# electronicarts/mesh2splat

Measured on AMD Instinct MI355X. Metric: Gaussians/sec emitted (mesh->3DGS conversion pass, density 1024^2), higher is better.
Workload: dtype f32

## Files before the change

### __graft_entry__.py

```python
import os
import subprocess
import sys

ROOT = os.path.dirname(os.path.abspath(__file__))
if ROOT not in sys.path:
    sys.path.insert(0, ROOT)


def build() -> None:
    from mesh2splat_amd import _lib
    _lib.build(force=False)
    _lib.load()
    subprocess.run(["make", "-C", os.path.join(ROOT, "oracle"), "all"], check=True, stdout=subprocess.DEVNULL)
    subprocess.run(["make", "-C", os.path.join(ROOT, "tests", "stub_rccl")], check=True, stdout=subprocess.DEVNULL)
    subprocess.run(["make", "-C", os.path.join(ROOT, "tests", "exact_math")], check=True, stdout=subprocess.DEVNULL)
    import mesh2splat_amd


def smoke() -> None:
    import numpy as np
    from mesh2splat_amd import synth
    from mesh2splat_amd.converter import ConversionPass, RenderContext
    from oracle import oracle

    scene = synth.cube_sphere(24, tex_size=64)
    ctx = RenderContext(scene, resolutionTarget=128, device=0)
    ConversionPass().execute(ctx)
    rec = ctx.converter.download()
    total, ref, _ = oracle.convert(scene, 128)
    assert ctx.numberOfGaussians == total, (ctx.numberOfGaussians, total)
    sys.path.insert(0, os.path.join(ROOT, "tests"))
    from parity import assert_records_match
    assert_records_match(rec, ref, "smoke")
    ran = [ctx.converter.last_pipeline]
    for pipe in ("multipass", "team", "lean"):
        ctx.converter.set_pipeline(pipe)
        assert ctx.converter.convert(128) == total
        assert np.array_equal(ctx.converter.download().view(np.uint32), rec.view(np.uint32)), pipe
        ran.append(ctx.converter.last_pipeline)
    import camera
    from mesh2splat_amd.prepass import PrepassParams
    pp = PrepassParams(view_mat=camera.look_at((1.6, 1.1, 2.3), (0.1, 0.0, -0.1)), proj_mat=camera.perspective(45.0, 16 / 9, 0.01, 100.0),
                       renderer_resolution=(1280, 720), resolution_target=128)
    vis, quads, depths = ctx.converter.prepass(pp)
    ovis, oquads, odepths = oracle.prepass(pp, rec)
    assert vis == ovis and np.array_equal(quads.view(np.uint32), oquads.view(np.uint32)) and np.array_equal(depths, odepths), "prepass"
    sq = ctx.converter.sort_prepass()
    assert np.array_equal(sq.view(np.uint32), oquads[np.argsort(odepths.view(np.uint32), kind="stable")].view(np.uint32)), "sort_prepass"
    assert np.array_equal(ctx.converter.prepass_sorted(pp).view(np.uint32), sq.view(np.uint32)), "prepass_sorted"
    import meshdepth_ref
    img, md_counts = ctx.converter.mesh_depth(pp)
    tri_pos, tri_opaque = meshdepth_ref.scene_triangles(scene)
    want = meshdepth_ref.mesh_depth(tri_pos, tri_opaque, pp.proj_mat, pp.view_mat, pp.model_mat, 1280, 720, want_winner=False)
    assert np.array_equal(img.view(np.uint32), want["image"].view(np.uint32)) and md_counts["drawn"] == want["counts"][0], "mesh_depth"
    occluded = ctx.converter.prepass(ctx.converter._with_device_mesh_depth(pp), download=False)
    assert 0 < occluded < vis, (occluded, vis)
    import tempfile
    from mesh2splat_amd.converter import write_ply
    ctx.converter.set_pipeline("auto")
    t2 = ctx.converter.convert(120)
    assert t2 == oracle.convert(scene, 120, count_only=True)[0]
    rec2 = ctx.converter.download()
    with tempfile.TemporaryDirectory() as d:
        for fmt in (1, 2):
            dev, host, sl = (os.path.join(d, n) for n in ("dev.ply", "host.ply", "slice.ply"))
            ctx.converter.export_ply(dev, fmt, 0.65)
            write_ply(host, rec2, fmt, np.float32(0.65) / np.float32(120))
            assert open(dev, "rb").read() == open(host, "rb").read(), f"device-encoded format {fmt}"
            half = len(rec2) // 2
            ctx.converter.export_ply_slice(sl, fmt, 0.65, half, len(rec2) - half, len(rec2))
            ctx.converter.export_ply_slice(sl, fmt, 0.65, 0, half, len(rec2))
            assert os.path.getsize(sl) == os.path.getsize(dev)
    from mesh2splat_amd.splat import SplatParams
    pp.resolution_target = 120
    ctx.converter.contrib_begin()
    assert ctx.converter.prepass_sorted(pp, download=False) > 0
    ctx.converter.contrib_accumulate(SplatParams((1280, 720), 0))
    wmax, _ = ctx.converter.download_contrib()
    pruned = ctx.converter.prune(0.0, 0)
    assert pruned["before"] == t2 and 0 < pruned["kept"] == int((wmax > 0).sum()) <= t2, pruned
    assert np.array_equal(ctx.converter.download().view(np.uint32), rec2[wmax > 0].view(np.uint32)), "prune"
    print(f"smoke ok: {total} Gaussians, prepass keeps {vis} ({occluded} with the mesh as occluder), bit-identical floats vs oracle: {(rec.view(np.uint32) == ref.view(np.uint32)).mean():.6f}, "
          f"pipelines run: {ran}; new density {t2} Gaussians, device-encoded .ply rows byte-identical to the host writer; "
          f"one view prunes {t2} -> {pruned['kept']}")


if __name__ == "__main__":
    build()
    if len(sys.argv) > 1 and sys.argv[1] == "smoke":
        smoke()
```

### include/m2s.h

```cpp
#ifndef M2S_H
#define M2S_H

#include <stddef.h>
#include <stdint.h>

#ifdef __cplusplus
extern "C" {
#endif

#define M2S_ABI_VERSION 1

typedef enum m2s_status {
    M2S_OK = 0,
    M2S_ERR_INVALID = 1,
    M2S_ERR_NO_DEVICE = 2,
    M2S_ERR_HIP = 3,
    M2S_ERR_OOM = 4,
    M2S_ERR_CAPACITY = 5,
    M2S_ERR_IO = 6,
    M2S_ERR_STATE = 7
} m2s_status;

typedef struct m2s_ctx m2s_ctx;

// ... 151 lines not shown
m2s_status m2s_last_splat_stage_ms(const m2s_ctx* ctx, float out_ms[3]);
m2s_status m2s_last_splat_counts(const m2s_ctx* ctx, uint64_t out[3]);

m2s_status m2s_contrib_begin(m2s_ctx* ctx);
m2s_status m2s_contrib_accumulate(m2s_ctx* ctx, const m2s_splat_params* params, float count_weight);
const void* m2s_device_contrib(const m2s_ctx* ctx, uint32_t which);
m2s_status m2s_download_contrib(m2s_ctx* ctx, uint32_t* dst_wmax, uint32_t* dst_npix, uint64_t capacity);
float m2s_last_contrib_ms(const m2s_ctx* ctx);
m2s_status m2s_last_contrib_stage_ms(const m2s_ctx* ctx, float out_ms[3]);
typedef struct m2s_prune_params {
    float min_weight;
    uint32_t min_pixels;
    uint32_t reserved;
} m2s_prune_params;
m2s_status m2s_prune(m2s_ctx* ctx, const m2s_prune_params* params, uint64_t* out_kept);
m2s_status m2s_last_prune_counts(const m2s_ctx* ctx, uint64_t out[4]);
float m2s_last_prune_ms(const m2s_ctx* ctx);

typedef struct m2s_light_params {
    float light_position[3];
    float light_color[3];
    float light_intensity;
    float camera_position[3];
    float near_far[2];
    int32_t render_mode;
    int32_t resolution[2];
    uint32_t shadow_resolution;
    uint32_t want_shadow_counts;
    uint32_t reserved;
} m2s_light_params;

typedef struct m2s_shadow_quad {
    float mean2d_ndc[4];
    float quad_scale_ndc[4];
    float ws_pos[4];
} m2s_shadow_quad;

m2s_status m2s_shadow(m2s_ctx* ctx, const m2s_prepass_params* prepass, const m2s_light_params* light, const void* d_records, uint64_t n,
                      uint64_t out_per_face[6], uint64_t* out_skipped);
m2s_status m2s_shadow_from_quads(m2s_ctx* ctx, const m2s_light_params* light, const m2s_shadow_quad* host_quads, const uint64_t per_face[6],
                                 uint64_t* out_skipped);
const void* m2s_device_shadow_cubemap(const m2s_ctx* ctx);
m2s_status m2s_download_shadow_cubemap(m2s_ctx* ctx, float* dst, uint64_t capacity_floats);
m2s_status m2s_download_shadow_quads(m2s_ctx* ctx, uint32_t face, m2s_shadow_quad* dst, uint64_t capacity_quads);
m2s_status m2s_upload_shadow_cubemap(m2s_ctx* ctx, const float* host, uint32_t S);
float m2s_last_shadow_ms(const m2s_ctx* ctx);
m2s_status m2s_last_shadow_stage_ms(const m2s_ctx* ctx, float out_ms[3]);
m2s_status m2s_last_shadow_counts(const m2s_ctx* ctx, uint64_t out[9]);

m2s_status m2s_relight(m2s_ctx* ctx, const m2s_light_params* light);
m2s_status m2s_upload_gbuffer(m2s_ctx* ctx, const void* const planes[5], int32_t W, int32_t H);
const void* m2s_device_frame(const m2s_ctx* ctx);
m2s_status m2s_download_frame(m2s_ctx* ctx, void* dst, uint64_t capacity_bytes);
m2s_status m2s_download_shadow_counts(m2s_ctx* ctx, uint8_t* dst, uint64_t capacity_bytes);
float m2s_last_relight_ms(const m2s_ctx* ctx);

typedef struct m2s_mesh_depth_params {
    float world_to_view[16], view_to_clip[16], model_to_world[16];
    int32_t resolution[2];
    uint32_t reserved[2];
} m2s_mesh_depth_params;
m2s_status m2s_mesh_depth(m2s_ctx* ctx, const m2s_mesh_depth_params* params, uint64_t out_counts[5]);
const void* m2s_device_mesh_depth(const m2s_ctx* ctx);
m2s_status m2s_download_mesh_depth(m2s_ctx* ctx, float* dst, uint64_t capacity_floats);
float m2s_last_mesh_depth_ms(const m2s_ctx* ctx);
m2s_status m2s_last_mesh_depth_stage_ms(const m2s_ctx* ctx, float out_ms[3]);
m2s_status m2s_last_mesh_depth_counts(const m2s_ctx* ctx, uint64_t out[5]);
m2s_status m2s_debug_set_mesh_depth_inplace(m2s_ctx* ctx, int32_t max_box);

typedef struct m2s_mesh_render_params {
    float world_to_view[16], view_to_clip[16], model_to_world[16];
    int32_t resolution[2];
    float near_far[2];
    int32_t render_mode;
    uint32_t reserved;
} m2s_mesh_render_params;
m2s_status m2s_mesh_render(m2s_ctx* ctx, const m2s_mesh_render_params* params, uint64_t out_counts[6]);
const void* m2s_device_mesh_gbuffer(const m2s_ctx* ctx, uint32_t attachment);
m2s_status m2s_download_mesh_gbuffer(m2s_ctx* ctx, uint32_t attachment, void* dst, uint64_t capacity_bytes);
m2s_status m2s_download_mesh_visibility(m2s_ctx* ctx, uint64_t* dst, uint64_t capacity_pixels);
float m2s_last_mesh_render_ms(const m2s_ctx* ctx);
m2s_status m2s_last_mesh_render_stage_ms(const m2s_ctx* ctx, float out_ms[4]);
m2s_status m2s_last_mesh_render_counts(const m2s_ctx* ctx, uint64_t out[6]);

m2s_status m2s_relight_split(m2s_ctx* ctx, const m2s_light_params* light, float split_position);

m2s_status m2s_relight_mesh(m2s_ctx* ctx, const m2s_light_params* light);
const void* m2s_device_mesh_frame(const m2s_ctx* ctx);
m2s_status m2s_download_mesh_frame(m2s_ctx* ctx, void* dst, uint64_t capacity_bytes);

enum { M2S_SCORE_NO_COVER = 1, M2S_SCORE_WANT_MAP = 2 };
typedef struct m2s_score_params {
    int32_t  resolution[2];
    uint32_t mask_mode;
    uint32_t flags;
    uint32_t reserved[2];
} m2s_score_params;
typedef struct m2s_score_result {
    uint64_t pixels;
    uint64_t cover[4];
    uint64_t sse[3], sad[3];
    uint32_t max_abs[3], pad;
    uint64_t windows;
    int64_t  ssim_q32;
} m2s_score_result;
m2s_status m2s_score_frames(m2s_ctx* ctx, const m2s_score_params* params, const void* d_a, const void* d_b, const void* d_cover_a,
                            const void* d_cover_b, m2s_score_result* out);
const void* m2s_device_score_map(const m2s_ctx* ctx);
m2s_status m2s_download_score_map(m2s_ctx* ctx, void* dst, uint64_t capacity_bytes);
float m2s_last_score_ms(const m2s_ctx* ctx);

typedef struct m2s_bake_params {
    float model_to_world[16];
    uint32_t degree;
    uint32_t n_theta, n_phi;
    uint32_t use_shadows;
    uint32_t viewer_metallic;
    uint32_t want_shadow_counts;
    uint32_t reserved;
} m2s_bake_params;
m2s_status m2s_bake_light(m2s_ctx* ctx, const m2s_bake_params* params, const m2s_light_params* light, const void* d_records, uint64_t n);
m2s_status m2s_bake_directions(uint32_t n_theta, uint32_t n_phi, float* out, uint64_t capacity_floats);
const void* m2s_device_sh(const m2s_ctx* ctx);
m2s_status m2s_download_sh(m2s_ctx* ctx, float* dst, uint64_t capacity_records);
m2s_status m2s_download_bake_shadow_counts(m2s_ctx* ctx, uint8_t* dst, uint64_t capacity_bytes);
float m2s_last_bake_ms(const m2s_ctx* ctx);
m2s_status m2s_sh_shade_records(m2s_ctx* ctx, const float model_to_world[16], const float camera_position[3], const void* d_records,
                                uint64_t n, void* d_dst);
m2s_status m2s_write_ply_sh(const char* path, const m2s_gaussian* records, const float* sh, uint64_t n, float scale_multiplier);
m2s_status m2s_export_ply_sh(m2s_ctx* ctx, const char* path, float gaussian_std);

m2s_status m2s_write_ply_compact(const char* path, const m2s_gaussian* records, const float* sh, uint32_t sh_degree, uint64_t n,
                                 float scale_multiplier, uint64_t out_counts[3]);
m2s_status m2s_export_ply_compact(m2s_ctx* ctx, const char* path, float gaussian_std, int use_baked_sh, uint64_t out_counts[3]);
m2s_status m2s_last_compact_stage_ms(const m2s_ctx* ctx, float out_ms[4]);

typedef struct m2s_host_scene m2s_host_scene;
m2s_status m2s_load_glb(const char* path, m2s_host_scene** out_scene);
void m2s_free_host_scene(m2s_host_scene* scene);
uint32_t m2s_host_scene_num_meshes(const m2s_host_scene* scene);
const m2s_mesh* m2s_host_scene_meshes(const m2s_host_scene* scene);
const char* m2s_host_scene_mesh_name(const m2s_host_scene* scene, uint32_t i);
const char* m2s_host_scene_warnings(const m2s_host_scene* scene);
m2s_status m2s_read_ply(const char* path, m2s_gaussian** out_records, uint64_t* out_n, int* out_has_pbr);
void m2s_free_records(m2s_gaussian* records);
const char* m2s_io_last_error(void);

enum { M2S_PIPELINE_AUTO = 0, M2S_PIPELINE_MULTIPASS = 1,
       M2S_PIPELINE_TEAM = 3 ,
       M2S_PIPELINE_SPARSE = 4 ,
       M2S_PIPELINE_LEAN = 5  };
m2s_status m2s_set_pipeline(m2s_ctx* ctx, int pipeline);
int m2s_last_pipeline(const m2s_ctx* ctx);

enum { M2S_K_COUNT = 0, M2S_K_SCAN = 1, M2S_K_OFFSETS = 2, M2S_K_EMIT = 3, M2S_K_FUSED = 4, M2S_K_N = 5 };
m2s_status m2s_set_profiling(m2s_ctx* ctx, int enabled);
m2s_status m2s_last_kernel_ms(const m2s_ctx* ctx, float out_ms[M2S_K_N]);
uint64_t m2s_num_triangles(const m2s_ctx* ctx);
m2s_status m2s_debug_set_launch_counter(m2s_ctx* ctx, uint32_t value);

#ifdef __cplusplus
}
#endif
#endif
```

### mesh2splat_amd/_lib.py

```python
from __future__ import annotations

import ctypes as C
import os
import subprocess

_HERE = os.path.dirname(os.path.abspath(__file__))
CSRC = os.path.join(_HERE, "csrc")
LIB_PATH = os.environ.get("M2S_LIB_PATH") or os.path.join(_HERE, "_build", "libm2s_hip.so")

M2S_OK = 0
STATUS_NAMES = {0: "M2S_OK", 1: "M2S_ERR_INVALID", 2: "M2S_ERR_NO_DEVICE", 3: "M2S_ERR_HIP", 4: "M2S_ERR_OOM",
                5: "M2S_ERR_CAPACITY", 6: "M2S_ERR_IO", 7: "M2S_ERR_STATE"}
KERNEL_NAMES = ("count", "scan", "offsets", "emit", "fused")

EXPORTS = (
    "m2s_abi_version", "m2s_create", "m2s_destroy", "m2s_last_error", "m2s_set_triangle_range", "m2s_upload_scene",
    "m2s_set_max_gaussians", "m2s_convert", "m2s_convert_into", "m2s_convert_submit", "m2s_convert_wait", "m2s_last_pipeline", "m2s_set_keep_positions", "m2s_positions_ready", "m2s_debug_set_launch_counter", "m2s_set_async_lanes", "m2s_num_stored", "m2s_device_records", "m2s_download",
    "m2s_download_triangle_counts", "m2s_write_ply", "m2s_export_ply", "m2s_set_profiling", "m2s_last_kernel_ms",
    "m2s_num_triangles", "m2s_set_pipeline", "m2s_load_glb", "m2s_free_host_scene", "m2s_host_scene_num_meshes",
    "m2s_host_scene_meshes", "m2s_host_scene_mesh_name", "m2s_host_scene_warnings", "m2s_read_ply", "m2s_free_records",
    "m2s_io_last_error", "m2s_sort_by_depth", "m2s_device_sorted_records", "m2s_download_sorted", "m2s_last_sort_ms",
    "m2s_upload_records", "m2s_prepass", "m2s_device_quads", "m2s_device_prepass_depths", "m2s_download_prepass", "m2s_last_prepass_ms",
    "m2s_sort_prepass", "m2s_prepass_sorted", "m2s_device_sorted_quads", "m2s_download_sorted_quads", "m2s_last_sort_prepass_ms",
    "m2s_last_upload_ms", "m2s_write_ply_slice", "m2s_export_ply_slice",
    "m2s_dist_unique_id", "m2s_dist_create", "m2s_dist_destroy", "m2s_dist_rank", "m2s_dist_world", "m2s_dist_last_error",
    "m2s_dist_shard_ranges", "m2s_dist_all_gather_counts", "m2s_dist_publish_count", "m2s_dist_collect_counts",
    "m2s_dist_clamp_to_cap", "m2s_dist_gather_records", "m2s_dist_wait", "m2s_set_records", "m2s_reserve_records", "m2s_prepare",
    "m2s_dist_local_id", "m2s_dist_sort_by_depth", "m2s_device_sorted_keys", "m2s_num_sorted", "m2s_last_resolution",
    "m2s_set_resolution_hint", "m2s_last_warm_ms", "m2s_dist_transport", "m2s_last_sort_stage_ms",
    "m2s_splat", "m2s_upload_quads", "m2s_device_gbuffer", "m2s_download_gbuffer", "m2s_last_splat_ms", "m2s_last_splat_stage_ms",
    "m2s_last_splat_counts",
    "m2s_shadow", "m2s_shadow_from_quads", "m2s_device_shadow_cubemap", "m2s_download_shadow_cubemap", "m2s_download_shadow_quads", "m2s_upload_shadow_cubemap",
    "m2s_last_shadow_ms", "m2s_last_shadow_stage_ms", "m2s_last_shadow_counts", "m2s_relight", "m2s_upload_gbuffer", "m2s_device_frame",
    "m2s_download_frame", "m2s_download_shadow_counts", "m2s_last_relight_ms",
    "m2s_mesh_depth", "m2s_device_mesh_depth", "m2s_download_mesh_depth", "m2s_last_mesh_depth_ms", "m2s_last_mesh_depth_stage_ms",
    "m2s_last_mesh_depth_counts", "m2s_debug_set_mesh_depth_inplace",
    "m2s_mesh_render", "m2s_device_mesh_gbuffer", "m2s_download_mesh_gbuffer", "m2s_download_mesh_visibility", "m2s_last_mesh_render_ms",
    "m2s_last_mesh_render_stage_ms", "m2s_last_mesh_render_counts", "m2s_relight_split",
    "m2s_relight_mesh", "m2s_device_mesh_frame", "m2s_download_mesh_frame", "m2s_score_frames", "m2s_device_score_map",
    "m2s_download_score_map", "m2s_last_score_ms",
    "m2s_bake_light", "m2s_bake_directions", "m2s_device_sh", "m2s_download_sh", "m2s_download_bake_shadow_counts", "m2s_last_bake_ms",
    "m2s_sh_shade_records", "m2s_write_ply_sh", "m2s_export_ply_sh",
    "m2s_device_sorted_sources", "m2s_download_sorted_sources", "m2s_upload_quad_sources", "m2s_contrib_begin", "m2s_contrib_accumulate", "m2s_device_contrib",
    "m2s_download_contrib", "m2s_last_contrib_ms", "m2s_last_contrib_stage_ms", "m2s_prune", "m2s_last_prune_counts", "m2s_last_prune_ms",
    "m2s_write_ply_compact", "m2s_export_ply_compact", "m2s_last_compact_stage_ms",
)


class M2SError(RuntimeError):
    def __init__(self, status: int, message: str):
        super().__init__(f"{STATUS_NAMES.get(status, status)}: {message}")
        self.status = status


class Texture(C.Structure):
    _fields_ = [("rgba8", C.c_void_p), ("width", C.c_uint32), ("height", C.c_uint32)]


class MeshC(C.Structure):
    _fields_ = [("vertices", C.c_void_p), ("n_vertices", C.c_uint32), ("stride_floats", C.c_uint32),
                ("bbox_min", C.c_float * 3), ("bbox_max", C.c_float * 3), ("base_color", C.c_float * 4),
                ("tex", Texture * 3)]


def build(force: bool = False) -> str:
    srcs = [os.path.join(CSRC, f) for f in os.listdir(CSRC)] + [os.path.join(_HERE, "..", "include", "m2s.h")]
    stale = (not os.path.exists(LIB_PATH)) or any(os.path.getmtime(s) > os.path.getmtime(LIB_PATH) for s in srcs)
    if force or stale:
        r = subprocess.run(["make", "-C", CSRC, "all"], stdout=subprocess.PIPE, stderr=subprocess.STDOUT, text=True)
        if r.returncode:
            raise RuntimeError("building libm2s_hip.so failed:\n" + r.stdout)
    return LIB_PATH


_lib = None


def _preload_torch_hip_runtime():
    import importlib.util
    import sys
    if "torch" in sys.modules:
        return
    try:
        spec = importlib.util.find_spec("torch")
        if spec is None or not spec.submodule_search_locations:
            return
        cand = os.path.join(list(spec.submodule_search_locations)[0], "lib", "libamdhip64.so")
        if os.path.exists(cand):
            C.CDLL(cand, mode=C.RTLD_GLOBAL)
    except Exception:
        pass


def load():
    global _lib
    if _lib is not None:
        return _lib
    if not os.path.exists(LIB_PATH):
        raise ImportError(f"{LIB_PATH} is missing: run `python -c 'import __graft_entry__ as g; g.build()'` "
                          "(there is no CPU fallback for the conversion pass)")
    _preload_torch_hip_runtime()
    L = C.CDLL(LIB_PATH)
    vp, u32, u64, i64 = C.c_void_p, C.c_uint32, C.c_uint64, C.c_int64
    sigs = {
        "m2s_abi_version": (u32, []),
        "m2s_create": (C.c_int, [C.c_int, C.POINTER(vp)]),
        "m2s_destroy": (None, [vp]),
        "m2s_last_error": (C.c_char_p, [vp]),
        "m2s_set_triangle_range": (C.c_int, [vp, u64, u64]),
        "m2s_upload_scene": (C.c_int, [vp, C.POINTER(MeshC), u32]),
        "m2s_set_max_gaussians": (C.c_int, [vp, i64]),
        "m2s_convert": (C.c_int, [vp, u32, C.POINTER(u64)]),
        "m2s_convert_into": (C.c_int, [vp, u32, vp, u64, vp, C.POINTER(u64)]),
        "m2s_convert_submit": (C.c_int, [vp, u32, vp, u64, vp]),
        "m2s_convert_wait": (C.c_int, [vp, C.POINTER(u64)]),
        "m2s_upload_records": (C.c_int, [vp, vp, u64]),
        "m2s_prepass": (C.c_int, [vp, vp, vp, u64, C.POINTER(u64)]),
        "m2s_device_quads": (vp, [vp]),
        "m2s_device_prepass_depths": (vp, [vp]),
        "m2s_download_prepass": (C.c_int, [vp, vp, vp, u64]),
        "m2s_last_prepass_ms": (C.c_float, [vp]),
        "m2s_sort_prepass": (C.c_int, [vp, C.POINTER(u64)]),
        "m2s_prepass_sorted": (C.c_int, [vp, vp, C.POINTER(u64)]),
        "m2s_device_sorted_quads": (vp, [vp]),
        "m2s_download_sorted_quads": (C.c_int, [vp, vp, u64]),
        "m2s_last_sort_prepass_ms": (C.c_float, [vp]),
        "m2s_last_pipeline": (C.c_int, [vp]),
        "m2s_set_keep_positions": (C.c_int, [vp, C.c_int]),
        "m2s_positions_ready": (C.c_int, [vp]),
        "m2s_debug_set_launch_counter": (C.c_int, [vp, u32]),
        "m2s_set_async_lanes": (C.c_int, [vp, C.c_int]),
        "m2s_num_stored": (u64, [vp]),
        "m2s_device_records": (vp, [vp]),
        "m2s_download": (C.c_int, [vp, vp, u64]),
        "m2s_download_triangle_counts": (C.c_int, [vp, vp, u64]),
        "m2s_write_ply": (C.c_int, [C.c_char_p, vp, u64, u32, C.c_float]),
        "m2s_export_ply": (C.c_int, [vp, C.c_char_p, u32, C.c_float]),
        "m2s_set_profiling": (C.c_int, [vp, C.c_int]),
        "m2s_last_kernel_ms": (C.c_int, [vp, C.POINTER(C.c_float)]),
        "m2s_num_triangles": (u64, [vp]),
        "m2s_set_pipeline": (C.c_int, [vp, C.c_int]),
        "m2s_load_glb": (C.c_int, [C.c_char_p, C.POINTER(vp)]),
        "m2s_free_host_scene": (None, [vp]),
        "m2s_host_scene_num_meshes": (u32, [vp]),
        "m2s_host_scene_meshes": (C.POINTER(MeshC), [vp]),
        "m2s_host_scene_mesh_name": (C.c_char_p, [vp, u32]),
        "m2s_host_scene_warnings": (C.c_char_p, [vp]),
        "m2s_read_ply": (C.c_int, [C.c_char_p, C.POINTER(vp), C.POINTER(u64), C.POINTER(C.c_int)]),
        "m2s_free_records": (None, [vp]),
        "m2s_io_last_error": (C.c_char_p, []),
        "m2s_sort_by_depth": (C.c_int, [vp, C.POINTER(C.c_float), C.POINTER(u64)]),
        "m2s_device_sorted_records": (vp, [vp]),
        "m2s_download_sorted": (C.c_int, [vp, vp, u64]),
        "m2s_last_sort_ms": (C.c_float, [vp]),
        "m2s_last_upload_ms": (C.c_int, [vp, C.POINTER(C.c_float)]),
        "m2s_write_ply_slice": (C.c_int, [C.c_char_p, vp, u64, u32, C.c_float, u64, u64]),
        "m2s_export_ply_slice": (C.c_int, [vp, C.c_char_p, u32, C.c_float, u64, u64, u64]),
        "m2s_dist_unique_id": (C.c_int, [vp]),
        "m2s_dist_create": (C.c_int, [C.c_int, vp, C.c_int, C.c_int, C.POINTER(vp)]),
        "m2s_dist_destroy": (None, [vp]),
        "m2s_dist_rank": (C.c_int, [vp]),
        "m2s_dist_world": (C.c_int, [vp]),
        "m2s_dist_last_error": (C.c_char_p, [vp]),
        "m2s_dist_shard_ranges": (C.c_int, [C.POINTER(MeshC), u32, u32, C.c_int, C.POINTER(u64), C.POINTER(u64)]),
        "m2s_dist_all_gather_counts": (C.c_int, [vp, u64, C.POINTER(u64), C.POINTER(u64)]),
        "m2s_dist_publish_count": (C.c_int, [vp, u64]),
        "m2s_dist_collect_counts": (C.c_int, [vp, C.POINTER(u64), C.POINTER(u64)]),
        "m2s_dist_clamp_to_cap": (None, [C.POINTER(u64), C.c_int, u64, C.POINTER(u64)]),
        "m2s_dist_gather_records": (C.c_int, [vp, vp, C.POINTER(u64), vp, C.c_int, vp]),
        "m2s_dist_wait": (C.c_int, [vp, vp]),
        "m2s_set_records": (C.c_int, [vp, vp, u64, u32]),
        "m2s_reserve_records": (C.c_int, [vp, u64, C.POINTER(vp)]),
        "m2s_prepare": (C.c_int, [vp, u32]),
        "m2s_dist_local_id": (C.c_int, [C.c_int, vp]),
        "m2s_dist_sort_by_depth": (C.c_int, [vp, vp, C.POINTER(C.c_float), C.POINTER(u64), C.POINTER(u64)]),
        "m2s_device_sorted_keys": (vp, [vp]),
        "m2s_num_sorted": (u64, [vp]),
        "m2s_last_resolution": (u32, [vp]),
        "m2s_set_resolution_hint": (C.c_int, [vp, u32]),
        "m2s_last_warm_ms": (C.c_float, [vp]),
        "m2s_dist_transport": (C.c_char_p, [vp]),
        "m2s_last_sort_stage_ms": (C.c_int, [vp, C.POINTER(C.c_float)]),
        "m2s_splat": (C.c_int, [vp, vp, vp, u64, C.POINTER(u64)]),
        "m2s_upload_quads": (C.c_int, [vp, vp, u64]),
        "m2s_device_gbuffer": (vp, [vp, u32]),
        "m2s_download_gbuffer": (C.c_int, [vp, u32, vp, u64]),
        "m2s_last_splat_ms": (C.c_float, [vp]),
        "m2s_last_splat_stage_ms": (C.c_int, [vp, C.POINTER(C.c_float)]),
        "m2s_last_splat_counts": (C.c_int, [vp, C.POINTER(u64)]),
        "m2s_shadow": (C.c_int, [vp, vp, vp, vp, u64, C.POINTER(u64), C.POINTER(u64)]),
        "m2s_shadow_from_quads": (C.c_int, [vp, vp, vp, C.POINTER(u64), C.POINTER(u64)]),
        "m2s_device_shadow_cubemap": (vp, [vp]),
        "m2s_download_shadow_cubemap": (C.c_int, [vp, vp, u64]),
        "m2s_download_shadow_quads": (C.c_int, [vp, u32, vp, u64]),
        "m2s_upload_shadow_cubemap": (C.c_int, [vp, vp, u32]),
        "m2s_last_shadow_ms": (C.c_float, [vp]),
        "m2s_last_shadow_stage_ms": (C.c_int, [vp, C.POINTER(C.c_float)]),
        "m2s_last_shadow_counts": (C.c_int, [vp, C.POINTER(u64)]),
        "m2s_relight": (C.c_int, [vp, vp]),
        "m2s_upload_gbuffer": (C.c_int, [vp, C.POINTER(vp), C.c_int32, C.c_int32]),
        "m2s_device_frame": (vp, [vp]),
        "m2s_download_frame": (C.c_int, [vp, vp, u64]),
        "m2s_download_shadow_counts": (C.c_int, [vp, vp, u64]),
        "m2s_last_relight_ms": (C.c_float, [vp]),
        "m2s_mesh_depth": (C.c_int, [vp, vp, C.POINTER(u64)]),
        "m2s_device_mesh_depth": (vp, [vp]),
        "m2s_download_mesh_depth": (C.c_int, [vp, vp, u64]),
        "m2s_last_mesh_depth_ms": (C.c_float, [vp]),
        "m2s_last_mesh_depth_stage_ms": (C.c_int, [vp, C.POINTER(C.c_float)]),
        "m2s_last_mesh_depth_counts": (C.c_int, [vp, C.POINTER(u64)]),
        "m2s_debug_set_mesh_depth_inplace": (C.c_int, [vp, C.c_int32]),
        "m2s_mesh_render": (C.c_int, [vp, vp, C.POINTER(u64)]),
        "m2s_device_mesh_gbuffer": (vp, [vp, C.c_uint32]),
        "m2s_download_mesh_gbuffer": (C.c_int, [vp, C.c_uint32, vp, u64]),
        "m2s_download_mesh_visibility": (C.c_int, [vp, vp, u64]),
        "m2s_last_mesh_render_ms": (C.c_float, [vp]),
        "m2s_last_mesh_render_stage_ms": (C.c_int, [vp, C.POINTER(C.c_float)]),
        "m2s_last_mesh_render_counts": (C.c_int, [vp, C.POINTER(u64)]),
        "m2s_relight_split": (C.c_int, [vp, vp, C.c_float]),
        "m2s_relight_mesh": (C.c_int, [vp, vp]),
        "m2s_device_mesh_frame": (vp, [vp]),
        "m2s_download_mesh_frame": (C.c_int, [vp, vp, u64]),
        "m2s_score_frames": (C.c_int, [vp, vp, vp, vp, vp, vp, vp]),
        "m2s_device_score_map": (vp, [vp]),
        "m2s_download_score_map": (C.c_int, [vp, vp, u64]),
        "m2s_last_score_ms": (C.c_float, [vp]),
        "m2s_bake_light": (C.c_int, [vp, vp, vp, vp, u64]),
        "m2s_bake_directions": (C.c_int, [u32, u32, vp, u64]),
        "m2s_device_sh": (vp, [vp]),
        "m2s_download_sh": (C.c_int, [vp, vp, u64]),
        "m2s_download_bake_shadow_counts": (C.c_int, [vp, vp, u64]),
        "m2s_last_bake_ms": (C.c_float, [vp]),
        "m2s_sh_shade_records": (C.c_int, [vp, vp, vp, vp, u64, vp]),
        "m2s_write_ply_sh": (C.c_int, [C.c_char_p, vp, vp, u64, C.c_float]),
        "m2s_export_ply_sh": (C.c_int, [vp, C.c_char_p, C.c_float]),
        "m2s_device_sorted_sources": (vp, [vp]),
        "m2s_download_sorted_sources": (C.c_int, [vp, vp, u64]),
        "m2s_upload_quad_sources": (C.c_int, [vp, vp, u64]),
        "m2s_contrib_begin": (C.c_int, [vp]),
        "m2s_contrib_accumulate": (C.c_int, [vp, vp, C.c_float]),
        "m2s_device_contrib": (vp, [vp, u32]),
        "m2s_download_contrib": (C.c_int, [vp, vp, vp, u64]),
        "m2s_last_contrib_ms": (C.c_float, [vp]),
        "m2s_last_contrib_stage_ms": (C.c_int, [vp, C.POINTER(C.c_float)]),
        "m2s_prune": (C.c_int, [vp, vp, C.POINTER(u64)]),
        "m2s_last_prune_counts": (C.c_int, [vp, C.POINTER(u64)]),
        "m2s_last_prune_ms": (C.c_float, [vp]),
        "m2s_write_ply_compact": (C.c_int, [C.c_char_p, vp, vp, u32, u64, C.c_float, C.POINTER(u64)]),
        "m2s_export_ply_compact": (C.c_int, [vp, C.c_char_p, C.c_float, C.c_int, C.POINTER(u64)]),
        "m2s_last_compact_stage_ms": (C.c_int, [vp, C.POINTER(C.c_float)]),
    }
    for name, (res, args) in sigs.items():
        fn = getattr(L, name)
        fn.restype = res
        fn.argtypes = args
    _lib = L
    return L
```

### mesh2splat_amd/converter.py

```python
from __future__ import annotations

import ctypes as C
import os
from typing import Optional

import numpy as np

from . import _lib
from .scene import RECORD_FLOATS, TEXTURE_SLOTS, Scene


def marshal_scene(scene: Scene):
    n = scene.n_meshes
    arr = (_lib.MeshC * max(1, n))()
    keep = []
    for i, m in enumerate(scene.meshes):
        v = np.ascontiguousarray(m.vertices, np.float32)
        keep.append(v)
        arr[i].vertices = v.ctypes.data
        arr[i].n_vertices = v.shape[0]
        arr[i].stride_floats = v.shape[1]
        for k in range(3):
            arr[i].bbox_min[k] = float(m.bbox_min[k])
            arr[i].bbox_max[k] = float(m.bbox_max[k])
# ... 611 lines not shown
            raise ValueError(f"{what} holds {img.numel() * img.element_size()} bytes, W x H x 4 is {nbytes}")
        return img.data_ptr(), True

    def score_frames(self, params, a=None, b=None, cover_a=None, cover_b=None, download_map: bool = False):
        from . import score as _sc
        pc = _sc.to_c(params)
        W, H = int(pc.resolution[0]), int(pc.resolution[1])
        ptrs, tensors = [], False
        for img, what in ((a, "a"), (b, "b"), (cover_a, "cover_a"), (cover_b, "cover_b")):
            ptr, is_tensor = self._image_ptr(img, what, max(W, 0) * max(H, 0) * 4)
            ptrs.append(ptr)
            tensors = tensors or is_tensor
        if tensors:
            import torch
            torch.cuda.current_stream().synchronize()
        out = _sc.ScoreResultC()
        self._check(self._L.m2s_score_frames(self._h, C.byref(pc), ptrs[0], ptrs[1], ptrs[2], ptrs[3], C.byref(out)))
        res = _sc.ScoreResult.from_c(out)
        if download_map:
            res.error_map = self.download_score_map(W, H)
        return res

    def download_score_map(self, W: int, H: int) -> np.ndarray:
        m = np.empty((int(H), int(W), 4), np.uint8)
        self._check(self._L.m2s_download_score_map(self._h, m.ctypes.data, m.nbytes))
        return m

    @property
    def device_score_map(self) -> int:
        return int(self._L.m2s_device_score_map(self._h) or 0)

    @property
    def last_score_ms(self) -> float:
        return float(self._L.m2s_last_score_ms(self._h))

    def score(self, prepass_params, light_params, mask_mode: int = 2, mesh_depth_test: bool = False, want_map: bool = False):
        from . import score as _sc
        self.render_frame(prepass_params, light_params, mesh_depth_test=mesh_depth_test, download=False)
        self.mesh_render(prepass_params, download=False)
        self.relight_mesh(light_params, download=False)
        res = tuple(int(v) for v in prepass_params.renderer_resolution)
        return self.score_frames(_sc.ScoreParams(res, int(mask_mode), False, bool(want_map)), download_map=bool(want_map))

    def score_views(self, cameras, resolution_target: int, light_position, light_intensity: float, gaussian_std: float = 0.65,
                    render_mode: int = 6, shadow_resolution: int = 1024, mask_mode: int = 2, mesh_depth_test: bool = False):
        from . import score as _sc
        views = [self.score(*cam.frame_params(resolution_target, light_position, light_intensity, gaussian_std, render_mode, shadow_resolution),
                            mask_mode=mask_mode, mesh_depth_test=mesh_depth_test) for cam in cameras]
        return views, _sc.pool(views)

    @property
    def device_sorted_sources(self) -> int:
        return int(self._L.m2s_device_sorted_sources(self._h) or 0)

    def download_sorted_sources(self, n: int) -> np.ndarray:
        out = np.empty(int(n), np.uint32)
        self._check(self._L.m2s_download_sorted_sources(self._h, out.ctypes.data, out.size))
        return out

    def upload_quad_sources(self, sources):
        s = np.ascontiguousarray(sources, np.uint32).reshape(-1)
        self._check(self._L.m2s_upload_quad_sources(self._h, s.ctypes.data if s.size else None, s.size))

    def contrib_begin(self):
        self._check(self._L.m2s_contrib_begin(self._h))

    def contrib_accumulate(self, params, count_weight: float = 1.0 / 255.0):
        from . import splat as _sp
        pc = _sp.to_c(params)
        self._check(self._L.m2s_contrib_accumulate(self._h, C.byref(pc), C.c_float(count_weight)))

    def download_contrib(self):
        n = self.num_stored
        w = np.empty(n, np.float32)
        k = np.empty(n, np.uint32)
        self._check(self._L.m2s_download_contrib(self._h, w.ctypes.data, k.ctypes.data, n))
        return w, k

    def device_contrib(self, which: int) -> int:
        return int(self._L.m2s_device_contrib(self._h, int(which)) or 0)

    @property
    def last_contrib_ms(self) -> float:
        return float(self._L.m2s_last_contrib_ms(self._h))

    def last_contrib_stage_ms(self) -> dict:
        ms = (C.c_float * 3)()
        self._check(self._L.m2s_last_contrib_stage_ms(self._h, ms))
        return {"setup_bin": float(ms[0]), "grouping": float(ms[1]), "blend": float(ms[2])}

    def prune(self, min_weight: float = 0.0, min_pixels: int = 0) -> dict:
        from . import prune as _pr
        pc = _pr.PruneParamsC(float(min_weight), int(min_pixels), 0)
        kept = C.c_uint64()
        had_plane = bool(self.device_sh)
        self._check(self._L.m2s_prune(self._h, C.byref(pc), C.byref(kept)))
        counts = self.last_prune_counts()
        if had_plane and getattr(self, "_last_bake_n", None) == counts["before"]:
            self._last_bake_n = counts["kept"]
        return counts

    def last_prune_counts(self) -> dict:
        v = (C.c_uint64 * 4)()
        self._check(self._L.m2s_last_prune_counts(self._h, v))
        return {"before": int(v[0]), "kept": int(v[1]), "dropped_weight": int(v[2]), "dropped_pixels": int(v[3])}

    @property
    def last_prune_ms(self) -> float:
        return float(self._L.m2s_last_prune_ms(self._h))

    def prune_views(self, cameras, resolution_target: int, size=None, gaussian_std: float = 0.65, count_weight: float = 1.0 / 255.0,
                    min_weight: float = 1.0 / 255.0, min_pixels: int = 1) -> dict:
        import dataclasses
        from . import splat as _sp
        if size is not None:
            size = (int(size[0]), int(size[1]))
        self.contrib_begin()
        for cam in cameras:
            pp, _ = cam.frame_params(resolution_target, (0.0, 0.0, 0.0), 0.0, gaussian_std)
            if size is not None:
                pp = dataclasses.replace(pp, renderer_resolution=size)
            if self.prepass_sorted(pp, download=False):
                self.contrib_accumulate(_sp.SplatParams(tuple(pp.renderer_resolution), 0), count_weight)
        return self.prune(min_weight, min_pixels)

    @property
    def last_shadow_ms(self) -> float:
        return float(self._L.m2s_last_shadow_ms(self._h))

    def last_shadow_stage_ms(self) -> dict:
        ms = (C.c_float * 3)()
        self._check(self._L.m2s_last_shadow_stage_ms(self._h, ms))
        return {"quads": float(ms[0]), "bin": float(ms[1]), "raster": float(ms[2])}

    def last_shadow_counts(self) -> dict:
        v = (C.c_uint64 * 9)()
        self._check(self._L.m2s_last_shadow_counts(self._h, v))
        return {"quads_per_face": [int(v[k]) for k in range(6)], "pairs": int(v[6]), "texel_updates": int(v[7]), "skipped": int(v[8])}

    @property
    def last_relight_ms(self) -> float:
        return float(self._L.m2s_last_relight_ms(self._h))

    def set_pipeline(self, name: str):
        self._check(self._L.m2s_set_pipeline(self._h, {"auto": 0, "multipass": 1, "team": 3, "sparse": 4, "lean": 5}[name]))

    def set_async_lanes(self, lanes: int):
        self._check(self._L.m2s_set_async_lanes(self._h, int(lanes)))

    @property
    def last_pipeline(self) -> str:
        return {0: "none", 1: "multipass", 3: "team", 4: "sparse", 5: "lean"}[self._L.m2s_last_pipeline(self._h)]

    def set_profiling(self, on: bool):
        self._check(self._L.m2s_set_profiling(self._h, 1 if on else 0))

    def last_kernel_ms(self) -> dict:
        ms = (C.c_float * len(_lib.KERNEL_NAMES))()
        self._check(self._L.m2s_last_kernel_ms(self._h, ms))
        return {k: float(ms[i]) for i, k in enumerate(_lib.KERNEL_NAMES)}


def write_ply(path: str, records: np.ndarray, fmt: int, scale_multiplier: float):
    r = np.ascontiguousarray(records, np.float32)
    if r.ndim != 2 or r.shape[1] != RECORD_FLOATS:
        raise ValueError("records must be (n, 24) float32")
    st = _lib.load().m2s_write_ply(os.fsencode(path), r.ctypes.data, r.shape[0], int(fmt), float(scale_multiplier))
    if st != _lib.M2S_OK:
        raise _lib.M2SError(st, f"could not write {path}")


def write_ply_compact(path: str, records: np.ndarray, scale_multiplier: float, sh: np.ndarray | None = None, sh_degree: int = 0) -> dict:
    r = np.ascontiguousarray(records, np.float32).reshape(-1, RECORD_FLOATS)
    p = None
    if sh is not None:
        p = np.ascontiguousarray(sh, np.float32)
        if p.shape != (r.shape[0], 48):
            raise ValueError("sh must be (n, 48) float32")
    counts = (C.c_uint64 * 3)()
    st = _lib.load().m2s_write_ply_compact(os.fsencode(path), r.ctypes.data if r.size else None, p.ctypes.data if p is not None else None,
                                           int(sh_degree), r.shape[0], float(scale_multiplier), counts)
    if st != _lib.M2S_OK:
        raise _lib.M2SError(st, f"could not write {path}")
    return {"rows": int(counts[0]), "chunks": int(counts[1]), "skipped": int(counts[2])}


def write_ply_slice(path: str, records: np.ndarray, fmt: int, scale_multiplier: float, first_row: int, total_rows: int):
    r = np.ascontiguousarray(records, np.float32).reshape(-1, RECORD_FLOATS)
    st = _lib.load().m2s_write_ply_slice(os.fsencode(path), r.ctypes.data, r.shape[0], int(fmt), float(scale_multiplier),
                                         int(first_row), int(total_rows))
    if st != _lib.M2S_OK:
        raise _lib.M2SError(st, f"could not write {path}")


class RenderContext:

    def __init__(self, scene: Optional[Scene] = None, resolutionTarget: int = 520, gaussianStd: float = 0.65,
                 device: int = 0):
        self.scene = scene
        self.resolutionTarget = int(resolutionTarget)
        self.gaussianStd = float(gaussianStd)
        self.numberOfGaussians = 0
        self.device = int(device)
        self.converter: Optional[Converter] = None
        self.rendererResolution = (1280, 720)
        self.renderMode = 0
        self.gBuffer = None
        self.splatSkipped = 0
        self.prepassParams = None
        self.lightParams = None
        self.shadowCubemap = None
        self.mesh_depth = None
        self.frame = None
        self.meshGBuffer = None
        self.splitScreenEnabled = False
        self.splitScreenPosition = 0.5
        self._uploaded_scene = None


class IRenderPass:

    def __init__(self):
        self._enabled = False

    def execute(self, context: RenderContext):
        raise NotImplementedError

    def isEnabled(self) -> bool:
        return self._enabled

    def setIsEnabled(self, enabled: bool):
        self._enabled = bool(enabled)


class ConversionPass(IRenderPass):

    def execute(self, context: RenderContext):
        if context.scene is None:
            raise ValueError("RenderContext.scene is not set (SceneManager::loadModel has not run)")
        if context.converter is None:
            context.converter = Converter(context.device)
        if context._uploaded_scene is not context.scene:
            context.converter.set_resolution_hint(context.resolutionTarget)
            context.converter.upload_scene(context.scene)
            context._uploaded_scene = context.scene
        context.numberOfGaussians = context.converter.convert(context.resolutionTarget)


class DepthPrepass(IRenderPass):

    def execute(self, context: RenderContext):
        if context.converter is None or context.prepassParams is None or context._uploaded_scene is None:
            raise RuntimeError("needs an uploaded scene (ConversionPass) and context.prepassParams")
        context.mesh_depth, _ = context.converter.mesh_depth(context.prepassParams)
        if context.prepassParams.perform_mesh_depth_test:
            context.prepassParams.mesh_depth = context.mesh_depth


class MeshRenderPass(IRenderPass):

    def execute(self, context: RenderContext):
        if context.converter is None or context.prepassParams is None or context._uploaded_scene is None:
            raise RuntimeError("needs an uploaded scene (ConversionPass) and context.prepassParams")
        context.meshGBuffer, _ = context.converter.mesh_render(context.prepassParams)


class GaussianSplattingPass(IRenderPass):

    def execute(self, context: RenderContext):
        from .splat import SplatParams
        if context.converter is None:
            raise RuntimeError("no quads: run the conversion, the prepass and the depth sort first")
        res = getattr(context, "rendererResolution", (1280, 720))
        mode = getattr(context, "renderMode", 0)
        context.gBuffer, context.splatSkipped = context.converter.splat(SplatParams(renderer_resolution=tuple(res), render_mode=int(mode)))


class GaussianShadowPass(IRenderPass):

    def execute(self, context: RenderContext):
        if context.converter is None or context.prepassParams is None or context.lightParams is None:
            raise RuntimeError("needs converted records, context.prepassParams and context.lightParams")
        _, _, context.shadowCubemap = context.converter.shadow(context.prepassParams, context.lightParams)


class GaussianRelightingPass(IRenderPass):

    def execute(self, context: RenderContext):
        if context.converter is None or context.lightParams is None:
            raise RuntimeError("needs a G-buffer, a shadow cube and context.lightParams")
        if context.splitScreenEnabled and context.meshGBuffer is not None:
            r = context.converter.relight_split(context.lightParams, context.splitScreenPosition)
        else:
            r = context.converter.relight(context.lightParams)
        context.frame = r[0] if isinstance(r, tuple) else r


class SceneManager:

    def __init__(self, context: RenderContext):
        self.renderContext = context

    def exportPly(self, outputFile: str, exportFormat: int = 0):
        ctx = self.renderContext
        if ctx.converter is None:
            raise RuntimeError("nothing converted yet")
# ... 2 lines not shown
```

### mesh2splat_amd/csrc/m2s_context.cpp

```cpp
#include "m2s_ctx.h"
#include "m2s_ply.h"

#include <algorithm>
#include <array>
#include <chrono>
#include <cstdio>
#include <cstring>
#include <string>
#include <thread>
#include <tuple>
#include <vector>

using namespace m2s;
using namespace m2s_host;

namespace {
thread_local std::string g_create_error = "";
}

namespace m2s_host {
void free_scene(m2s_ctx* c) {
    if (c->tri_mem) (void)hipFree(c->tri_mem);
    if (c->scene_arena) (void)hipFree(c->scene_arena);
    if (c->d_chain_b) (void)hipFree(c->d_chain_b);
    if (c->d_setup) (void)hipFree(c->d_setup);
    if (c->d_off_b) (void)hipFree(c->d_off_b);
    if (c->d_start_b) (void)hipFree(c->d_start_b);
    if (c->d_setup_b) (void)hipFree(c->d_setup_b);
    if (c->d_total_b) (void)hipFree(c->d_total_b);
    c->d_chain_b = nullptr; c->d_setup = nullptr;
    c->d_off_b = nullptr; c->d_start_b = nullptr; c->start_b_cap = 0; c->d_setup_b = nullptr; c->d_total_b = nullptr;
    c->tri_mem = nullptr; c->scene_arena = nullptr;
    c->d_meshes = nullptr; c->d_mesh_first = nullptr;
    c->d_cnt = c->d_off = c->d_partials = nullptr;
    c->d_chain = nullptr; c->d_biglist = nullptr; c->d_bigmeta = nullptr; c->d_bands = nullptr; c->run_table_words = 0; c->d_run_order = nullptr; c->run_order_unit = 0;
    c->d_batch_first = nullptr; c->n_batch_tab = 0; c->chain_words = 0;
    c->rinfo.clear();
    ++c->rinfo_gen;
    c->frag_per_R2 = -1.0;
    c->warm_R = 0; c->warm_total = 0; c->warm_mismatch_seen = false;
    c->sparse_off_R = c->team_off_R = c->lean_off_R = UINT32_MAX;
    c->lean_ok = false;
    c->scene = SceneDev{};
    c->has_scene = false;
}

m2s_ctx::RInfo& rinfo_for(m2s_ctx* c, uint32_t R) {
    auto it = c->rinfo.find(R);
    if (it != c->rinfo.end()) return it->second;
    if (c->rinfo.size() >= (size_t)kBandSlots) { drain_in_flight(c); c->rinfo.clear(); ++c->rinfo_gen; }
    m2s_ctx::RInfo ri;
    ri.gen = c->rinfo_gen;
    ri.band_slot = (int)c->rinfo.size();
    return c->rinfo.emplace(R, ri).first->second;
}

static bool spin_waits() { static const bool on = !debug_on("M2S_NO_SPIN"); return on; }
template <class Query, class Block>
static hipError_t spin_then_block(Query query, Block block) {
    if (spin_waits()) {
        const auto t0 = std::chrono::steady_clock::now();
        for (uint32_t i = 0;; ++i) {
            const hipError_t e = query();
            if (e != hipErrorNotReady) return e;
            if ((i & 15u) == 15u && std::chrono::steady_clock::now() - t0 > std::chrono::microseconds(400)) break;
        }
        (void)hipGetLastError();
    }
    return block();
}
hipError_t wait_stream(hipStream_t st) { return spin_then_block([&] { return hipStreamQuery(st); }, [&] { return hipStreamSynchronize(st); }); }
hipError_t wait_event(hipEvent_t ev) { return spin_then_block([&] { return hipEventQuery(ev); }, [&] { return hipEventSynchronize(ev); }); }

void drain_in_flight(m2s_ctx* c) {
    for (uint32_t k = 0; k < c->slot_count; ++k) {
        auto& sl = c->slot[(c->slot_head + k) % M2S_MAX_IN_FLIGHT];
        if (!sl.sync_result) (void)hipEventSynchronize(sl.done);
    }
}

hipError_t next_epoch(m2s_ctx* c, uint32_t* out) {
    const uint32_t e = ++c->epoch;
    *out = e;
    if ((e & 0xFFFFu) != 0) return hipSuccess;
    const size_t bytes = std::max<size_t>(c->chain_words, 1) * sizeof(unsigned long long);
    hipError_t r = hipDeviceSynchronize();
    if (r == hipSuccess && c->d_chain) r = hipMemset(c->d_chain, 0, bytes);
    if (r == hipSuccess && c->d_chain_b) r = hipMemset(c->d_chain_b, 0, bytes);
    return r;
}

m2s_status ensure_records(m2s_ctx* c, uint64_t want) {
    if (c->records_cap >= want && c->d_records) return M2S_OK;
    uint64_t grow = std::max<uint64_t>(want, 1);
    if (c->records_cap) grow = std::max(grow, 2 * c->records_cap);
    if (c->cap_policy < 0) grow = std::max(want, std::min<uint64_t>(grow, kMaxGaussiansToSort));
    drain_in_flight(c);
    if (c->d_records && c->last_records == c->d_records) { c->last_records = nullptr; c->last_stored = 0; }
    if (c->d_records) { (void)hipFree(c->d_records); c->d_records = nullptr; c->records_cap = 0; }
    hipError_t e = hipMalloc(&c->d_records, grow * sizeof(m2s_gaussian));
    if (e != hipSuccess && grow > want) { grow = want; e = hipMalloc(&c->d_records, grow * sizeof(m2s_gaussian)); }
    HIPCHK(c, e);
    c->records_cap = grow;
    for (uint32_t k = 0; k < c->slot_count; ++k) {
        auto& sl = c->slot[(c->slot_head + k) % M2S_MAX_IN_FLIGHT];
        if (sl.own_lane == 0) { sl.d_out = c->d_records; sl.gen = c->buf_gen[0] - 1u; }
    }
    return M2S_OK;
}
}

extern "C" {

uint32_t m2s_abi_version(void) { return M2S_ABI_VERSION; }

const char* m2s_last_error(const m2s_ctx* ctx) { return ctx ? ctx->err.c_str() : g_create_error.c_str(); }

m2s_status m2s_create(int device, m2s_ctx** out_ctx) {
    if (!out_ctx) { g_create_error = "out_ctx is NULL"; return M2S_ERR_INVALID; }
    *out_ctx = nullptr;
    int n = 0;
    hipError_t e = hipGetDeviceCount(&n);
    if (e != hipSuccess || n <= 0) {
        g_create_error = std::string("no HIP device available (") + (e != hipSuccess ? hipGetErrorString(e) : "count=0") +
                         "); this library has no CPU path";
        return M2S_ERR_NO_DEVICE;
    }
    if (device < 0 || device >= n) { g_create_error = "device index out of range"; return M2S_ERR_NO_DEVICE; }
    m2s_ctx* c = new (std::nothrow) m2s_ctx();
    if (!c) { g_create_error = "host allocation failed"; return M2S_ERR_OOM; }
    c->device = device;
    auto bail = [&](const char* what, hipError_t he) {
        g_create_error = std::string(what) + ": " + hipGetErrorString(he);
        delete c;
        return M2S_ERR_HIP;
    };
    if ((e = hipSetDevice(device)) != hipSuccess) return bail("hipSetDevice", e);
    if ((e = hipStreamCreateWithFlags(&c->stream, hipStreamNonBlocking)) != hipSuccess) return bail("hipStreamCreate", e);
    if ((e = hipMalloc(&c->d_total, sizeof(unsigned long long))) != hipSuccess) return bail("hipMalloc", e);
    if ((e = hipHostMalloc((void**)&c->h_total, m2s_ctx::kPinnedWords * sizeof(unsigned long long), hipHostMallocDefault)) != hipSuccess)
        return bail("hipHostMalloc", e);
    for (auto& ev : c->ev)
        if ((e = hipEventCreate(&ev)) != hipSuccess) return bail("hipEventCreate", e);
    for (auto& ev : c->stage_ev)
        if ((e = hipEventCreateWithFlags(&ev, hipEventDisableTiming)) != hipSuccess) return bail("hipEventCreate", e);
    unsigned done_flags = hipEventDisableTiming;
    if (const char* v = debug_env("M2S_DONE_EVENT_FLAGS")) {
        const unsigned f = (unsigned)strtoul(v, nullptr, 0);
        if ((f & ~(hipEventBlockingSync | hipEventDisableTiming | hipEventReleaseToDevice | hipEventReleaseToSystem)) == 0u) done_flags = f;
    }
    for (auto& sl : c->slot)
        if ((e = hipEventCreateWithFlags(&sl.done, done_flags)) != hipSuccess || (e = hipEventCreate(&sl.t0)) != hipSuccess ||
            (e = hipEventCreate(&sl.t1)) != hipSuccess)
            return bail("hipEventCreate", e);
    *out_ctx = c;
    return M2S_OK;
}

void m2s_destroy(m2s_ctx* c) {
    if (!c) return;
    (void)hipSetDevice(c->device);
    if (c->stream) (void)hipStreamSynchronize(c->stream);
    drain_in_flight(c);
    free_scene(c);
    if (c->d_start) (void)hipFree(c->d_start);
    if (c->d_records) (void)hipFree(c->d_records);
    if (c->d_records_b) (void)hipFree(c->d_records_b);
    if (c->stream_b) { (void)hipStreamSynchronize(c->stream_b); (void)hipStreamDestroy(c->stream_b); }
    for (int k = 0; k < 2; ++k) {
        if (c->h_stage[k]) (void)hipHostFree(c->h_stage[k]);
        if (c->d_stage[k]) (void)hipFree(c->d_stage[k]);
        if (c->stage_ev[k]) (void)hipEventDestroy(c->stage_ev[k]);
    }
    if (c->d_total) (void)hipFree(c->d_total);
    if (c->h_total) (void)hipHostFree(c->h_total);
    for (auto& ev : c->ev) if (ev) (void)hipEventDestroy(ev);
    for (auto& sl : c->slot) {
        if (sl.done) (void)hipEventDestroy(sl.done);
        if (sl.t0) (void)hipEventDestroy(sl.t0);
        if (sl.t1) (void)hipEventDestroy(sl.t1);
    }
    if (c->stream) (void)hipStreamDestroy(c->stream);
    delete c;
}

m2s_status m2s_set_triangle_range(m2s_ctx* c, uint64_t first, uint64_t count) {
    if (!c) return M2S_ERR_INVALID;
    c->range_first = first;
    c->range_count = count;
    return M2S_OK;
}

m2s_status m2s_set_max_gaussians(m2s_ctx* c, int64_t cap) {
    if (!c) return M2S_ERR_INVALID;
    if (cap < -1) return fail(c, M2S_ERR_INVALID, "cap must be -1 (reference formula), 0 (unlimited) or > 0");
    c->cap_policy = cap;
    return M2S_OK;
}

m2s_status m2s_set_profiling(m2s_ctx* c, int enabled) {
    if (!c) return M2S_ERR_INVALID;
    c->profiling = enabled != 0;
    return M2S_OK;
}

m2s_status m2s_set_pipeline(m2s_ctx* c, int pipeline) {
    if (!c) return M2S_ERR_INVALID;
    if (pipeline < M2S_PIPELINE_AUTO || pipeline > M2S_PIPELINE_LEAN) return fail(c, M2S_ERR_INVALID, "unknown pipeline");
    if (pipeline == 2) return fail(c, M2S_ERR_INVALID, "pipeline 2 (the one-wave-per-batch kernel of rounds 1-5) no longer exists: use M2S_PIPELINE_TEAM");
    if (c->slot_count) return fail(c, M2S_ERR_STATE, kInFlightMsg);
    if (c->pipeline != pipeline) {
        c->rinfo.clear();
        ++c->rinfo_gen;
    }
    c->pipeline = pipeline;
    return M2S_OK;
}

int m2s_last_pipeline(const m2s_ctx* c) { return c ? c->last_pipeline : 0; }

int m2s_positions_ready(const m2s_ctx* c) {
    return c && c->d_pos_plane && c->last_records && c->pos_plane_of == c->last_records && c->pos_plane_n == c->last_stored &&
           c->pos_plane_epoch == c->records_epoch && c->last_stored ? 1 : 0;
}

m2s_status m2s_set_keep_positions(m2s_ctx* c, int enabled) {
    if (!c) return M2S_ERR_INVALID;
    c->keep_positions = enabled != 0;
    return M2S_OK;
}

m2s_status m2s_debug_set_launch_counter(m2s_ctx* c, uint32_t value) {
    if (!c) return M2S_ERR_INVALID;
    if (c->slot_count) return fail(c, M2S_ERR_STATE, kInFlightMsg);
    c->epoch = value;
    return M2S_OK;
}

m2s_status m2s_set_async_lanes(m2s_ctx* c, int lanes) {
    if (!c) return M2S_ERR_INVALID;
    if (lanes != 1 && lanes != 2) return fail(c, M2S_ERR_INVALID, "lanes must be 1 or 2");
    if (c->slot_count) return fail(c, M2S_ERR_STATE, kInFlightMsg);
    c->lanes = lanes;
    return M2S_OK;
}

m2s_status m2s_last_kernel_ms(const m2s_ctx* c, float out_ms[M2S_K_N]) {
    if (!c || !out_ms) return M2S_ERR_INVALID;
    memcpy(out_ms, c->last_ms, sizeof c->last_ms);
    return M2S_OK;
}

}
```

### mesh2splat_amd/csrc/m2s_ctx.h

```cpp
#pragma once
#include "../../include/m2s.h"
#include "m2s_devbuf.h"
#include "m2s_device.h"

#include <cstdint>
#include <cstdlib>
#include <map>
#include <string>

namespace m2s_host {
constexpr uint32_t kMaxGaussiansToSort = 7000000u;
constexpr uint64_t kMaxTriangles = (1ull << 28) - 1;
inline size_t align_up(size_t v, size_t a) { return (v + a - 1) / a * a; }
inline const char* const kStaleMsg = "the records of the conversion last waited for have been overwritten by a later submission at another R "
                                     "(wait for it, or submit into your own buffers)";
inline const char* const kInFlightMsg = "conversions are still in flight: m2s_convert_wait first";
struct GBufPlanes {
    DevBuf<void> plane[5];
    void* ptr[5] = {};
    m2s_status reserve(std::string& err, uint64_t px) {
        for (int k = 0; k < 5; ++k) {
            const m2s_status s = plane[k].reserve(err, px, (k == 2 || k == 4) ? 4 : 8);
            ptr[k] = plane[k].get();
            if (s) return s;
        }
        return M2S_OK;
    }
};
}

constexpr int kBandSlotsMax = 64;
struct m2s_ctx {
    int device = 0;
    hipStream_t stream = nullptr;
    std::string err;

    void* tri_mem = nullptr;
    m2s::SceneDev scene{};
    m2s::MeshParams* d_meshes = nullptr;
    uint32_t* d_mesh_first = nullptr;
    uint32_t n_meshes_total = 0;
    bool has_scene = false;
    bool lean_ok = false;
    uint64_t range_first = 0, range_count = UINT64_MAX;

    uint32_t* d_cnt = nullptr;
    uint32_t* d_off = nullptr;
    uint32_t* d_partials = nullptr;
    uint32_t* d_start = nullptr;
    size_t start_cap = 0;
    unsigned long long* d_total = nullptr;
    unsigned long long* h_total = nullptr;
    static constexpr int kPinnedPrepass = 2 + 2 * M2S_MAX_IN_FLIGHT;
    static constexpr int kPinnedSortMM = 4 + 2 * M2S_MAX_IN_FLIGHT;
    static constexpr int kPinnedWords = 6 + 2 * M2S_MAX_IN_FLIGHT;
    unsigned long long* d_chain = nullptr;
    m2s::BigItem* d_biglist = nullptr;
    uint32_t* d_bigmeta = nullptr;
    struct RInfo {
        int form = M2S_PIPELINE_AUTO;
        uint32_t tpw = 0;
        bool async_ok = false;
        bool mp_ready = false;
        bool bands_ready = false;
        uint32_t bands_unit = 0;
        int band_slot = 0;
        uint32_t gen = 0;
    };
    uint32_t sparse_off_R = UINT32_MAX, team_off_R = UINT32_MAX, lean_off_R = UINT32_MAX;
    uint32_t rinfo_gen = 0;
    std::map<uint32_t, RInfo> rinfo;
    double frag_per_R2 = -1.0;
    uint64_t warm_total = 0;
    uint64_t warm_big = 0;
    bool warm_mismatch_seen = false;
    uint32_t hint_R = 0;
    uint32_t warm_R = 0;
    int warm_spec_form = 0;
    uint32_t warm_spec_unit = 0, warm_spec_shift = 0;
    unsigned long long* d_bands = nullptr;
    size_t run_table_words = 0;
    uint32_t* d_run_order = nullptr;
    uint32_t run_order_unit = 0, run_order_shift = 0;
    uint32_t* d_batch_first = nullptr;
    uint32_t n_batch_tab = 0;
    size_t chain_words = 0;
    void* d_setup = nullptr;
    int last_pipeline = 0;
    int lanes = 1;
    hipStream_t stream_b = nullptr;
    unsigned long long* d_chain_b = nullptr;
    void* d_records_b = nullptr;
    uint64_t records_b_cap = 0;
    uint32_t* d_off_b = nullptr;
    uint32_t* d_start_b = nullptr;
    size_t start_b_cap = 0;
    void* d_setup_b = nullptr;
    unsigned long long* d_total_b = nullptr;
    int pipeline = M2S_PIPELINE_AUTO;
    uint32_t epoch = 0;

    struct Slot { hipEvent_t done = nullptr, t0 = nullptr, t1 = nullptr; uint64_t limit = 0; void* d_out = nullptr; uint32_t R = 0;
                  bool sync_result = false; uint64_t sync_total = 0; bool prof = false; float ms[M2S_K_N] = {};
                  int own_lane = -1; uint32_t gen = 0;
                  bool wrote_bands = false; uint32_t bands_unit = 0; uint32_t ri_gen = 0;
                  hipStream_t st = nullptr; bool shared_work = false; };
    Slot slot[M2S_MAX_IN_FLIGHT];
    uint32_t slot_head = 0, slot_count = 0;
    hipStream_t last_submit_stream = nullptr;
    uint32_t buf_R[2] = { 0, 0 };
    uint32_t buf_gen[2] = { 0, 0 };
    bool records_stale = false;

    void* d_records = nullptr;
    uint64_t records_cap = 0;
    const void* last_records = nullptr;
    int64_t cap_policy = -1;
    uint64_t last_total = 0, last_stored = 0;
    uint32_t last_R = 0;

    m2s_host::DevBuf<float4> d_sorted;
    uint64_t sorted_n = 0;
    m2s_host::DevBuf<uint32_t> d_sort_u32;
    uint32_t sorted_key_offset = 0;
    m2s_host::DevBuf<void> d_sort_temp;
    float last_sort_ms = 0.0f;
    float last_sort_stage_ms[3] = { 0, 0, 0 };
    m2s_host::DevBuf<float4> d_pos_plane;
    uint64_t pos_plane_n = 0, pos_plane_epoch = 0;
    const void* pos_plane_of = nullptr;
    bool keep_positions = false;
    uint64_t records_epoch = 1;
    m2s_host::DevBuf<float4> d_quads;
    m2s_host::DevBuf<float> d_pp_depths;
    uint64_t pp_visible = 0;
    m2s_host::DevBuf<unsigned long long> d_pp_chain;
    uint32_t pp_epoch = 0;
    m2s_host::DevBuf<float> d_pp_depthtex;
    float last_prepass_ms = 0.0f;
    m2s_host::PinnedBuf<m2s_gaussian> h_export[2];
    void* h_stage[2] = { nullptr, nullptr };
    void* d_stage[2] = { nullptr, nullptr };
    hipEvent_t stage_ev[2] = { nullptr, nullptr };
    void* scene_arena = nullptr;
    float last_upload_ms[5] = { 0, 0, 0, 0, 0 };
    m2s_host::DevBuf<uint8_t> d_rows;
    m2s_host::DevBuf<void> d_loaded;
    m2s_host::DevBuf<float4> d_sorted_quads;
    uint64_t sq_n = 0;
    float last_sort_prepass_ms = 0.0f;
    m2s_host::GBufPlanes d_gbuf;
    int32_t gbuf_w = 0, gbuf_h = 0;
    m2s_host::BinWork splat_work;
    m2s_host::DevBuf<uint32_t> d_splat_tiles;
    float last_splat_ms = 0.0f;
    float last_splat_stage_ms[3] = { 0, 0, 0 };
    uint64_t last_splat_counts[3] = { 0, 0, 0 };
    const uint32_t* sq_src = nullptr;
    uint64_t sq_src_epoch = 0;
    m2s_host::DevBuf<uint32_t> d_sq_src;
    m2s_host::DevBuf<uint32_t> d_contrib;
    uint64_t contrib_n = 0, contrib_epoch = 0;
    const void* contrib_of = nullptr;
    bool contrib_active = false;
    float last_contrib_ms = 0.0f;
    float last_contrib_stage_ms[3] = { 0, 0, 0 };
    m2s_host::DevBuf<uint32_t> d_prune_u32;
    m2s_host::DevBuf<char> d_prune_temp;
    m2s_host::DevBuf<float4> d_prune_stage;
    uint64_t last_prune_counts[4] = { 0, 0, 0, 0 };
    float last_prune_ms = 0.0f;
    m2s_host::EventSet<2> prune_ev;
    m2s_host::DevBuf<float4> d_shadow_quads;
    uint32_t shadow_base[7] = { 0, 0, 0, 0, 0, 0, 0 };
    bool shadow_lists = false;
    m2s_host::DevBuf<float> d_shadow_cube;
    int32_t shadow_S = 0;
    m2s_host::DevBuf<uint32_t> d_sh_tab;
    m2s_host::DevBuf<float> d_sh_views;
    m2s_host::BinWork shadow_work;
    m2s_host::EventSet<10> light_ev;
    float last_shadow_ms = 0.0f;
    float last_shadow_stage_ms[3] = { 0, 0, 0 };
    uint64_t last_shadow_counts[9] = {};
    m2s_host::DevBuf<uint32_t> d_frame;
    m2s_host::DevBuf<uint8_t> d_shadow_counts;
    int32_t frame_w = 0, frame_h = 0;
    bool frame_has_counts = false;
    float last_relight_ms = 0.0f;
    m2s_host::DevBuf<float> d_md_image;
    int32_t md_w = 0, md_h = 0;
    int32_t md_inplace = -1;
    m2s_host::DevBuf<uint32_t> d_md_deferred;
    m2s_host::BinWork md_work;
    m2s_host::EventSet<6> md_ev;
    float last_md_ms = 0.0f;
    float last_md_stage_ms[3] = { 0, 0, 0 };
// ... 106 lines not shown
```

### mesh2splat_amd/csrc/m2s_devfn.h

```cpp
#pragma once
#include "m2s_device.h"
#include "m2s_exact.h"

#pragma clang fp contract(off)

namespace m2s {

__device__ __forceinline__ float len3(float x, float y, float z) { return sqrtf((x * x + y * y) + z * z); }
__device__ __forceinline__ float len3sq(float x, float y, float z) { return (x * x + y * y) + z * z; }
__device__ __forceinline__ float inv_len3(float x, float y, float z) {
    const float q = len3sq(x, y, z);
    if (wave_all(in_sqrt_range(q))) return rcp_rn(sqrt_rn(q));
    return 1.0f / sqrtf(q);
}

__device__ __forceinline__ uint32_t wave_incl_scan(uint32_t v, int ) {
    v += (uint32_t)__builtin_amdgcn_update_dpp(0, (int)v, 0x111, 0xf, 0xf, true);
    v += (uint32_t)__builtin_amdgcn_update_dpp(0, (int)v, 0x112, 0xf, 0xf, true);
    v += (uint32_t)__builtin_amdgcn_update_dpp(0, (int)v, 0x114, 0xf, 0xf, true);
    v += (uint32_t)__builtin_amdgcn_update_dpp(0, (int)v, 0x118, 0xf, 0xf, true);
    v += (uint32_t)__builtin_amdgcn_update_dpp(0, (int)v, 0x142, 0xa, 0xf, true);
    v += (uint32_t)__builtin_amdgcn_update_dpp(0, (int)v, 0x143, 0xc, 0xf, true);
    return v;
}
__device__ __forceinline__ uint32_t wave_sum(uint32_t v) {
    return (uint32_t)__builtin_amdgcn_readlane((int)wave_incl_scan(v, 0), 63);
}
__device__ __forceinline__ void wave_lds_sync() {
    __builtin_amdgcn_fence(__ATOMIC_RELEASE, "workgroup");
    __builtin_amdgcn_wave_barrier();
    __builtin_amdgcn_fence(__ATOMIC_ACQUIRE, "workgroup");
}

__device__ __forceinline__ double rcp_f64(double d) {
    double y = __builtin_amdgcn_rcp(d);
    double e = __builtin_fma(-d, y, 1.0);
    y = __builtin_fma(e, y, y);
    e = __builtin_fma(-d, y, 1.0);
    return __builtin_fma(e, y, y);
}
__device__ __forceinline__ long long floordivmod_by(long long num, long long den, double y, long long& rem) {
    long long q = (long long)floor((double)num * y);
    long long r = num - q * den;
    if (r < 0) { q -= 1; r += den; }
    else if (r >= den) { q += 1; r -= den; }
    rem = r;
    return q;
}
__device__ __forceinline__ long long floordiv_pos(long long num, long long den) {
    long long r;
    return floordivmod_by(num, den, rcp_f64((double)den), r);
}

typedef const __attribute__((address_space(4))) MeshParams* ConstMeshPtr;
__device__ __forceinline__ ConstMeshPtr kConstMesh(const MeshParams* p) { return (ConstMeshPtr)p; }

struct Geo {
    float xx, xy, xz;
    float nx, ny, nz;
    float ou[3], ov[3];
};

__device__ __forceinline__ void geo_setup(const float p[9], const float* __restrict__ bmin,
                                          const float* __restrict__ bmax, Geo& g) {
    float e1x = p[3] - p[0], e1y = p[4] - p[1], e1z = p[5] - p[2];
    float e2x = p[6] - p[0], e2y = p[7] - p[1], e2z = p[8] - p[2];
    float e3x = p[6] - p[3], e3y = p[7] - p[4], e3z = p[8] - p[5];
    const float q1 = len3sq(e1x, e1y, e1z), q2 = len3sq(e2x, e2y, e2z), q3 = len3sq(e3x, e3y, e3z);
    const bool fast_len = wave_all(in_sqrt_range3(q1, q2, q3));
    float l1, l2, l3;
    if (fast_len) { l1 = sqrt_rn(q1); l2 = sqrt_rn(q2); l3 = sqrt_rn(q3); }
    else { l1 = sqrtf(q1); l2 = sqrtf(q2); l3 = sqrtf(q3); }
    float ls = l1;
    if (l2 > l1 && l2 > l3) {
        float tx = e1x, ty = e1y, tz = e1z;
        e1x = e2x; e1y = e2y; e1z = e2z;
        e2x = tx; e2y = ty; e2z = tz;
        ls = l2;
    } else if (l3 > l1 && l3 > l2) {
        e1x = e3x; e1y = e3y; e1z = e3z;
        ls = l3;
    }
    float inv;
    if (fast_len) inv = rcp_rn(ls);
    else inv = 1.0f / ls;
    g.xx = e1x * inv; g.xy = e1y * inv; g.xz = e1z * inv;
    float cx = g.xy * e2z - g.xz * e2y, cy = g.xz * e2x - g.xx * e2z, cz = g.xx * e2y - g.xy * e2x;
    inv = inv_len3(cx, cy, cz);
    g.nx = cx * inv; g.ny = cy * inv; g.nz = cz * inv;
    float ax = fabsf(g.nx), ay = fabsf(g.ny), az = fabsf(g.nz);
    const bool first = (ax > ay) && (ax > az);
    const bool second = !first && (ay > az);
    const bool useY_asA = first;
    const bool useY_asB = !first && !second;
    float bminA = useY_asA ? bmin[1] : bmin[0], bmaxA = useY_asA ? bmax[1] : bmax[0];
    float bminB = useY_asB ? bmin[1] : bmin[2], bmaxB = useY_asB ? bmax[1] : bmax[2];
    float range = fmaxf(bmaxA - bminA, bmaxB - bminB);
    float ra[3], rb[3];
#pragma unroll
    for (int i = 0; i < 3; i++) {
        const float pa = useY_asA ? p[3 * i + 1] : p[3 * i + 0];
        const float pb = useY_asB ? p[3 * i + 1] : p[3 * i + 2];
        ra[i] = pa - bminA;
        rb[i] = pb - bminB;
    }
    const float lo = fminf(fminf(fminf(fabsf(ra[0]), fabsf(ra[1])), fabsf(ra[2])), fminf(fminf(fabsf(rb[0]), fabsf(rb[1])), fminf(fabsf(rb[2]), range)));
    const float hi = fmaxf(fmaxf(fmaxf(fabsf(ra[0]), fabsf(ra[1])), fabsf(ra[2])), fmaxf(fmaxf(fabsf(rb[0]), fabsf(rb[1])), fmaxf(fabsf(rb[2]), range)));
    if (wave_all(lo >= kDivLo && hi <= kDivHi)) {
        const float y = rcp_rn(range);
#pragma unroll
        for (int i = 0; i < 3; i++) { g.ou[i] = div_rn(ra[i], range, y); g.ov[i] = div_rn(rb[i], range, y); }
    } else {
#pragma unroll
        for (int i = 0; i < 3; i++) { g.ou[i] = ra[i] / range; g.ov[i] = rb[i] / range; }
    }
}

template <class MP>
__device__ __forceinline__ void geo_setup_mp(const float p[9], MP mp, Geo& g) {
    const float bmin[3] = { mp->bmin[0], mp->bmin[1], mp->bmin[2] }, bmax[3] = { mp->bmax[0], mp->bmax[1], mp->bmax[2] };
    geo_setup(p, bmin, bmax, g);
}

__device__ __forceinline__ float i64_to_f32(long long v) {
    const double d = __builtin_fma((double)(int)(v >> 32), 4294967296.0, (double)(unsigned)v);
    return (float)d;
}

__device__ __forceinline__ float fma_(float a, float b, float c) { return __builtin_fmaf(a, b, c); }
__device__ __forceinline__ float dot3_(float ax, float ay, float az, float bx, float by, float bz) { return fma_(az, bz, fma_(ay, by, ax * bx)); }
__device__ __forceinline__ float fast_rcp(float x) { return __builtin_amdgcn_rcpf(x); }
__device__ __forceinline__ float fast_rsq(float x) { return __builtin_amdgcn_rsqf(x); }
__device__ __forceinline__ float fast_sqrt(float x) { return __builtin_amdgcn_sqrtf(x); }
__device__ __forceinline__ float fast_log2(float x) { return __builtin_amdgcn_logf(x); }

__device__ __forceinline__ void geo_flat(const float p[9], const Geo& g, float& sx, float& sy, float4& rot) {
    float cx = g.ny * g.xz - g.nz * g.xy, cy = g.nz * g.xx - g.nx * g.xz, cz = g.nx * g.xy - g.ny * g.xx;
    const float inv = inv_len3(cx, cy, cz);
    float yx = cx * inv, yy = cy * inv, yz = cz * inv;
    const float m00 = g.xx, m01 = g.xy, m02 = g.xz;
    const float m10 = yx, m11 = yy, m12 = yz;
    const float m20 = g.nx, m21 = g.ny, m22 = g.nz;
    float fx = m00 - m11 - m22, fy = m11 - m00 - m22, fz = m22 - m00 - m11, fw = m00 + m11 + m22;
    int bi = 0;
    float fb = fw;
    if (fx > fb) { fb = fx; bi = 1; }
    if (fy > fb) { fb = fy; bi = 2; }
    if (fz > fb) { fb = fz; bi = 3; }
    {
        const float bv = fast_sqrt(fb + 1.0f) * 0.5f;
        const float mult = 0.25f * fast_rcp(bv);
        const float d0 = m12 - m21, d1 = m20 - m02, d2 = m01 - m10;
        const float s0 = m01 + m10, s1 = m20 + m02, s2 = m12 + m21;
        float qw, qx, qy, qz;
        if (bi == 0) { qw = bv; qx = d0 * mult; qy = d1 * mult; qz = d2 * mult; }
// ... 286 lines not shown
                    else k1 = f < k1 ? f : k1;
                } else k1 = -1;
            }
        }
    }
    w.x0 = s.x0; w.x1 = s.x1;
    w.lower = 0;
    if (k0 > k1) { k0 = 0; k1 = -1; }
    w.k0 = (int)k0; w.k1 = (int)k1;
    const int yy = y + (int)k0 * stride;
    const long long steps = k1 - k0;
    const long long Py = 256ll * yy + 128;
    bool safe = true;
#pragma unroll
    for (int i = 0; i < 3; i++) {
        const long long alpha = 256ll * s.a[i];
        const long long beta = 128ll * s.a[i] + (long long)s.b[i] * Py + s.c[i] + ((s.bias >> i) & 1);
        const long long bs = 256ll * s.b[i] * stride;
        long long q;
        walker_edge(alpha, beta, bs, q, w.r[i], w.sq[i], w.sr[i], w.D[i]);
        if (alpha > 0 || alpha == 0) w.lower |= 1 << i;
        if (alpha == 0) { q = -2 * kWalk32; w.D[i] = 1u; }
        else if (steps >= 0) {
            const float qe = fabsf((float)q + (float)(int)steps * (float)w.sq[i]);
            safe = safe && (q >> 29) == (q >> 63) && qe < 268435456.0f;
        }
        w.q[i] = (int)q;
    }
    return safe || steps < 0;
}
__device__ __forceinline__ uint32_t jump_quot(unsigned long long x, uint32_t D, uint32_t& rem) {
    uint32_t e = (uint32_t)((float)x * __builtin_amdgcn_rcpf((float)D));
    long long r = (long long)x - (long long)((unsigned long long)e * D);
    if (r < 0) { e -= 1u; r += D; }
    else if (r >= (long long)D) { e += 1u; r -= D; }
    rem = (uint32_t)r;
    return e;
}
__device__ __forceinline__ void row_walker32_jump(RowWalker32& w, uint32_t d) {
#pragma unroll
    for (int i = 0; i < 3; i++) {
        uint32_t rem;
        const uint32_t e = jump_quot((unsigned long long)w.r[i] + (unsigned long long)d * w.sr[i], w.D[i], rem);
        w.q[i] = (int)((uint32_t)w.q[i] + d * (uint32_t)w.sq[i] + e);
        w.r[i] = rem;
    }
}
__device__ __forceinline__ void row_walker32_next(RowWalker32& w, int& xa, int& xb) {
    int lo = w.x0, hi = w.x1;
#pragma unroll
    for (int i = 0; i < 3; i++) {
        const bool l = (w.lower >> i) & 1;
        const int ql = l ? w.q[i] : (int)0x80000000, qh = l ? 0x7FFFFFFF : w.q[i];
        lo = ql > lo ? ql : lo;
        hi = qh < hi ? qh : hi;
        const uint32_t t = w.r[i] + w.sr[i];
        const bool c = t >= w.D[i];
        w.r[i] = c ? t - w.D[i] : t;
        w.q[i] += w.sq[i] + (c ? 1 : 0);
    }
    xa = lo; xb = hi;
}

__device__ __forceinline__ Raster shfl_raster(const Raster& s, int src) {
    Raster r;
#pragma unroll
    for (int i = 0; i < 3; i++) {
        r.a[i] = __shfl(s.a[i], src);
        r.b[i] = __shfl(s.b[i], src);
        r.c[i] = __shfl(s.c[i], src);
    }
    r.area2 = 0;
    r.bias = __shfl(s.bias, src);
    r.ext = 0;
    r.x0 = __shfl(s.x0, src); r.x1 = __shfl(s.x1, src);
    r.y0 = __shfl(s.y0, src); r.y1 = __shfl(s.y1, src);
    return r;
}

__device__ __forceinline__ void load_positions(const TriPlanes& tp, uint32_t t, float p[9]) {
    float4 a0 = tp.A0[t], a1 = tp.A1[t];
    float a2 = tp.A2[t];
    p[0] = a0.x; p[1] = a0.y; p[2] = a0.z; p[3] = a0.w;
    p[4] = a1.x; p[5] = a1.y; p[6] = a1.z; p[7] = a1.w;
    p[8] = a2;
}

__device__ __forceinline__ uint32_t find_mesh(const SceneDev& sc, uint32_t gt) {
    uint32_t lo = 0, hi = sc.n_meshes;
    while (hi - lo > 1) {
        uint32_t mid = (lo + hi) >> 1;
        if (sc.mesh_first[mid] <= gt) lo = mid; else hi = mid;
    }
    return lo;
}

__device__ __forceinline__ uint32_t mesh_of_range(const SceneDev& sc, uint32_t t0, uint32_t t_last, bool& uniform) {
    const __attribute__((address_space(4))) uint32_t* q = (const __attribute__((address_space(4))) uint32_t*)sc.mesh_of8;
    const uint32_t m = q[2u * (t0 >> 3)], end = q[2u * (t0 >> 3) + 1u];
    uniform = end > t_last;
    return m;
}

__device__ __forceinline__ bool setup_raster_for(const SceneDev& sc, uint32_t t, uint32_t mesh_hint, bool uniform_mesh,
                                                 uint32_t R, Raster& rs) {
    float p[9];
    load_positions(sc.tri, t, p);
    uint32_t m = uniform_mesh ? mesh_hint : find_mesh(sc, sc.tri_first + t);
    const MeshParams* mp = sc.meshes + m;
    Geo g;
    geo_setup(p, mp->bmin, mp->bmax, g);
    return raster_setup(g, R, rs);
}

constexpr float kUnorm8 = 0.003921568859368563f;

struct __attribute__((packed, aligned(4))) ComboPair { uint32_t v[6]; };

typedef const __attribute__((address_space(1))) char* GlobalBytes;
__device__ __forceinline__ GlobalBytes as_global(const void* p) { return (GlobalBytes)p; }
__device__ __forceinline__ ComboPair ld_combo(GlobalBytes base, uint32_t dword_off) {
    const __attribute__((address_space(1))) uint32_t* p = reinterpret_cast<const __attribute__((address_space(1))) uint32_t*>(base + (size_t)(dword_off * 4u));
    ComboPair r;
#pragma unroll
    for (int i = 0; i < 6; ++i) r.v[i] = p[i];
    return r;
}
__device__ __forceinline__ uint32_t ld_texel(GlobalBytes base, uint32_t texel) {
    return *reinterpret_cast<const __attribute__((address_space(1))) uint32_t*>(base + (size_t)(texel * 4u));
}


struct TriShade {
    int a1, b1, a2, b2;
    long long e1, e2;
    float inva, sx, sy, lod0;
    float4 rot;
    float lod1, lod2;
    uint32_t org;
    uint32_t mesh;
};
static_assert(sizeof(TriShade) == 80, "TriShade must be five float4");

struct TriShadeS {
    short a1, b1, a2, b2;
    int e1, e2;
    float inva, sx, sy, lod0;
    float4 rot;
    float lod1, lod2;
    uint32_t org;
    uint32_t mesh;
};
static_assert(sizeof(TriShadeS) == 64, "TriShadeS must be four float4");

__device__ __forceinline__ float lod_from_grad(float fw, float fh, float dudx, float dvdx, float dudy, float dvdy) {
    const float sx = dudx * fw, tx = dvdx * fh, sy = dudy * fw, ty = dvdy * fh;
    const float r2 = fmaxf(fma_(tx, tx, sx * sx), fma_(ty, ty, sy * sy));
    return 0.5f * fast_log2(r2);
}

template <class MP, class TS>
__device__ __forceinline__ void tri_shade_rest(const float p[9], const Geo& g, int a1, int b1, int a2, int b2, MP mp,
                                               float4 b0, float2 b1uv, TS& ts) {
    ts.mesh = 0;
    const float A1 = (float)a1 * 256.0f * ts.inva, B1 = (float)b1 * 256.0f * ts.inva;
    const float A2 = (float)a2 * 256.0f * ts.inva, B2 = (float)b2 * 256.0f * ts.inva;
    geo_flat(p, g, ts.sx, ts.sy, ts.rot);
    ts.lod0 = ts.lod1 = ts.lod2 = 0.0f;
    const auto ta = &mp->tex[0];
    const auto tn = &mp->tex[1];
    const auto tm = &mp->tex[2];
    const bool hasA = ta->texels != nullptr, hasN = tn->texels != nullptr, hasM = tm->texels != nullptr;
    if (hasA || hasN || hasM) {
        const float du1 = b0.z - b0.x, du2 = b1uv.x - b0.x, dv1 = b0.w - b0.y, dv2 = b1uv.y - b0.y;
        const float dudx = fma_(A2, du2, A1 * du1), dvdx = fma_(A2, dv2, A1 * dv1);
        const float dudy = fma_(B2, du2, B1 * du1), dvdy = fma_(B2, dv2, B1 * dv1);
        if (hasA) ts.lod0 = lod_from_grad((float)ta->w, (float)ta->h, dudx, dvdx, dudy, dvdy);
        if (hasN) ts.lod1 = (hasA && tn->w == ta->w && tn->h == ta->h) ? ts.lod0
                          : lod_from_grad((float)tn->w, (float)tn->h, dudx, dvdx, dudy, dvdy);
        if (hasM) ts.lod2 = (hasA && tm->w == ta->w && tm->h == ta->h) ? ts.lod0
                          : (hasN && tm->w == tn->w && tm->h == tn->h) ? ts.lod1
                          : lod_from_grad((float)tm->w, (float)tm->h, dudx, dvdx, dudy, dvdy);
        if (mp->combo.texels != nullptr) {
            const uint32_t nl = ta->n_levels;
            const float q = (float)(nl - 1), lambda = ts.lod0;
            float d = 0.0f, f = 0.0f;
            if (lambda > 0.0f) {
                if (lambda >= q) d = q;
                else { d = floorf(lambda); f = lambda - d; }
            }
            const uint32_t l0 = (uint32_t)d, l1 = min(l0 + 1u, nl - 1u);
            const uint32_t c1 = mp->combo.coff[1], c2 = mp->combo.coff[2], c3 = mp->combo.coff[3], c4 = mp->combo.coff[4];
            const uint32_t off0 = l0 == 0 ? 0u : l0 == 1 ? c1 : l0 == 2 ? c2 : l0 == 3 ? c3 : c4;
            const uint32_t off1 = l1 == 0 ? 0u : l1 == 1 ? c1 : l1 == 2 ? c2 : l1 == 3 ? c3 : c4;
            ts.lod0 = f;
            ts.lod1 = __uint_as_float(off0);
            ts.lod2 = __uint_as_float(off1);
            ts.mesh = (l0 | (l1 << 4)) << 24;
        }
    }
}

template <class MP>
__device__ __forceinline__ void tri_shade_setup(const float p[9], const Geo& g, const Raster& rs, MP mp,
                                                float4 b0, float2 b1, TriShade& ts) {
    {
#pragma clang fp contract(off)
        ts.inva = rcp_rn((float)rs.area2);
    }
    const long long Px0 = 256ll * rs.x0 + 128, Py0 = 256ll * rs.y0 + 128;
    ts.a1 = rs.a[1]; ts.b1 = rs.b[1]; ts.a2 = rs.a[2]; ts.b2 = rs.b[2];
    ts.e1 = (long long)rs.a[1] * Px0 + (long long)rs.b[1] * Py0 + rs.c[1];
    ts.e2 = (long long)rs.a[2] * Px0 + (long long)rs.b[2] * Py0 + rs.c[2];
    ts.org = ((uint32_t)rs.y0 << 12) | (uint32_t)rs.x0;
    tri_shade_rest(p, g, rs.a[1], rs.b[1], rs.a[2], rs.b[2], mp, b0, b1, ts);
}

template <class MP>
__device__ __forceinline__ void tri_shade_small(const float p[9], const Geo& g, const RasterHead& h, const RasterSmall& rs, MP mp, float4 b0, float2 b1,
                                                uint32_t m, TriShadeS& c) {
    {
#pragma clang fp contract(off)
        c.inva = rcp_rn((float)rs.area2);
    }
    c.a1 = (short)rs.a[1]; c.b1 = (short)rs.b[1]; c.a2 = (short)rs.a[2]; c.b2 = (short)rs.b[2];
    c.e1 = rs.e[1]; c.e2 = rs.e[2];
    c.org = ((uint32_t)h.y0 << 12) | (uint32_t)h.x0;
    tri_shade_rest(p, g, rs.a[1], rs.b[1], rs.a[2], rs.b[2], mp, b0, b1, c);
    c.mesh |= m;
}

struct TexTap {
    uint32_t o00, o10, o01, o11;
    float w00, w10, w01, w11;
};

__device__ __forceinline__ void tex_tap(uint32_t W, uint32_t H, uint32_t level_off, float uf, float vf, TexTap& t) {
    float up, vp;
    {
#pragma clang fp contract(off)
        up = uf * (float)W - 0.5f;
        vp = vf * (float)H - 0.5f;
    }
    const float fi = floorf(up), fj = floorf(vp);
    const float a = up - fi, b = vp - fj;
    int i0 = (int)fi, j0 = (int)fj;
    int i1 = i0 + 1, j1 = j0 + 1;
    i0 = i0 < 0 ? i0 + (int)W : i0;
    j0 = j0 < 0 ? j0 + (int)H : j0;
    i1 = i1 >= (int)W ? i1 - (int)W : i1;
    j1 = j1 >= (int)H ? j1 - (int)H : j1;
    const uint32_t r0 = level_off + __umul24((uint32_t)j0, W), r1 = level_off + __umul24((uint32_t)j1, W);
    t.o00 = r0 + (uint32_t)i0; t.o10 = r0 + (uint32_t)i1;
    t.o01 = r1 + (uint32_t)i0; t.o11 = r1 + (uint32_t)i1;
    const float na = 1.0f - a, nb = 1.0f - b;
    t.w00 = na * nb; t.w10 = a * nb; t.w01 = na * b; t.w11 = a * b;
}

struct TexState {
    TexTap lo, hi;
    float f;
};

template <class TD>
__device__ __forceinline__ void tex_state(TD t, float uf, float vf, float lambda, TexState& st) {
    const uint32_t nl = t->n_levels, w = t->w, h = t->h;
    const float q = (float)(nl - 1);
    float d = 0.0f, f = 0.0f;
    if (lambda > 0.0f) {
        if (lambda >= q) d = q;
        else { d = floorf(lambda); f = lambda - d; }
    }
    const uint32_t l0 = (uint32_t)d, l1 = min(l0 + 1u, nl - 1u);
    const uint32_t o1 = t->off[1], o2 = t->off[2], o3 = t->off[3], o4 = t->off[4];
    const uint32_t off0 = l0 == 0 ? 0u : l0 == 1 ? o1 : l0 == 2 ? o2 : l0 == 3 ? o3 : o4;
    const uint32_t off1 = l1 == 0 ? 0u : l1 == 1 ? o1 : l1 == 2 ? o2 : l1 == 3 ? o3 : o4;
    tex_tap(max(1u, w >> l0), max(1u, h >> l0), off0, uf, vf, st.lo);
    st.f = f;
    if (__ballot(f != 0.0f) != 0ull) tex_tap(max(1u, w >> l1), max(1u, h >> l1), off1, uf, vf, st.hi);
    else st.hi = st.lo;
}

struct TexFetch { uint32_t lo[4], hi[4]; };
__device__ __forceinline__ void tex_issue(const uint32_t* __restrict__ texels, const TexState& st, TexFetch& tf) {
    const GlobalBytes gb = as_global(texels);
    tf.lo[0] = ld_texel(gb, st.lo.o00); tf.lo[1] = ld_texel(gb, st.lo.o10); tf.lo[2] = ld_texel(gb, st.lo.o01); tf.lo[3] = ld_texel(gb, st.lo.o11);
    tf.hi[0] = ld_texel(gb, st.hi.o00); tf.hi[1] = ld_texel(gb, st.hi.o10); tf.hi[2] = ld_texel(gb, st.hi.o01); tf.hi[3] = ld_texel(gb, st.hi.o11);
}
template <int NCH>
__device__ __forceinline__ void tap_filter(const uint32_t t[4], const TexTap& tp, float out[NCH]) {
#pragma unroll
    for (int ch = 0; ch < NCH; ch++) {
        const float c00 = (float)((t[0] >> (8 * ch)) & 255u), c10 = (float)((t[1] >> (8 * ch)) & 255u);
        const float c01 = (float)((t[2] >> (8 * ch)) & 255u), c11 = (float)((t[3] >> (8 * ch)) & 255u);
        out[ch] = fma_(tp.w11, c11, fma_(tp.w01, c01, fma_(tp.w10, c10, tp.w00 * c00)));
    }
}
template <int NCH>
__device__ __forceinline__ void tex_finish(const TexFetch& tf, const TexState& st, float out[NCH]) {
    float lo[NCH], hi[NCH];
    tap_filter<NCH>(tf.lo, st.lo, lo);
    tap_filter<NCH>(tf.hi, st.hi, hi);
    const float f = st.f, nf = 1.0f - st.f;
#pragma unroll
    for (int ch = 0; ch < NCH; ch++) out[ch] = fma_(f, hi[ch], nf * lo[ch]) * kUnorm8;
}


struct ComboTap {
    uint32_t o0, o1;
    float w00, w10, w01, w11;
};

__device__ __forceinline__ void combo_tap(uint32_t level_off, uint32_t W, uint32_t H, float uf, float vf, ComboTap& t) {
    float up, vp;
    {
#pragma clang fp contract(off)
        up = uf * (float)W - 0.5f;
        vp = vf * (float)H - 0.5f;
    }
    const float fi = floorf(up), fj = floorf(vp);
    const float a = up - fi, b = vp - fj;
    int i0 = (int)fi, j0 = (int)fj;
    int j1 = j0 + 1;
    i0 = i0 < 0 ? i0 + (int)W : i0;
    j0 = j0 < 0 ? j0 + (int)H : j0;
    j1 = j1 >= (int)H ? j1 - (int)H : j1;
    const uint32_t stride = W + 1;
    t.o0 = level_off + (__umul24((uint32_t)j0, stride) + (uint32_t)i0) * 3u;
    t.o1 = level_off + (__umul24((uint32_t)j1, stride) + (uint32_t)i0) * 3u;
    const float na = 1.0f - a, nb = 1.0f - b;
    t.w00 = na * nb; t.w10 = a * nb; t.w01 = na * b; t.w11 = a * b;
}

__device__ __forceinline__ void combo_filter(const ComboPair& r0, const ComboPair& r1, const ComboTap& t, float out[9]) {
#define M2S_CH(word, sh) fma_(t.w11, (float)((r1.v[(word) + 3] >> (sh)) & 255u), fma_(t.w01, (float)((r1.v[word] >> (sh)) & 255u), \
                          fma_(t.w10, (float)((r0.v[(word) + 3] >> (sh)) & 255u), t.w00 * (float)((r0.v[word] >> (sh)) & 255u))))
    out[0] = M2S_CH(0, 0); out[1] = M2S_CH(0, 8); out[2] = M2S_CH(0, 16); out[3] = M2S_CH(0, 24);
    out[4] = M2S_CH(1, 0); out[5] = M2S_CH(1, 8); out[6] = M2S_CH(1, 16);
    out[7] = M2S_CH(2, 8); out[8] = M2S_CH(2, 16);
#undef M2S_CH
}

__device__ __forceinline__ float frac_repeat(float u) {
    float f = u - floorf(u);
    f = (f >= 0.0f) ? f : 0.0f;
    return fminf(f, 1.0f);
}

struct ComboFetch {
    ComboTap tlo, thi;
    ComboPair a0, a1, b0, b1;
    float f;
};
template <class MP, class TD, class TS>
__device__ __forceinline__ void combo_issue(MP mp, TD t, float uf, float vf, const TS& ts, ComboFetch& cf) {
    const uint32_t w = t->w, h = t->h;
    const float f = ts.lod0;
    const uint32_t off0 = __float_as_uint(ts.lod1), off1 = __float_as_uint(ts.lod2);
    const uint32_t l0 = (ts.mesh >> 24) & 15u, l1 = ts.mesh >> 28;
    const uint32_t* __restrict__ base = mp->combo.texels;
    ComboTap& tlo = cf.tlo;
    ComboTap& thi = cf.thi;
    cf.f = f;
    combo_tap(off0, max(1u, w >> l0), max(1u, h >> l0), uf, vf, tlo);
    combo_tap(off1, max(1u, w >> l1), max(1u, h >> l1), uf, vf, thi);
    const GlobalBytes gb = as_global(base);
    cf.a0 = ld_combo(gb, tlo.o0);
    cf.a1 = ld_combo(gb, tlo.o1);
    cf.b0 = ld_combo(gb, thi.o0);
    cf.b1 = ld_combo(gb, thi.o1);
#ifdef M2S_FUSED3_PRIO
    __builtin_amdgcn_s_setprio(0);
#endif
}
__device__ __forceinline__ void combo_finish(ComboFetch& cf, float out[9]) {
    ComboTap& tlo = cf.tlo;
    ComboTap& thi = cf.thi;
    const float f = cf.f;
    const float klo = (1.0f - f) * kUnorm8, khi = f * kUnorm8;
    tlo.w00 *= klo; tlo.w10 *= klo; tlo.w01 *= klo; tlo.w11 *= klo;
    thi.w00 *= khi; thi.w10 *= khi; thi.w01 *= khi; thi.w11 *= khi;
    float lo[9], hi[9];
    combo_filter(cf.a0, cf.a1, tlo, lo);
    combo_filter(cf.b0, cf.b1, thi, hi);
#pragma unroll
    for (int ch = 0; ch < 9; ch++) out[ch] = lo[ch] + hi[ch];
}
template <class MP, class TD, class TS>
__device__ __forceinline__ void combo_sample(MP mp, TD t, float uf, float vf, const TS& ts, float out[9]) {
    ComboFetch cf;
    combo_issue(mp, t, uf, vf, ts, cf);
    combo_finish(cf, out);
}


template <typename T>
__device__ __forceinline__ T ld_plane(const T* base, uint32_t t) {
    return *reinterpret_cast<const T*>(reinterpret_cast<const char*>(base) + (size_t)(t * (uint32_t)sizeof(T)));
}

template <bool kNT, typename T>
__device__ __forceinline__ T ld_attr(const T* base, uint32_t t) {
    if constexpr (!kNT) return ld_plane(base, t);
    else {
        const T* p = reinterpret_cast<const T*>(reinterpret_cast<const char*>(base) + (size_t)(t * (uint32_t)sizeof(T)));
        if constexpr (sizeof(T) == 16) {
            return make_float4(__builtin_nontemporal_load(&p->x), __builtin_nontemporal_load(&p->y),
                               __builtin_nontemporal_load(&p->z), __builtin_nontemporal_load(&p->w));
        } else return __builtin_nontemporal_load(p);
    }
}


template <class MP, class TS = TriShade, bool kComboOnly = false, bool kStreamAttr = false>
__device__ __forceinline__ void shade_from_tri(const TriPlanes& tp, uint32_t t, int x, int y, MP mp,
                                               const TS& ts, float4 rec[6], unsigned long long* stamps = nullptr,
                                               const float2* uvl = nullptr ,
                                               const float* posl = nullptr ) {
    const int dx256 = (x - (int)(ts.org & 0xFFFu)) * 256, dy256 = (y - (int)(ts.org >> 12)) * 256;
    float l1, l2;
    if constexpr (sizeof(ts.e1) == 4) {
        const int E1 = ts.e1 + (int)ts.a1 * dx256 + (int)ts.b1 * dy256;
        const int E2 = ts.e2 + (int)ts.a2 * dx256 + (int)ts.b2 * dy256;
        l1 = (float)E1 * ts.inva;
        l2 = (float)E2 * ts.inva;
    } else {
        const long long E1 = ts.e1 + (long long)ts.a1 * dx256 + (long long)ts.b1 * dy256;
        const long long E2 = ts.e2 + (long long)ts.a2 * dx256 + (long long)ts.b2 * dy256;
        l1 = i64_to_f32(E1) * ts.inva;
        l2 = i64_to_f32(E2) * ts.inva;
    }

    float4 b0 = make_float4(0, 0, 0, 0);
    float2 b1 = make_float2(0, 0);
    if (uvl == nullptr) {
        b0 = ld_plane(tp.B0, t);
        b1 = ld_plane(tp.B1, t);
    }
    float4 a0, a1;
    float a2;
    if (posl == nullptr) {
        a0 = ld_plane(tp.A0, t); a1 = ld_plane(tp.A1, t);
        a2 = ld_plane(tp.A2, t);
    }
    const float4 c0 = ld_attr<kStreamAttr>(tp.C0, t), c1 = ld_attr<kStreamAttr>(tp.C1, t);
    const float c2 = ld_attr<kStreamAttr>(tp.C2, t);
    const float4 d0 = ld_attr<kStreamAttr>(tp.D0, t), d1 = ld_attr<kStreamAttr>(tp.D1, t), d2 = ld_attr<kStreamAttr>(tp.D2, t);
    if (posl != nullptr) {
        a0 = make_float4(posl[0], posl[1], posl[2], posl[3]);
        a1 = make_float4(posl[4], posl[5], posl[6], posl[7]);
        a2 = posl[8];
    }
    float U, V;
    {
#pragma clang fp contract(off)
        if (uvl != nullptr) {
            const float2 q0 = uvl[0], q1 = uvl[1], q2 = uvl[2];
            U = (q0.x + l1 * q1.x) + l2 * q2.x;
            V = (q0.y + l1 * q1.y) + l2 * q2.y;
        } else {
            U = (b0.x + l1 * (b0.z - b0.x)) + l2 * (b1.x - b0.x);
            V = (b0.y + l1 * (b0.w - b0.y)) + l2 * (b1.y - b0.y);
        }
    }
#define M2S_LERP(f0, f1, f2) fma_(l2, (f2) - (f0), fma_(l1, (f1) - (f0), (f0)))

    const auto ta = &mp->tex[0];
    const auto tn = &mp->tex[1];
    const auto tm = &mp->tex[2];
    const uint32_t* xa = ta->texels;
    const uint32_t* xn = tn->texels;
    const uint32_t* xm = tm->texels;
    if (stamps) stamps[0] = __builtin_amdgcn_s_memtime();
    const float uf = frac_repeat(U), vf = frac_repeat(V);
    float col[4] = { 1.0f, 1.0f, 1.0f, 1.0f };
    float nrm[3] = { 0.0f, 0.0f, 1.0f };
    float metal = 0.1f, rough = 0.5f;
    const uint32_t* __restrict__ cmb = mp->combo.texels;
    if (cmb != nullptr) {
        float acc[9];
        combo_sample(mp, ta, uf, vf, ts, acc);
        col[0] = acc[0]; col[1] = acc[1]; col[2] = acc[2]; col[3] = acc[3];
        nrm[0] = acc[4]; nrm[1] = acc[5]; nrm[2] = acc[6];
        rough = acc[7]; metal = acc[8];
    } else if constexpr (!kComboOnly) {
        TexState sa, sn, sm;
        TexFetch fa, fn, fm;
        const bool n_like_a = xa != nullptr && xn != nullptr && tn->w == ta->w && tn->h == ta->h;
        const bool m_like_a = xa != nullptr && xm != nullptr && tm->w == ta->w && tm->h == ta->h;
        const bool m_like_n = xn != nullptr && xm != nullptr && tm->w == tn->w && tm->h == tn->h;
        if (xa != nullptr) tex_state(ta, uf, vf, ts.lod0, sa);
        if (xn != nullptr) { if (n_like_a) sn = sa; else tex_state(tn, uf, vf, ts.lod1, sn); }
        if (xm != nullptr) {
            if (xn != nullptr ? m_like_n : m_like_a) sm = (xn != nullptr) ? sn : sa;
            else tex_state(tm, uf, vf, ts.lod2, sm);
        }
        if (xa != nullptr) tex_issue(xa, sa, fa);
        if (xn != nullptr) tex_issue(xn, sn, fn);
        if (xm != nullptr) tex_issue(xm, sm, fm);
        if (xa != nullptr) tex_finish<4>(fa, sa, col);
        if (xn != nullptr) tex_finish<3>(fn, sn, nrm);
        if (xm != nullptr) {
            float sv[3];
            tex_finish<3>(fm, sm, sv);
            metal = sv[2]; rough = sv[1];
        }
    }
    if (stamps) stamps[1] = __builtin_amdgcn_s_memtime();
    const float Pxw = M2S_LERP(a0.x, a0.w, a1.z), Pyw = M2S_LERP(a0.y, a1.x, a1.w), Pzw = M2S_LERP(a0.z, a1.y, a2);
    const float Nx = M2S_LERP(c0.x, c0.w, c1.z), Ny = M2S_LERP(c0.y, c1.x, c1.w), Nz = M2S_LERP(c0.z, c1.y, c2);
    float ox = Nx, oy = Ny, oz = Nz;
    if (xn != nullptr) {
        const float Tx = M2S_LERP(d0.x, d1.x, d2.x), Ty = M2S_LERP(d0.y, d1.y, d2.y), Tz = M2S_LERP(d0.z, d1.z, d2.z);
        const float Tw = M2S_LERP(d0.w, d1.w, d2.w);
        float rx = fma_(nrm[0], 2.0f, -1.0f), ry = fma_(nrm[1], 2.0f, -1.0f), rz = fma_(nrm[2], 2.0f, -1.0f);
        float inv = fast_rsq(dot3_(rx, ry, rz, rx, ry, rz));
        rx *= inv; ry *= inv; rz *= inv;
        float bx = fma_(Ny, Tz, -(Nz * Ty)), by = fma_(Nz, Tx, -(Nx * Tz)), bz = fma_(Nx, Ty, -(Ny * Tx));
        inv = fast_rsq(dot3_(bx, by, bz, bx, by, bz)) * Tw;
        bx *= inv; by *= inv; bz *= inv;
        inv = fast_rsq(dot3_(Nx, Ny, Nz, Nx, Ny, Nz));
        const float nnx = Nx * inv, nny = Ny * inv, nnz = Nz * inv;
        const float wx = fma_(nnx, rz, fma_(bx, ry, Tx * rx)), wy = fma_(nny, rz, fma_(by, ry, Ty * rx)), wz = fma_(nnz, rz, fma_(bz, ry, Tz * rx));
        inv = fast_rsq(dot3_(wx, wy, wz, wx, wy, wz));
        ox = wx * inv; oy = wy * inv; oz = wz * inv;
    }
#undef M2S_LERP
    if (stamps) stamps[2] = __builtin_amdgcn_s_memtime();
    rec[0] = make_float4(Pxw, Pyw, Pzw, 1.0f);
    rec[1] = make_float4(col[0] * mp->color[0], col[1] * mp->color[1], col[2] * mp->color[2], col[3] * mp->color[3]);
    rec[2] = make_float4(ts.sx, ts.sy, 1e-7f, 0.0f);
    rec[3] = make_float4(ox, oy, oz, 0.0f);
    rec[4] = ts.rot;
    rec[5] = make_float4(metal, rough, 0.0f, 1.0f);
}

__device__ __forceinline__ void nt_store(float4* p, float4 v) {
    __builtin_nontemporal_store(v.x, &p->x); __builtin_nontemporal_store(v.y, &p->y);
    __builtin_nontemporal_store(v.z, &p->z); __builtin_nontemporal_store(v.w, &p->w);
}

}
```

### mesh2splat_amd/csrc/m2s_device.h

```cpp
#pragma once
#include <cstdlib>
#include <hip/hip_runtime.h>
#include <stdint.h>

namespace m2s {

#ifdef M2S_DEBUG_BUILD
inline const char* debug_env(const char* name) {
    static const bool enabled = std::getenv("M2S_DEBUG") != nullptr;
    return enabled ? std::getenv(name) : nullptr;
}
#else
inline const char* debug_env(const char*) { return nullptr; }
#endif
inline bool debug_on(const char* name) { const char* v = debug_env(name); return v && *v && *v != '0'; }

constexpr int kBlock = 256;
constexpr int kTriPerBlock = 1024;
constexpr int kEmitF = 1024;
constexpr int kRowsThread = 32;
constexpr int kRowsCount = 128;
constexpr int kStageStride = 7;

struct TriPlanes {
    const float4* A0;
    const float4* A1;
    const float*  A2;
    const float4* B0;
    const float2* B1;
    const float4* C0;
    const float4* C1;
    const float*  C2;
    const float4* D0;
    const float4* D1;
    const float4* D2;
};

struct TexDesc {
    const uint32_t* texels;
    uint32_t w, h, n_levels;
    uint32_t off[5];
};

struct ComboDesc {
    const uint32_t* texels;
    uint32_t coff[5];
};

struct MeshParams {
    float bmin[3];
    float bmax[3];
    float color[4];
    TexDesc tex[3];
    ComboDesc combo;
};

struct BigItem {
    uint32_t t, cnt;
    unsigned long long off;
};

struct SceneDev {
    TriPlanes tri;
    const MeshParams* meshes;
    const uint32_t* mesh_first;
    const uint2* mesh_of8;
    uint32_t n_meshes;
    uint32_t n_tri;
    uint32_t tri_first;
};

void launch_repack(const float* d_aos, uint32_t stride_floats, uint32_t n_tri_src, uint32_t src_first,
                   uint32_t n, uint32_t dst_first, TriPlanes dst , hipStream_t st);
void launch_mesh_table(const SceneDev& sc, uint2* table, hipStream_t st);
void launch_mip_level(const uint32_t* src, uint32_t sw, uint32_t sh, uint32_t* dst, uint32_t dw, uint32_t dh,
                      hipStream_t st);
void launch_combo_level(const uint32_t* a, const uint32_t* n, const uint32_t* m, uint32_t w, uint32_t h, uint32_t* dst,
                        hipStream_t st);
void launch_count(const SceneDev& sc, uint32_t R, uint32_t* cnt, uint32_t* partials, hipStream_t st);
void launch_scan_partials(uint32_t* partials, uint32_t n_partials, unsigned long long* total, hipStream_t st);
void launch_big_share(const uint32_t* cnt, uint32_t n_tri, uint32_t threshold, unsigned long long* out, hipStream_t st);
void launch_unit_bases(const uint32_t* cnt, const uint32_t* partials, uint32_t n_tri, uint32_t unit, uint32_t shift, unsigned long long* run_base, hipStream_t st);
void launch_run_order(const unsigned long long* run_base, uint32_t n_runs, const unsigned long long* total, uint32_t* order, uint32_t n_slots,
                      uint32_t first_set, hipStream_t st);
inline uint32_t resident_workgroups(const void* kernel, int threads) {
    int dev = 0, cus = 0, per_cu = 0;
    if (hipGetDevice(&dev) != hipSuccess || hipDeviceGetAttribute(&cus, hipDeviceAttributeMultiprocessorCount, dev) != hipSuccess ||
        hipOccupancyMaxActiveBlocksPerMultiprocessor(&per_cu, kernel, threads, 0) != hipSuccess || cus <= 0 || per_cu <= 0) {
        (void)hipGetLastError();
        return 0u;
    }
    return (uint32_t)per_cu * (uint32_t)cus;
}
uint32_t fused2_resident_workgroups();
uint32_t fused3_resident_workgroups();
uint32_t sparse_resident_workgroups();
inline uint32_t run_order_slots(uint32_t n_units, uint32_t shift) { return ((n_units + (8u << shift) - 1u) / (8u << shift)) * 8u; }
uint32_t emit2_slices(uint64_t limit);
uint32_t count_scan_blocks(uint32_t n_tri);
size_t setup_bytes(uint32_t n_tri);
size_t setup_tall_offset(uint32_t n_tri);
void launch_count_scan(const SceneDev& sc, uint32_t R, uint32_t* off, uint32_t* start, uint32_t n_start, unsigned long long* chain,
                       uint32_t epoch, unsigned long long* total, void* setup, uint32_t* status, unsigned long long* total_host, hipStream_t st);
void launch_emit2(const SceneDev& sc, uint32_t R, const uint32_t* off, const uint32_t* start, const unsigned long long* total,
                  uint64_t limit, const void* setup, float4* out, hipStream_t st);

void launch_encode_rows(const float4* rec, uint64_t n, uint32_t format, float scale_multiplier, uint8_t* out, hipStream_t st);

struct RunInfo {
    const unsigned long long* base;
    unsigned long long* out;
    uint32_t shift;
    const uint32_t* order;
};
inline uint32_t run_shift_for(uint32_t n_units) {
    if (const char* v = debug_env("M2S_RUN_SHIFT")) { const uint32_t s = (uint32_t)std::atoi(v) & 15u; return n_units >= (32u << s) ? s : 0u; }
    for (uint32_t shift = 5; shift >= 3; --shift)
        if (n_units >= (32u << shift)) return shift;
    return 0u;
}
inline uint32_t n_runs(uint32_t n_units, uint32_t shift) { return (n_units + (1u << shift) - 1u) >> shift; }
struct BatchTable {
    const uint32_t* first;
    uint32_t n;
    uint32_t tpw;
};
uint32_t fused2_band_workgroups(uint32_t n_tri);
void launch_fused2(const SceneDev& sc, uint32_t R, unsigned long long* chain, uint64_t limit, float4* out,
                   unsigned long long* total, uint32_t* status, uint32_t epoch, BigItem* biglist, uint32_t* bigmeta,
                   const RunInfo& runs, const BatchTable& batches, hipStream_t st);
void launch_fused3(const SceneDev& sc, uint32_t R, unsigned long long* chain, uint64_t limit, float4* out,
                   unsigned long long* total, uint32_t* status, uint32_t epoch, BigItem* biglist, uint32_t* bigmeta,
                   const RunInfo& runs, const BatchTable& batches, hipStream_t st);
void launch_sparse(const SceneDev& sc, uint32_t R, unsigned long long* chain, uint64_t limit, float4* out,
                   unsigned long long* total, uint32_t* status, uint32_t epoch, BigItem* biglist, uint32_t* bigmeta,
                   const RunInfo& runs, hipStream_t st, float4* plane = nullptr);
bool sparse_supported(uint32_t n_tri);
uint32_t sparse_workgroups(uint32_t n_tri);
constexpr uint32_t kSparseTrianglesPerWorkgroup = 512;
void launch_emit_big(const SceneDev& sc, uint32_t R, const BigItem* biglist, uint32_t n_big, uint32_t max_cnt, uint64_t limit,
                     float4* out, hipStream_t st);

struct PrepassK {
    float M[16], V[16], P[16];
    float MinvT[16];
    float mr_inv[9];
    float ms2[3];
    float res[2], near_far[2], std_dev;
    int32_t render_mode;
    uint32_t format, ply_has_pbr, depth_test, arrival_order;
    const float* depth;
    uint32_t depth_w, depth_h;
    uint32_t global_w;
};
}
struct m2s_prepass_params;
namespace m2s {
void prepass_prepare(const m2s_prepass_params& p, uint64_t n, PrepassK* out);
hipError_t launch_prepass(const PrepassK& k, const float4* rec, uint32_t n, float4* quads, float* depths, unsigned long long* chain,
                          uint32_t epoch, unsigned long long* counter, unsigned long long* total, uint32_t* status, hipStream_t st,
                          const uint32_t* perm = nullptr, bool dense = false, uint32_t* sources = nullptr);

size_t sort_prepass_temp_bytes(uint32_t n);
hipError_t sort_prepass(const float* depths, const float4* quads, uint32_t n, uint32_t* keys_out, uint32_t* vals_out, void* temp,
                        size_t temp_bytes, float4* sorted, hipStream_t st);
size_t sort_temp_bytes(uint32_t n);
hipError_t sort_by_depth(const float4* rec, uint32_t n, const float view[16], uint32_t* keys_in, uint32_t* keys_out, uint32_t* vals_out,
                         void* temp, size_t temp_bytes, float4* sorted, float4* plane, bool plane_valid, hipEvent_t* stage_ev, hipStream_t st,
                         uint32_t* key_offset_out, uint32_t* pinned_mm );
void launch_add_to_keys(uint32_t* keys, uint32_t n, uint32_t offset, hipStream_t st);
hipError_t sort_prepass_permutation(const float4* rec, uint32_t n, const float model[16], const float view[16], const float proj[16], bool cull,
                                    uint32_t* keys_in, uint32_t* keys_out, uint32_t* vals_out, void* temp, size_t temp_bytes, float4* plane, bool plane_valid,
                                    hipEvent_t* ev, hipStream_t st, uint32_t* pinned_mm4, uint32_t* n_visible, bool* clash);

constexpr int kSplatTile = 16;
constexpr size_t kSplatRecBytes = 128;
size_t splat_scan_temp_bytes(uint32_t n);
size_t splat_sort_temp_bytes(uint32_t pairs, uint32_t n_tiles);
hipError_t splat_setup(const float4* quads, uint32_t n, int W, int H, float4* rec, uint32_t* cnt, unsigned long long* off, void* temp,
                       size_t temp_bytes, unsigned long long* totals, hipStream_t st);
hipError_t splat_pairs(const float4* rec, const uint32_t* cnt, const unsigned long long* off, uint32_t n, int tiles_x, uint32_t* keys,
                       uint32_t* vals, hipStream_t st);
hipError_t splat_group(uint32_t* keys_in, uint32_t* vals_in, uint32_t* keys_out, uint32_t* vals_out, uint32_t pairs, uint32_t n_tiles,
                       uint2* ranges, uint32_t* len, uint32_t* len_sorted, uint32_t* order, void* temp, size_t temp_bytes, hipStream_t st);
hipError_t splat_blend(const float4* rec, const uint32_t* vals, const uint2* ranges, const uint32_t* order, int W, int H, int render_mode,
                       void* const planes[5], unsigned long long* frag_count, hipStream_t st);
hipError_t preload_splat();

hipError_t contrib_blend(const float4* rec, const uint32_t* vals, const uint2* ranges, const uint32_t* order, int W, int H,
                         const uint32_t* sources, float count_weight, uint32_t* wmax, uint32_t* npix, hipStream_t st);
size_t prune_scan_temp_bytes(uint32_t n);
hipError_t prune_flags_scan(const uint32_t* wmax, const uint32_t* npix, uint32_t n, float min_weight, uint32_t min_pixels, uint32_t* flags,
                            uint32_t* offsets, unsigned long long* counters, void* temp, size_t temp_bytes, hipStream_t st);
hipError_t prune_compact(const float4* src, const uint32_t* flags, const uint32_t* offsets, uint32_t n, uint32_t f4_per_row, float4* dst,
                         hipStream_t st);

struct ShadowBases { uint32_t b[7]; };
struct RelightK {
    float light[3], cam[3], color[3];
    float intensity, far_plane;
    int32_t mode, W, H, S;
};
inline uint32_t shadow_blocks(uint32_t n) { return (n + 255u) / 256u; }
size_t shadow_temp_bytes(uint32_t n_words, uint32_t n_quads, uint32_t pairs);
hipError_t shadow_count(const PrepassK& k, const float* views, const float light[3], const float4* rec, uint32_t n, uint32_t* cnt, uint32_t* off,
                        void* temp, size_t temp_bytes, uint32_t* bases, hipStream_t st);
hipError_t shadow_emit(const PrepassK& k, const float* views, const float light[3], const float4* rec, uint32_t n, const uint32_t* off, float4* quads,
                       hipStream_t st);
hipError_t shadow_setup(const float4* quads, uint32_t n, const ShadowBases& fb, int S, const float light[3], float far_plane, float4* rec, uint32_t* cnt,
                        unsigned long long* off, void* temp, size_t temp_bytes, unsigned long long* totals, hipStream_t st);
hipError_t shadow_bin(const float4* rec, const uint32_t* cnt, const unsigned long long* off, uint32_t n, int S, uint32_t* keys_in, uint32_t* vals_in,
                      uint32_t* keys_out, uint32_t* vals_out, uint32_t pairs, void* temp, size_t temp_bytes, hipStream_t st);
hipError_t shadow_clear(float* cube, int S, hipStream_t st);
hipError_t shadow_raster(const float4* rec, const uint32_t* keys, const uint32_t* vals, uint32_t pairs, int S, float* cube, unsigned long long* writes,
                         hipStream_t st);
hipError_t launch_relight(const RelightK& k, const void* const planes[5], const float* cube, uint32_t* frame, uint8_t* counts, hipStream_t st,
                          const void* const left_planes[5] = nullptr, int split_x = 0, int div_x = 0);
hipError_t preload_light();

struct BakeK {
    float M[16], MinvT[16];
    float light[3], color[3];
    float intensity, far_plane;
    int32_t S;
    uint32_t n_dirs;
    uint32_t n_coef;
    uint32_t use_shadows, viewer_metallic;
};
struct ShadeK { float M[16]; float cam[3]; };
constexpr int kBakeTableRow = 20;
hipError_t launch_bake_sh(const BakeK& k, const float4* rec, uint32_t n, const float* table, const float* cube, float* plane, uint8_t* counts,
                          hipStream_t st);
hipError_t launch_sh_shade(const ShadeK& k, const float4* rec, const float* sh, uint32_t n, float4* dst, hipStream_t st);

struct MeshDepthK {
    float PVM[16];
    int32_t W, H;
    int32_t inplace;
};
constexpr int kMdInplace = 4;
constexpr int kMdSlotsPerTriangle = 6;
size_t meshdepth_temp_bytes(uint32_t n_slots, uint32_t pairs);
hipError_t meshdepth_clear(float* image, int W, int H, hipStream_t st);
hipError_t meshdepth_setup(const MeshDepthK& k, const SceneDev& sc, float* image, uint32_t* deferred, unsigned long long* totals, hipStream_t st);
hipError_t meshdepth_deferred(const MeshDepthK& k, const SceneDev& sc, const uint32_t* deferred, uint32_t nd, float4* rec, uint32_t* cnt,
                              unsigned long long* off, void* temp, size_t temp_bytes, unsigned long long* totals, hipStream_t st, bool vis = false);
hipError_t meshdepth_bin(const MeshDepthK& k, const float4* rec, const uint32_t* cnt, const unsigned long long* off, uint32_t nd, uint32_t* keys_in,
                         uint32_t* vals_in, uint32_t* keys_out, uint32_t* vals_out, uint32_t pairs, void* temp, size_t temp_bytes, hipStream_t st);
hipError_t meshdepth_raster(const MeshDepthK& k, const float4* rec, const uint32_t* keys, const uint32_t* vals, uint32_t pairs, float* image,
                            unsigned long long* totals, hipStream_t st);
hipError_t preload_meshdepth();

hipError_t meshvis_clear(unsigned long long* image, int W, int H, hipStream_t st);
hipError_t meshvis_setup(const MeshDepthK& k, const SceneDev& sc, unsigned long long* image, uint32_t* deferred, unsigned long long* totals, hipStream_t st);
hipError_t meshvis_raster(const MeshDepthK& k, const float4* rec, const uint32_t* keys, const uint32_t* vals, uint32_t pairs, unsigned long long* image,
                          unsigned long long* totals, hipStream_t st);
struct MeshRenderK {
    float PVM[16];
    float M[16], V[16];
    float N[9];
    float near_far[2];
    int32_t W, H, mode;
};
hipError_t meshrender_shade(const MeshRenderK& k, const SceneDev& sc, const unsigned long long* vis, void* const planes[5], hipStream_t st);
hipError_t preload_meshrender();

struct ScoreK {
    int32_t W, H;
    uint32_t mask_mode;
    uint32_t tiles_x;
};
constexpr int kScoreTileCells = 16;
constexpr int kScoreGridCells = 17;
constexpr int kScoreThreads = 320;
constexpr int kScoreCounters = 16;
constexpr int kScoreMaxFirst = 11, kScoreMaxLast = 13;
constexpr int kScoreShards = 32;
inline uint32_t score_tiles(int n) { return (uint32_t)((n + 4 * kScoreTileCells - 1) / (4 * kScoreTileCells)); }
hipError_t launch_score(const ScoreK& k, const uint32_t* a, const uint32_t* b, const uint32_t* cover_a, const uint32_t* cover_b, uint32_t* map,
                        unsigned long long* acc, hipStream_t st);
hipError_t preload_score();

inline uint32_t compact_waves(uint32_t n) { return (n + kBlock - 1) / kBlock * (kBlock / 64); }
size_t compact_sort_temp_bytes(uint32_t n);
hipError_t compact_keys_and_sort(const float4* rec, const float4* plane, uint32_t n, uint32_t* wave_box, uint32_t* head, uint32_t* keys_in, uint32_t* vals_in,
                                 uint32_t* keys_out, uint32_t* vals_out, void* temp, size_t temp_bytes, hipEvent_t* ev, hipStream_t st);
// ... 29 lines not shown
```

### mesh2splat_amd/csrc/m2s_fused3.hip

```cpp
#include "m2s_fused_common.h"

#pragma clang fp contract(off)

namespace m2s {

#ifndef M2S_FUSED3_WAVES
#define M2S_FUSED3_WAVES 4
#endif
#ifndef M2S_FUSED3_ENTRIES
#define M2S_FUSED3_ENTRIES 1024
#endif
#ifndef M2S_FUSED3_STAGE
#define M2S_FUSED3_STAGE (M2S_FUSED3_WAVES >= 5 ? 16 : 32)
#endif
constexpr int kL3Team = 4;
constexpr int kL3Threads = kL3Team * 64;
constexpr uint32_t kL3Entries = (uint32_t)M2S_FUSED3_ENTRIES * kL3Team;
constexpr int kL3Stage = M2S_FUSED3_STAGE;
constexpr uint32_t kL3Wait = 1u << 24;
constexpr uint32_t kL3Stop = 1u << 28;

struct F3Ctl {
    unsigned long long base;
    unsigned long long total_w[kL3Team];
    uint32_t total_c[kL3Team];
    uint32_t counted[kL3Team];
    uint32_t expanded[kL3Team];
    uint32_t t0[kL3Team];
    uint32_t claimed;
    uint32_t base_state;
    uint32_t flags;
    uint32_t pad_;
};
struct F3Lds {
    float4 tri[kL3Team][64 * 4];
    uint32_t tskip[kL3Team][64];
    float2 uv[kL3Team][64 * 3];
    uint16_t cum[kL3Team][64];
    uint8_t lane_of[kL3Team][64];
    uint8_t entries[kL3Entries];
    float4 stage[kL3Team][kL3Stage * 6];
    F3Ctl ctl;
};
static_assert(sizeof(F3Lds) * M2S_FUSED3_WAVES <= 163840, "M2S_FUSED3_WAVES workgroups per CU must fit the 160 KB of LDS");
static_assert((uint32_t)M2S_FUSED3_ENTRIES * kL3Team < 0xFFFFu && 64u * 64u < 0xFFFFu, "cum is 16 bits wide, 0xFFFF marks an unused slot");
#ifdef M2S_FUSED3_NT_ATTR
constexpr bool kF3StreamAttr = true;
#else
constexpr bool kF3StreamAttr = false;
#endif
constexpr uint32_t kF3Irregular = 1u << 8;
#ifndef M2S_FUSED3_TRI_PRIO
#define M2S_FUSED3_TRI_PRIO 1
#endif
#ifndef M2S_FUSED3_PRIO_FLOOR
#define M2S_FUSED3_PRIO_FLOOR 0
#endif
constexpr uint32_t kF3ClassShift = 5;
__device__ __forceinline__ uint32_t f3_class(uint32_t round) { return (round >> kF3ClassShift) & 3u; }

__device__ __forceinline__ uint32_t l3_load(const uint32_t* p) { return __hip_atomic_load(p, __ATOMIC_ACQUIRE, __HIP_MEMORY_SCOPE_WORKGROUP); }
__device__ __forceinline__ void l3_store(uint32_t* p, uint32_t v) { __hip_atomic_store(p, v, __ATOMIC_RELEASE, __HIP_MEMORY_SCOPE_WORKGROUP); }
__device__ __forceinline__ uint32_t l3_uniform(const uint32_t* p) {
    return __builtin_amdgcn_readfirstlane(__hip_atomic_load(p, __ATOMIC_RELAXED, __HIP_MEMORY_SCOPE_WORKGROUP));
}
__device__ __forceinline__ void l3_fail(F3Ctl& C, uint32_t why, int lane) {
    if (lane == 0) {
        __hip_atomic_fetch_or(&C.flags, why, __ATOMIC_RELEASE, __HIP_MEMORY_SCOPE_WORKGROUP);
        __hip_atomic_fetch_add(&C.claimed, kL3Stop, __ATOMIC_RELAXED, __HIP_MEMORY_SCOPE_WORKGROUP);
    }
}

__device__ __forceinline__ bool f3_get_base(F3Ctl& C, unsigned long long* chain, uint32_t b0, int lane, uint32_t epoch, uint32_t* status,
                                            unsigned long long& base) {
    uint32_t st = l3_load(&C.base_state);
    if (st != 2) {
        uint32_t got = 1;
        if (lane == 0) {
            uint32_t expect = 0;
            got = __hip_atomic_compare_exchange_strong(&C.base_state, &expect, 1u, __ATOMIC_ACQ_REL, __ATOMIC_ACQUIRE, __HIP_MEMORY_SCOPE_WORKGROUP) ? 0u : 1u;
        }
        got = __builtin_amdgcn_readfirstlane(got);
        if (got == 0) {
            const unsigned long long b = b0 == 0 ? 0ull : lookback(chain, b0, lane, epoch, status);
            if (lane == 0) {
                C.base = b;
                chain_store(&chain[b0], kFlagPrefix | ((unsigned long long)epoch << kEpochShift) | ((b + C.total_w[0]) & kValMask));
            }
            l3_store(&C.base_state, 2u);
        } else {
            uint32_t spins = 0;
            while (l3_load(&C.base_state) != 2) {
                if (++spins > kL3Wait) { l3_fail(C, 1u, lane); return false; }
                __builtin_amdgcn_s_sleep(2);
            }
        }
    }
    base = C.base;
    return true;
}

#ifdef M2S_TIMELINE
__device__ unsigned long long g_tl_f3[16384 * 4 * 8];
constexpr int kTlHwId = 4 | (31 << 11);
constexpr int kTlXccId = 20 | (3 << 11);
#define TLF(k) do { __builtin_amdgcn_sched_barrier(0); if (lane == 0 && blockIdx.x < 16384u) g_tl_f3[((size_t)blockIdx.x * 4 + wave) * 8 + (k)] = wall_clock64(); __builtin_amdgcn_sched_barrier(0); } while (0)
#define TLFV(k, v) do { if (lane == 0 && blockIdx.x < 16384u) g_tl_f3[((size_t)blockIdx.x * 4 + wave) * 8 + (k)] = (v); } while (0)
#else
#define TLF(k) do { } while (0)
#define TLFV(k, v) do { } while (0)
#endif

__global__ void __launch_bounds__(kL3Threads, M2S_FUSED3_WAVES) k_fused3(SceneDev sc, uint32_t R, unsigned long long* __restrict__ chain,
                                                      unsigned long long limit, float4* __restrict__ out,
                                                      unsigned long long* __restrict__ total_out,
                                                      uint32_t* __restrict__ status , uint32_t epoch,
                                                      BigItem* __restrict__ biglist, uint32_t* __restrict__ bigmeta,
                                                      uint32_t tpw ,
                                                      RunInfo runs, BatchTable bt) {
    __shared__ F3Lds S;
    F3Ctl& C = S.ctl;
    const int lane = threadIdx.x & 63;
    const uint32_t wave = __builtin_amdgcn_readfirstlane(threadIdx.x >> 6);
    const uint32_t n_batches = bt.first ? bt.n : (sc.n_tri + tpw - 1u) / tpw;
    const uint32_t hb = blockIdx.x, xcd = hb & 7u, round = hb >> 3;
    const bool in_runs = runs.base != nullptr;
    const uint32_t rmask = (1u << runs.shift) - 1u;
    const unsigned long long etag = (unsigned long long)epoch << kEpochShift;
    uint32_t lb = hb;
    if (in_runs) {
        uint32_t rr = ((round >> runs.shift) << 3) + xcd;
        if (runs.order) rr = ((const __attribute__((address_space(4))) uint32_t*)runs.order)[rr];
        lb = (rr << runs.shift) + (round & rmask);
    }
    const bool band_first = in_runs && (round & rmask) == 0u;
    if (lb * (uint32_t)kL3Team >= n_batches) return;
#if M2S_FUSED3_TRI_PRIO == 1
    __builtin_amdgcn_s_setprio(1);
#elif M2S_FUSED3_TRI_PRIO == 2
    switch (f3_class(round)) {
        case 0: __builtin_amdgcn_s_setprio(3); break;
        case 1: __builtin_amdgcn_s_setprio(2); break;
        case 2: __builtin_amdgcn_s_setprio(M2S_FUSED3_PRIO_FLOOR > 1 ? M2S_FUSED3_PRIO_FLOOR : 1); break;
        default: __builtin_amdgcn_s_setprio(M2S_FUSED3_PRIO_FLOOR); break;
    }
#endif
    TLF(0);
    if (lane == 0) { C.counted[wave] = 0; C.expanded[wave] = 0; }
    if (wave == 0 && lane == 0) {
        C.claimed = 0; C.flags = 0;
        C.base_state = (lb == 0 || band_first) ? 2u : 0u;
        C.base = band_first ? runs.base[lb >> runs.shift] : 0ull;
    }
    __syncthreads();
    const uint32_t b0 = lb * kL3Team;
    const uint32_t nb_here = min((uint32_t)kL3Team, n_batches - b0);
    const uint32_t b = b0 + wave;
    const bool has_batch = wave < nb_here;
    const unsigned long long band_base = band_first ? C.base : 0ull;

    uint32_t t0 = b * tpw, nt = tpw;
    if (bt.first && has_batch) {
        const __attribute__((address_space(4))) uint32_t* q = (const __attribute__((address_space(4))) uint32_t*)bt.first;
        t0 = q[b];
        nt = q[b + 1] - t0;
    }
    const uint32_t t = t0 + lane;
    const bool valid = has_batch && (uint32_t)lane < nt && t < sc.n_tri;
    if (lane == 0) C.t0[wave] = t0;
    int kind = kNone;
    unsigned long long mask = 0;
    uint32_t cnt = 0;
    {
        float p[9];
        Geo g;
        RasterHead h;
        h.x0 = h.y0 = 0; h.x1 = h.y1 = -1; h.ext = 0;
        bool box = false;
        uint32_t m = 0;
        float4 uvb0 = make_float4(0, 0, 0, 0);
        float2 uvb1 = make_float2(0, 0);
        bool uniform_mesh = false;
        uint32_t m0 = 0;
        if (has_batch) {
            const uint32_t lastT = min(t0 + nt, sc.n_tri) - 1;
            m0 = mesh_of_range(sc, t0, lastT, uniform_mesh);
            m = m0;
            if (valid) {
                load_positions(sc.tri, t, p);
                uvb0 = sc.tri.B0[t];
                uvb1 = sc.tri.B1[t];
                if (uniform_mesh) geo_setup_mp(p, kConstMesh(sc.meshes + m0), g);
                else { m = find_mesh(sc, sc.tri_first + t); geo_setup_mp(p, sc.meshes + m, g); }
                box = raster_head(g, R, h);
            }
        }
        const int w = h.x1 - h.x0 + 1, rows = h.y1 - h.y0 + 1;
        RasterSmall rs;
        bool small = box && w <= 8 && rows <= 8 && h.ext <= 2304;
        if (small) small = raster_small(h, rs);
        else if (box) kind = kBig;
        {
            uint32_t mlo = 0, mhi = 0;
            small_coverage(small, w, rows, rs, mlo, mhi);
            mask = (unsigned long long)mlo | ((unsigned long long)mhi << 32);
            cnt = (uint32_t)__popc(mlo) + (uint32_t)__popc(mhi);
            if (small) kind = kSmall;
        }
        if (cnt != 0 && kind == kSmall) {
            TriShadeS c;
            if (uniform_mesh) tri_shade_small(p, g, h, rs, kConstMesh(sc.meshes + m0), uvb0, uvb1, m, c);
            else tri_shade_small(p, g, h, rs, sc.meshes + m, uvb0, uvb1, m, c);
            const float4* src = reinterpret_cast<const float4*>(&c);
#pragma unroll
            for (int k = 0; k < 4; ++k) S.tri[wave][lane * 4 + k] = src[k];
            float2* const uvs = &S.uv[wave][lane * 3];
            uvs[0] = make_float2(uvb0.x, uvb0.y);
            uvs[1] = make_float2(uvb0.z - uvb0.x, uvb0.w - uvb0.y);
            uvs[2] = make_float2(uvb1.x - uvb0.x, uvb1.y - uvb0.y);
        }
        if (__ballot(kind == kBig) != 0ull) {
            Raster rb;
            rb.x0 = rb.y0 = 0; rb.x1 = rb.y1 = -1; rb.ext = 0; rb.bias = 0; rb.area2 = 1;
#pragma unroll
            for (int i = 0; i < 3; i++) { rb.a[i] = rb.b[i] = 0; rb.c[i] = 0; }
            if (kind == kBig && !raster_setup(g, R, rb)) kind = kNone;
            unsigned long long bigm = __ballot(kind == kBig);
            while (bigm) {
                const int src = __ffsll((long long)bigm) - 1;
                bigm &= bigm - 1;
                const Raster br = shfl_raster(rb, src);
                uint32_t part = 0;
                for (int y = br.y0 + lane; y <= br.y1; y += 64) {
                    int xa, xb;
                    row_span(br, y, xa, xb);
                    part += (uint32_t)max(xb - xa + 1, 0);
                }
                part = wave_sum(part);
                if (lane == src) cnt = part;
            }
        }
    }
    if (cnt == 0) kind = kNone;
    const uint32_t cntc = kind == kSmall ? cnt : 0;
    const bool anybig = __ballot(kind == kBig) != 0ull;

    const uint32_t incl = wave_incl_scan(cnt, lane);
    const uint32_t inclc = wave_incl_scan(cntc, lane);
    const unsigned long long total_w = __builtin_amdgcn_readlane(incl, 63);
    const uint32_t total_c = __builtin_amdgcn_readlane(inclc, 63);
    const uint32_t toff = incl - cnt;
    const uint32_t ctoff = inclc - cntc;

    if (has_batch && lane == 0) {
        const bool knows = b == 0 || (band_first && wave == 0);
        chain_store(&chain[b], (knows ? kFlagPrefix : kFlagAgg) | etag | (((knows ? band_base : 0ull) + total_w) & kValMask));
    }
    if (lane == 0) {
        C.total_w[wave] = total_w; C.total_c[wave] = total_c;
        if (anybig) __hip_atomic_fetch_or(&C.flags, kF3Irregular, __ATOMIC_RELAXED, __HIP_MEMORY_SCOPE_WORKGROUP);
    }
#if M2S_FUSED3_TRI_PRIO
    __builtin_amdgcn_s_setprio(0);
#endif
    l3_store(&C.counted[wave], 1u);
    TLF(1);

    uint32_t stream0 = 0;
    unsigned long long out0 = 0;
    bool alive = true;
    for (uint32_t k = 0; k < wave && alive; ++k) {
        uint32_t spins = 0;
        while (l3_load(&C.counted[k]) == 0) {
            if (++spins > kL3Wait) { alive = false; break; }
            __builtin_amdgcn_s_sleep(1);
        }
        stream0 += C.total_c[k];
        out0 += C.total_w[k];
    }
    if (!alive) l3_fail(C, 1u, lane);
    if (alive && (unsigned long long)stream0 + total_c > kL3Entries) {
        alive = false;
        l3_fail(C, 2u, lane);
    }
    unsigned long long base = 0;
    bool have_base = false;
    if (alive && wave == (uint32_t)kL3Team - 1 && (l3_load(&C.flags) & 0xFFu) == 0) {
        have_base = f3_get_base(C, chain, b0, lane, epoch, status, base);
        if (!have_base) alive = false;
    }

    if (alive) {
        if (cntc) S.tskip[wave][lane] = (uint32_t)((out0 + toff) - ((unsigned long long)stream0 + ctoff));
        {
            const unsigned long long cov = __ballot(cntc != 0);
            const uint32_t ncov = (uint32_t)__popcll(cov);
            if ((uint32_t)lane >= ncov) S.cum[wave][lane] = 0xFFFFu;
            if (cntc) {
                const uint32_t slot = __builtin_amdgcn_mbcnt_hi((uint32_t)(cov >> 32), __builtin_amdgcn_mbcnt_lo((uint32_t)cov, 0u));
                S.cum[wave][slot] = (uint16_t)inclc;
                S.lane_of[wave][slot] = (uint8_t)lane;
            }
        }
        if (anybig) {
            unsigned long long bb;
            if (f3_get_base(C, chain, b0, lane, epoch, status, bb)) {
                if (kind == kBig) {
                    const uint32_t slot = atomicAdd(&bigmeta[0], 1u);
                    atomicMax(&bigmeta[1], cnt);
                    atomicAdd(&bigmeta[2], cnt);
                    BigItem it2;
                    it2.t = t; it2.cnt = cnt; it2.off = bb + out0 + toff;
                    biglist[slot] = it2;
                }
                if (lane == 0) __hip_atomic_store(&status[0], 1u, __ATOMIC_RELAXED, __HIP_MEMORY_SCOPE_SYSTEM);
            } else alive = false;
        }
        if (kind == kSmall) {
            unsigned long long mm = mask;
            uint32_t ci = stream0 + ctoff;
            uint32_t first = 64u;
            while (mm) {
                const int bit = __ffsll((long long)mm) - 1;
                mm &= mm - 1;
                S.entries[ci++] = (uint8_t)(first | (uint32_t)bit);
                first = 0u;
            }
        }
    }
    l3_store(&C.expanded[wave], 1u);
    TLF(2);
    [[maybe_unused]] unsigned long long tl_strips = 0;

    for (uint32_t k = 0; k < (uint32_t)kL3Team && alive; ++k) {
        uint32_t spins = 0;
        while (l3_load(&C.counted[k]) == 0) {
            if (++spins > kL3Wait) { alive = false; l3_fail(C, 1u, lane); break; }
            __builtin_amdgcn_s_sleep(1);
        }
    }
    float4* const stage = S.stage[wave];
    uint32_t exp_seen = 0;
    TLF(3);
    while (alive) {
        uint32_t s = 0;
        if (lane == 0) s = __hip_atomic_fetch_add(&C.claimed, 1u, __ATOMIC_RELAXED, __HIP_MEMORY_SCOPE_WORKGROUP);
        s = __builtin_amdgcn_readfirstlane(s);
        const uint32_t c1 = l3_uniform(&C.total_c[0]), c2 = c1 + l3_uniform(&C.total_c[1]), c3 = c2 + l3_uniform(&C.total_c[2]),
                       stream_total = c3 + l3_uniform(&C.total_c[3]);
        const uint32_t pos0 = s * 64u;
        if (s >= kL3Stop / 64u || pos0 >= stream_total) break;
#ifdef M2S_TIMELINE
        ++tl_strips;
#endif
        const uint32_t n = min(64u, stream_total - pos0);
        const uint32_t lo[4] = { 0u, c1, c2, c3 }, hi[4] = { c1, c2, c3, stream_total };
        if (exp_seen != 15u) {
#pragma unroll
            for (int k = 0; k < kL3Team; ++k) {
                if ((exp_seen >> k) & 1u) continue;
                if (hi[k] <= pos0 || lo[k] >= pos0 + n) continue;
                uint32_t spins = 0;
                while (l3_load(&C.expanded[k]) == 0) {
                    if (++spins > kL3Wait) { alive = false; l3_fail(C, 1u, lane); break; }
                    __builtin_amdgcn_s_sleep(1);
                }
                exp_seen |= 1u << k;
            }
            if (!alive) break;
        }
#ifdef M2S_FUSED3_PRIO
        __builtin_amdgcn_s_setprio(M2S_FUSED3_PRIO);
#endif
        const uint32_t pos = pos0 + (uint32_t)lane;
        const bool have = (uint32_t)lane < n;
        uint32_t en = 0;
        if (have) en = S.entries[pos];
        const uint32_t ow = (pos >= c1 ? 1u : 0u) + (pos >= c2 ? 1u : 0u) + (pos >= c3 ? 1u : 0u);
        const uint32_t bit = en & 63u;
        uint32_t slot = 0;
        {
            const unsigned long long fm = __ballot(have && (en & 64u) != 0u);
#pragma unroll
            for (int k = 0; k < kL3Team; ++k) {
                if (hi[k] <= pos0 || lo[k] >= pos0 + n || hi[k] == lo[k]) continue;
                const uint32_t p0 = max(pos0, lo[k]);
                const uint32_t q0 = p0 - lo[k], sl = p0 - pos0;
                const uint32_t s0 = (uint32_t)__popcll(__ballot((uint32_t)S.cum[k][lane] <= q0));
                const unsigned long long fk = fm & ~((2ull << sl) - 1ull);
                const uint32_t below = __builtin_amdgcn_mbcnt_hi((uint32_t)(fk >> 32), __builtin_amdgcn_mbcnt_lo((uint32_t)fk, 0u));
                if (ow == (uint32_t)k) slot = s0 + below + (uint32_t)((fk >> lane) & 1ull);
            }
        }
        uint32_t tl = 0;
        if (have) tl = S.lane_of[ow][slot & 63u] & 63u;
        float4 rec[6];
        uint32_t my_mesh = 0;
        if (have) my_mesh = reinterpret_cast<const uint32_t*>(&S.tri[ow][tl * 4 + 3])[3] & 0xFFFFFFu;
        unsigned long long todo = __ballot(have);
        while (todo) {
            const uint32_t m_now = __builtin_amdgcn_readlane(my_mesh, __ffsll((long long)todo) - 1);
            const bool mine = have && my_mesh == m_now;
            if (mine) {
                const TriShadeS& ts = *reinterpret_cast<const TriShadeS*>(&S.tri[ow][tl * 4]);
                const uint32_t tt = C.t0[ow] + tl;
                const uint32_t org = ts.org;
                const int x = (int)(org & 0xFFFu) + (int)(bit & 7u), y = (int)(org >> 12) + (int)(bit >> 3);
#ifdef M2S_FUSED3_UV_GLOBAL
                const float2* const uvl = nullptr;
#else
                const float2* const uvl = &S.uv[ow][tl * 3];
#endif
#ifdef M2S_FUSED3_ABL_POS
                const float* const posl = reinterpret_cast<const float*>(&S.tri[ow][tl * 4]);
#else
                const float* const posl = nullptr;
#endif
                shade_from_tri<ConstMeshPtr, TriShadeS, true, kF3StreamAttr>(sc.tri, tt, x, y, kConstMesh(sc.meshes + __builtin_amdgcn_readfirstlane(my_mesh)),
                                                                              ts, rec, nullptr, uvl, posl);
            }
            todo &= ~__ballot(mine);
        }
        if (!have_base) {
            if (!f3_get_base(C, chain, b0, lane, epoch, status, base)) break;
            have_base = true;
        }
        const uint32_t fl = l3_load(&C.flags);
        if (fl & 0xFFu) break;
        const unsigned long long base_now = (unsigned long long)l3_uniform(reinterpret_cast<const uint32_t*>(&C.base)) |
                                            ((unsigned long long)l3_uniform(reinterpret_cast<const uint32_t*>(&C.base) + 1) << 32);
        if ((fl & kF3Irregular) == 0) {
            const unsigned long long o0 = base_now + pos0;
            uint32_t nvalid = n;
            if (o0 + 64ull > limit) {
                if (o0 >= limit) nvalid = 0;
                else if (limit - o0 < nvalid) nvalid = (uint32_t)(limit - o0);
            }
#pragma unroll 1
            for (int part = 0; part < 64 / kL3Stage; ++part) {
                if (have && (lane / kL3Stage) == part) {
#pragma unroll
                    for (int k = 0; k < 6; ++k) stage[(lane % kL3Stage) * 6 + k] = rec[k];
                }
                wave_lds_sync();
                float4* __restrict__ dsto = out + (o0 + (uint32_t)kL3Stage * part) * 6;
                const uint32_t nv = nvalid > (uint32_t)kL3Stage * part ? min((uint32_t)kL3Stage, nvalid - (uint32_t)kL3Stage * part) : 0u;
#pragma unroll
                for (int j = 0; j < (kL3Stage * 6 + 63) / 64; ++j) {
                    const uint32_t q = (uint32_t)lane + 64u * j;
                    const uint32_t r = q / 6u;
                    if (r < nv) nt_store(&dsto[q], stage[q]);
                }
                wave_lds_sync();
            }
        } else if (have) {
            const unsigned long long oidx = base_now + S.tskip[ow][tl] + pos;
            if (oidx < limit) {
                float4* __restrict__ dsto = out + oidx * 6;
#pragma unroll
                for (int k = 0; k < 6; ++k) nt_store(&dsto[k], rec[k]);
            }
        }
    }
    TLF(4);
    TLFV(6, tl_strips | ((unsigned long long)(__builtin_amdgcn_s_getreg(kTlXccId) | (f3_class(round) << 8)) << 32));
    const uint32_t err = l3_load(&C.flags) & 0xFFu;
    if (alive && wave == nb_here - 1 && err == 0) {
        if (!have_base) have_base = f3_get_base(C, chain, b0, lane, epoch, status, base);
        if (have_base && lane == 0) {
            const unsigned long long out_total = (C.total_w[0] + C.total_w[1]) + (C.total_w[2] + C.total_w[3]);
            chain_store(&chain[b0 + nb_here - 1], kFlagPrefix | etag | ((base + out_total) & kValMask));
            if (b0 + nb_here == n_batches) *total_out = base + out_total;
            if (runs.out && (lb & rmask) == 0u) runs.out[lb >> runs.shift] = base;
        }
    }
    if (err && lane == 0) __hip_atomic_store(&status[1], err, __ATOMIC_RELAXED, __HIP_MEMORY_SCOPE_SYSTEM);
    TLF(5);
    TLFV(7, (unsigned long long)lb | ((unsigned long long)__builtin_amdgcn_s_getreg(kTlHwId) << 32));
}

void launch_fused3(const SceneDev& sc, uint32_t R, unsigned long long* chain, uint64_t limit, float4* out,
                   unsigned long long* total, uint32_t* status, uint32_t epoch, BigItem* biglist, uint32_t* bigmeta,
                   const RunInfo& runs, const BatchTable& bt, hipStream_t st) {
    const uint32_t tpw = fused_tpw(sc.n_tri);
    const uint32_t n_batches = bt.first ? bt.n : n_fused_waves(sc.n_tri);
    if (!n_batches) return;
    uint32_t nb = (n_batches + kL3Team - 1) / kL3Team;
    RunInfo r = runs;
    if (tpw != 64u || bt.first) r = RunInfo{ nullptr, nullptr, 0u, nullptr };
    if (r.base) r.out = nullptr;
    if (r.base) nb = ((nb + (8u << r.shift) - 1u) / (8u << r.shift)) * (8u << r.shift);
    else nb = (nb + 7u) & ~7u;
    hipLaunchKernelGGL(k_fused3, dim3(nb), dim3(kL3Threads), 0, st, sc, R, chain, (unsigned long long)limit, out, total, status,
                       epoch & 0xFFFFu, biglist, bigmeta, tpw, r, bt);
}

#ifdef M2S_TIMELINE
}
extern "C" int m2s_debug_timeline_f3(void* dst, size_t bytes) {
    return hipMemcpyFromSymbol(dst, HIP_SYMBOL(m2s::g_tl_f3), std::min(bytes, sizeof(m2s::g_tl_f3))) == hipSuccess ? 0 : 1;
}
extern "C" int m2s_debug_timeline_f3_clear() {
    void* p = nullptr;
    if (hipGetSymbolAddress(&p, HIP_SYMBOL(m2s::g_tl_f3)) != hipSuccess) return 1;
    return hipMemset(p, 0, sizeof(m2s::g_tl_f3)) == hipSuccess ? 0 : 2;
}
namespace m2s {
#endif
uint32_t fused3_resident_workgroups() { return resident_workgroups(reinterpret_cast<const void*>(&k_fused3), kL3Threads); }
hipError_t preload_fused3() { hipFuncAttributes a; return hipFuncGetAttributes(&a, reinterpret_cast<const void*>(&k_fused3)); }

}
```

### mesh2splat_amd/csrc/m2s_pass.cpp

```cpp
#include "m2s_ctx.h"
#include "m2s_ply.h"

#include <algorithm>
#include <array>
#include <chrono>
#include <cstdio>
#include <cstring>
#include <string>
#include <thread>
#include <tuple>
#include <vector>

using namespace m2s;
using namespace m2s_host;

namespace {
static double sparse_frags_per_triangle(uint32_t n_tri) { return n_tri >= 2000000u ? 1.75 : 0.5; }
static uint32_t band_workgroups(const m2s_ctx* c, uint32_t unit) {
    const uint32_t team = fused2_band_workgroups(c->scene.n_tri);
    return !team ? 0u : unit == 256u ? team : sparse_workgroups(c->scene.n_tri);
}
static uint32_t first_resident_slots([[maybe_unused]] int form, [[maybe_unused]] uint32_t shift) {
#ifdef M2S_RUN_ORDER_SPREAD
    const uint32_t wgs = form == M2S_PIPELINE_SPARSE ? sparse_resident_workgroups() : form == M2S_PIPELINE_LEAN ? fused3_resident_workgroups()
                                                                                                                 : fused2_resident_workgroups();
    return wgs >> shift;
#else
    return 0u;
#endif
}
}

namespace m2s_host {
RunInfo bands_for(const m2s_ctx* c, const m2s_ctx::RInfo& ri, uint32_t unit, bool may_write, bool* writes) {
    RunInfo r{ nullptr, nullptr, 0u, nullptr };
    if (writes) *writes = false;
    const uint32_t n_wg = band_workgroups(c, unit);
    const uint32_t shift = run_shift_for(n_wg);
    if (!n_wg || !shift || !c->d_bands || !c->run_table_words || (unit == 256u && (c->n_batch_tab || ri.tpw)) || debug_on("M2S_NO_BANDS")) return r;
    if ((size_t)n_runs(n_wg, shift) > c->run_table_words) return r;
    unsigned long long* table = c->d_bands + (size_t)ri.band_slot * c->run_table_words;
    r.shift = shift;
    if (ri.bands_ready && ri.bands_unit == unit) {
        r.base = table;
        if (c->run_order_unit == unit && c->run_order_shift == shift && !debug_on("M2S_NO_RUN_ORDER")) r.order = c->d_run_order;
    }
    else if (may_write) { r.out = table; if (writes) *writes = true; }
    return r;
}

BatchTable batches_for(const m2s_ctx* c, const m2s_ctx::RInfo& ri) {
    return c->n_batch_tab ? BatchTable{ c->d_batch_first, c->n_batch_tab, 0u } : BatchTable{ nullptr, 0u, ri.tpw };
}

uint32_t unit_of(int form) { return form == M2S_PIPELINE_SPARSE ? kSparseTrianglesPerWorkgroup : 256u; }

void launch_single(const m2s_ctx* c, const m2s_ctx::RInfo& ri, uint32_t R, unsigned long long* chain, uint64_t limit, float4* d_out,
                   unsigned long long* res, uint32_t epoch, const RunInfo& runs, hipStream_t st, float4* plane) {
    uint32_t* status = reinterpret_cast<uint32_t*>(&res[1]);
    if (ri.form == M2S_PIPELINE_SPARSE)
        launch_sparse(c->scene, R, chain, limit, d_out, &res[0], status, epoch, c->d_biglist, c->d_bigmeta, runs, st, plane);
    else if (ri.form == M2S_PIPELINE_LEAN)
        launch_fused3(c->scene, R, chain, limit, d_out, &res[0], status, epoch, c->d_biglist, c->d_bigmeta, runs, batches_for(c, ri), st);
    else
        launch_fused2(c->scene, R, chain, limit, d_out, &res[0], status, epoch, c->d_biglist, c->d_bigmeta, runs, batches_for(c, ri), st);
}

uint64_t resolve_cap(const m2s_ctx* c, uint32_t R) {
    if (c->cap_policy == 0) return 0;
    if (c->cap_policy > 0) return (uint64_t)c->cap_policy;
    const uint32_t mc = std::max<uint32_t>(1u, c->n_meshes_total);
    const uint32_t mx = R * R * 6u * mc;
    return std::min(mx, kMaxGaussiansToSort);
}
}

static bool lean_eligible(const m2s_ctx* c, uint32_t R) {
    if (!c->lean_ok || R >= c->lean_off_R || debug_on("M2S_NO_LEAN")) return false;
    return c->pipeline == M2S_PIPELINE_LEAN || (c->pipeline == M2S_PIPELINE_AUTO && fused_tpw(c->scene.n_tri) == 64u);
}

static void decide(const m2s_ctx* c, m2s_ctx::RInfo& ri, double frags, uint32_t R) {
    const double n_tri = (double)c->scene.n_tri;
    ri.tpw = 0;
    ri.form = M2S_PIPELINE_MULTIPASS;
    if (c->pipeline == M2S_PIPELINE_MULTIPASS || R >= c->team_off_R) return;
    if (c->pipeline == M2S_PIPELINE_AUTO && frags >= 11.0 * n_tri) {
        if (frags < 13.0 * n_tri && R == c->warm_R && c->warm_total > 0 && c->warm_big * 8ull < c->warm_total &&
            fused_tpw(c->scene.n_tri) == 64u && !c->n_batch_tab && !debug_on("M2S_NO_BAND_TPW")) {
            ri.form = M2S_PIPELINE_TEAM;
            ri.tpw = 40;
        }
        return;
    }
    const bool sparse = c->pipeline == M2S_PIPELINE_SPARSE ||
                        (c->pipeline == M2S_PIPELINE_AUTO && frags < sparse_frags_per_triangle(c->scene.n_tri) * n_tri && !debug_on("M2S_NO_SPARSE"));
    if (sparse && R < c->sparse_off_R && sparse_supported(c->scene.n_tri)) ri.form = M2S_PIPELINE_SPARSE;
    else ri.form = lean_eligible(c, R) ? M2S_PIPELINE_LEAN : M2S_PIPELINE_TEAM;
}

enum class Trouble { full, stalled, lean_defers, big_share };

static void demote(m2s_ctx* c, m2s_ctx::RInfo& ri, uint32_t R, Trouble why) {
    const bool every_larger_R = why == Trouble::full || why == Trouble::lean_defers;
    if (why == Trouble::big_share) {
        ri.form = M2S_PIPELINE_MULTIPASS;
    } else if (ri.form == M2S_PIPELINE_SPARSE) {
        if (every_larger_R) c->sparse_off_R = std::min(c->sparse_off_R, R);
        ri.form = lean_eligible(c, R) ? M2S_PIPELINE_LEAN : M2S_PIPELINE_TEAM;
    } else if (ri.form == M2S_PIPELINE_LEAN) {
        if (every_larger_R) c->lean_off_R = std::min(c->lean_off_R, R);
        ri.form = M2S_PIPELINE_TEAM;
    } else {
        if (ri.tpw) ri.tpw = 0;
        else if (every_larger_R) c->team_off_R = std::min(c->team_off_R, R);
        ri.form = M2S_PIPELINE_MULTIPASS;
    }
}

static m2s_status ensure_multipass_buffers(m2s_ctx* c, uint64_t limit);

namespace m2s_host {
m2s_status warm_count_enqueue(m2s_ctx* c, uint32_t R) {
    const SceneDev& sc = c->scene;
    if (!sc.n_tri || R == 0 || R > 4096) return M2S_ERR_INVALID;
    hipStream_t st = c->stream;
    launch_count(sc, R, c->d_cnt, c->d_partials, st);
    launch_scan_partials(c->d_partials, n_count_blocks(sc.n_tri), c->d_total, st);
    HIPCHK(c, hipGetLastError());
    HIPCHK(c, hipMemcpyAsync(c->h_total, c->d_total, 8, hipMemcpyDeviceToHost, st));
    c->warm_spec_unit = 0;
    if (!debug_on("M2S_NO_WARM_BANDS")) {
        m2s_ctx::RInfo& ri = rinfo_for(c, R);
        const uint32_t unit = unit_of(M2S_PIPELINE_TEAM);
        bool writes = false;
        const RunInfo table = bands_for(c, ri, unit, true, &writes);
        if (writes) {
            const uint32_t n_units = band_workgroups(c, unit);
            launch_unit_bases(c->d_cnt, c->d_partials, sc.n_tri, unit, table.shift, table.out, st);
            const int form = lean_eligible(c, R) ? M2S_PIPELINE_LEAN : M2S_PIPELINE_TEAM;
            launch_run_order(table.out, n_runs(n_units, table.shift), c->d_total, c->d_run_order, run_order_slots(n_units, table.shift),
                             first_resident_slots(form, table.shift), st);
            HIPCHK(c, hipGetLastError());
            c->warm_spec_unit = unit; c->warm_spec_shift = table.shift; c->warm_spec_form = form;
        }
    }
    return M2S_OK;
}

m2s_status warm_scene(m2s_ctx* c, uint32_t R, bool counted) {
    const SceneDev& sc = c->scene;
    if (!sc.n_tri || R == 0 || R > 4096) return M2S_OK;
    hipStream_t st = c->stream;
    if (!counted) {
        const m2s_status s = warm_count_enqueue(c, R);
        if (s != M2S_OK) return s;
        HIPCHK(c, hipStreamSynchronize(st));
    }
    const uint64_t total = c->h_total[0];
    c->frag_per_R2 = (double)total / ((double)R * (double)R);
    c->warm_R = R;
    c->warm_total = total;
    c->warm_big = 0;
    if (total >= 11ull * sc.n_tri && total < 13ull * sc.n_tri) {
        HIPCHK(c, hipMemsetAsync(c->d_total, 0, 8, st));
        launch_big_share(c->d_cnt, sc.n_tri, 96u, c->d_total, st);
        HIPCHK(c, hipGetLastError());
        HIPCHK(c, hipMemcpyAsync(&c->h_total[1], c->d_total, 8, hipMemcpyDeviceToHost, st));
        HIPCHK(c, hipStreamSynchronize(st));
        c->warm_big = c->h_total[1];
        c->h_total[1] = 0;
        const unsigned long long tot = total;
        HIPCHK(c, hipMemcpy(c->d_total, &tot, sizeof tot, hipMemcpyHostToDevice));
    }
    if (batch_table_capacity(sc.n_tri) && !c->n_batch_tab && !debug_on("M2S_NO_BATCH_TABLE")) {
        try {
            std::vector<uint32_t> cnt(sc.n_tri), first;
            HIPCHK(c, hipMemcpy(cnt.data(), c->d_cnt, (size_t)sc.n_tri * sizeof(uint32_t), hipMemcpyDeviceToHost));
            uint32_t n_target = n_fused_waves(sc.n_tri);
            if (const char* v = debug_env("M2S_BATCH_TARGET")) { const unsigned long q = strtoul(v, nullptr, 10); if (q >= 1 && q <= 8192) n_target = (uint32_t)q; }
            double ct = 214.0;
            const double cf = 140.0;
            if (const char* v = debug_env("M2S_BATCH_CT")) ct = atof(v);
            double total = 0.0;
            for (uint32_t t = 0; t < sc.n_tri; ++t) total += ct + cf * (double)cnt[t];
            const double quota = total / (double)n_target;
            first.reserve(batch_table_capacity(sc.n_tri));
            first.push_back(0);
            double acc = 0.0;
            uint32_t in_batch = 0;
            for (uint32_t g = 0; g < sc.n_tri; g += 8) {
                const uint32_t ge = std::min(g + 8u, sc.n_tri);
                double gc = 0.0;
                for (uint32_t t = g; t < ge; ++t) gc += ct + cf * (double)cnt[t];
                if (in_batch && (in_batch + (ge - g) > 64u || acc + 0.5 * gc >= quota * (double)first.size())) { first.push_back(g); in_batch = 0; }
                acc += gc;
                in_batch += ge - g;
            }
            first.push_back(sc.n_tri);
            if (first.size() <= batch_table_capacity(sc.n_tri)) {
                HIPCHK(c, hipMemcpy(c->d_batch_first, first.data(), first.size() * sizeof(uint32_t), hipMemcpyHostToDevice));
                c->n_batch_tab = (uint32_t)first.size() - 1u;
            }
        } catch (...) {  }
    }
    m2s_ctx::RInfo& ri = rinfo_for(c, R);
    if (ri.form == M2S_PIPELINE_AUTO) decide(c, ri, (double)total, R);
    const uint64_t cap = resolve_cap(c, R);
    const bool single = ri.form != M2S_PIPELINE_MULTIPASS;
    if (!debug_on("M2S_NO_PRELOAD")) {
        if (!single) { (void)preload_multipass(); if (!debug_on("M2S_NO_SCRATCH_WARM")) launch_scratch_warm(st); }
        else if (ri.form == M2S_PIPELINE_SPARSE) { (void)preload_sparse(); (void)preload_fused2(); }
        else if (ri.form == M2S_PIPELINE_LEAN) { (void)preload_fused3(); }
        else { (void)preload_fused2(); }
        (void)hipGetLastError();
    }
// ... 296 lines not shown
```

### mesh2splat_amd/csrc/m2s_upload.cpp

```cpp
#include "m2s_ctx.h"
#include "m2s_ply.h"

#include <algorithm>
#include <array>
#include <chrono>
#include <cstdio>
#include <cstring>
#include <string>
#include <thread>
#include <tuple>
#include <vector>

using namespace m2s;
using namespace m2s_host;

namespace {
constexpr size_t kStageChunk = 16ull << 20;

void par_memcpy(void* dst, const void* src, size_t n) {
    const size_t kMin = 2ull << 20;
    unsigned nt = (unsigned)std::min<size_t>(4, n / kMin);
    if (const char* e = std::getenv("M2S_HOST_THREADS")) { if (std::atol(e) == 1) nt = 1; }
    if (nt <= 1) { memcpy(dst, src, n); return; }
    std::vector<std::thread> pool;
// ... 78 lines not shown

    const auto t_alloc = std::chrono::steady_clock::now();
    const size_t np = std::max<size_t>(n_tri, 1);
    size_t offs[11], cur = 0;
    const size_t widths[11] = { 16, 16, 4, 16, 8, 16, 16, 4, 16, 16, 16 };
    for (int k = 0; k < 11; ++k) { offs[k] = cur; cur = align_up(cur + np * widths[k], 256); }
    HIPCHK(c, hipMalloc(&c->tri_mem, cur));

    struct TexPlan { const uint8_t* src; TexDesc d; size_t arena_off; };
    struct ComboPlan { ComboDesc d; size_t arena_off; uint32_t ia, in, im; };
    std::vector<TexPlan> tex_plan;
    std::vector<ComboPlan> combo_plan;
    std::map<std::tuple<const uint8_t*, uint32_t, uint32_t>, uint32_t> dedup;
    std::map<std::tuple<uint32_t, uint32_t, uint32_t>, uint32_t> cdedup;
    std::vector<std::array<int, 3>> mesh_tex(std::max<uint32_t>(n_meshes, 1), std::array<int, 3>{ -1, -1, -1 });
    std::vector<int> mesh_combo(std::max<uint32_t>(n_meshes, 1), -1);
    size_t arena = 0;
    auto take = [&](size_t bytes) { const size_t o = arena; arena = align_up(arena + std::max<size_t>(bytes, 4), 256); return o; };
    for (uint32_t i = 0; i < n_meshes; ++i) {
        const m2s_mesh& m = meshes[i];
        for (int k = 0; k < 3; ++k) {
            const m2s_texture& t = m.tex[k];
            if (!t.rgba8) continue;
            const auto key = std::make_tuple(t.rgba8, t.width, t.height);
            auto it = dedup.find(key);
            if (it != dedup.end()) { mesh_tex[i][k] = (int)it->second; continue; }
            TexPlan p{};
            p.src = t.rgba8;
            p.d.w = t.width; p.d.h = t.height;
            uint32_t mx = std::max(t.width, t.height), nl = 1;
            while (mx > 1 && nl < 5) { mx >>= 1; nl++; }
            p.d.n_levels = nl;
            size_t tot = 0;
            for (uint32_t l = 0; l < nl; ++l) {
                p.d.off[l] = (uint32_t)tot;
                tot += (size_t)std::max(1u, t.width >> l) * std::max(1u, t.height >> l);
            }
            p.arena_off = take(tot * 4);
            dedup[key] = (uint32_t)tex_plan.size();
            mesh_tex[i][k] = (int)tex_plan.size();
            tex_plan.push_back(p);
        }
        const int ia = mesh_tex[i][0], in = mesh_tex[i][1], im = mesh_tex[i][2];
        if (ia < 0 || in < 0 || im < 0) continue;
        const TexDesc &ta = tex_plan[ia].d, &tn = tex_plan[in].d, &tm = tex_plan[im].d;
        if (ta.w != tn.w || ta.w != tm.w || ta.h != tn.h || ta.h != tm.h) continue;
        const auto ckey = std::make_tuple((uint32_t)ia, (uint32_t)in, (uint32_t)im);
        auto cit = cdedup.find(ckey);
        if (cit != cdedup.end()) { mesh_combo[i] = (int)cit->second; continue; }
        ComboPlan cp{};
        size_t tot = 0;
        for (uint32_t l = 0; l < ta.n_levels; ++l) {
            cp.d.coff[l] = (uint32_t)tot;
            tot += (size_t)(std::max(1u, ta.w >> l) + 1) * std::max(1u, ta.h >> l) * 3;
        }
        if (tot > 0x3FFFFFF0ull) continue;
        cp.arena_off = take(tot * 4);
        cp.ia = (uint32_t)ia; cp.in = (uint32_t)in; cp.im = (uint32_t)im;
        cdedup[ckey] = (uint32_t)combo_plan.size();
        mesh_combo[i] = (int)combo_plan.size();
        combo_plan.push_back(cp);
    }
    const size_t n_mp = std::max<uint32_t>(n_meshes, 1);
    const size_t chain_words = std::max<size_t>(std::max<size_t>(std::max<size_t>(n_fused_waves(n_tri), batch_table_capacity(n_tri)), (size_t)n_tri / 32 + 1), 1);
    const size_t o_meshes = take(n_mp * sizeof(MeshParams));
    const size_t o_mesh_first = take(mesh_first.size() * sizeof(uint32_t));
    const size_t o_mesh_of8 = take(((np + 7) / 8 + 1) * sizeof(uint2));
    const size_t o_cnt = take(np * sizeof(uint32_t));
    const size_t o_off = take((np + 1) * sizeof(uint32_t));
    const size_t o_partials = take(std::max<size_t>(n_count_blocks(n_tri), 1) * sizeof(uint32_t));
    const size_t o_chain = take(chain_words * sizeof(unsigned long long));
    const size_t o_biglist = take(np * sizeof(BigItem));
    const size_t o_bigmeta = take(4 * sizeof(uint32_t));
    const uint32_t units = fused2_band_workgroups(n_tri);
    const size_t run_words = run_shift_for(units) ? (size_t)n_runs(units, run_shift_for(units)) + 1 : 0;
    const size_t o_bands = take(std::max<size_t>((size_t)kBandSlots * run_words, 1) * sizeof(unsigned long long));
    const size_t o_run_order = take(std::max<size_t>(run_shift_for(units) ? run_order_slots(units, run_shift_for(units)) : 0, 1) * sizeof(uint32_t));
    const size_t o_batch = take(std::max<size_t>(batch_table_capacity(n_tri), 1) * sizeof(uint32_t));
    HIPCHK(c, hipMalloc(&c->scene_arena, arena));
    { const m2s_status s = ensure_stage(c); if (s != M2S_OK) return s; }
    c->last_upload_ms[3] = ms_since(t_alloc);
    char* A = (char*)c->scene_arena;
    char* b = (char*)c->tri_mem;
    TriPlanes& tp = c->scene.tri;
    tp.A0 = (const float4*)(b + offs[0]); tp.A1 = (const float4*)(b + offs[1]); tp.A2 = (const float*)(b + offs[2]);
    tp.B0 = (const float4*)(b + offs[3]); tp.B1 = (const float2*)(b + offs[4]);
    tp.C0 = (const float4*)(b + offs[5]); tp.C1 = (const float4*)(b + offs[6]); tp.C2 = (const float*)(b + offs[7]);
    tp.D0 = (const float4*)(b + offs[8]); tp.D1 = (const float4*)(b + offs[9]); tp.D2 = (const float4*)(b + offs[10]);

    const auto t_geo = std::chrono::steady_clock::now();
    uint32_t turn = 0;
    for (uint32_t i = 0; i < n_meshes && n_tri; ++i) {
        const uint64_t s = std::max<uint64_t>(first, mesh_first[i]), e = std::min<uint64_t>(last, mesh_first[i + 1]);
        if (e <= s) continue;
        const uint32_t stride = meshes[i].stride_floats;
        const size_t tri_bytes = (size_t)3 * stride * sizeof(float);
        const size_t per_chunk = std::max<size_t>(1, kStageChunk / tri_bytes) * tri_bytes;
        const char* src = (const char*)(meshes[i].vertices + (size_t)(s - mesh_first[i]) * 3 * stride);
        const uint32_t dst0 = (uint32_t)(s - first);
        const m2s_status st = staged_h2d(c, src, (size_t)(e - s) * tri_bytes, per_chunk, nullptr, turn,
            [&](char* d, size_t off, size_t n) {
                launch_repack((const float*)d, stride, (uint32_t)(n / tri_bytes), 0, (uint32_t)(n / tri_bytes),
                              dst0 + (uint32_t)(off / tri_bytes), tp, c->stream);
            });
        if (st != M2S_OK) return st;
    }
    c->last_upload_ms[1] = ms_since(t_geo);

    const auto t_tex = std::chrono::steady_clock::now();
    for (TexPlan& p : tex_plan) p.d.texels = (uint32_t*)(A + p.arena_off);
    for (ComboPlan& cp : combo_plan) cp.d.texels = (uint32_t*)(A + cp.arena_off);
    std::vector<MeshParams> mp(n_mp);
    memset(mp.data(), 0, mp.size() * sizeof(MeshParams));
    for (uint32_t i = 0; i < n_meshes; ++i) {
        const m2s_mesh& m = meshes[i];
        MeshParams& p = mp[i];
        memcpy(p.bmin, m.bbox_min, 12);
        memcpy(p.bmax, m.bbox_max, 12);
        memcpy(p.color, m.base_color, 16);
        for (int k = 0; k < 3; ++k) if (mesh_tex[i][k] >= 0) p.tex[k] = tex_plan[mesh_tex[i][k]].d;
        if (mesh_combo[i] >= 0) p.combo = combo_plan[mesh_combo[i]].d;
    }
    c->lean_ok = true;
    for (uint32_t i = 0; i < n_meshes; ++i)
        if (mesh_combo[i] < 0 && (mesh_tex[i][0] >= 0 || mesh_tex[i][1] >= 0 || mesh_tex[i][2] >= 0)) c->lean_ok = false;
    c->d_meshes = (MeshParams*)(A + o_meshes);
    c->d_mesh_first = (uint32_t*)(A + o_mesh_first);
    HIPCHK(c, hipMemcpyAsync(c->d_meshes, mp.data(), mp.size() * sizeof(MeshParams), hipMemcpyHostToDevice, c->stream));
    HIPCHK(c, hipMemcpyAsync(c->d_mesh_first, mesh_first.data(), mesh_first.size() * sizeof(uint32_t), hipMemcpyHostToDevice, c->stream));
    c->scene.meshes = c->d_meshes;
    c->scene.mesh_first = c->d_mesh_first;
    c->scene.mesh_of8 = (const uint2*)(A + o_mesh_of8);
    launch_mesh_table(c->scene, (uint2*)(A + o_mesh_of8), c->stream);

    c->d_cnt = (uint32_t*)(A + o_cnt);
    c->d_off = (uint32_t*)(A + o_off);
    c->d_partials = (uint32_t*)(A + o_partials);
    c->d_chain = (unsigned long long*)(A + o_chain);
    c->d_biglist = (BigItem*)(A + o_biglist);
    c->d_bigmeta = (uint32_t*)(A + o_bigmeta);
    c->d_bands = (unsigned long long*)(A + o_bands);
    c->run_table_words = run_words;
    c->d_run_order = (uint32_t*)(A + o_run_order);
    c->run_order_unit = 0; c->run_order_shift = 0;
    c->d_batch_first = (uint32_t*)(A + o_batch);
    c->n_batch_tab = 0;
    c->chain_words = chain_words;
    HIPCHK(c, hipMemsetAsync(c->d_chain, 0, chain_words * sizeof(unsigned long long), c->stream));
    HIPCHK(c, hipMemsetAsync(c->d_bigmeta, 0, 4 * sizeof(uint32_t), c->stream));
    const uint32_t warm_R = c->hint_R ? c->hint_R : c->last_R ? c->last_R : 1024u;
    const bool warm = !debug_on("M2S_NO_WARM");
    bool counted = false;
    if (warm && !debug_on("M2S_NO_WARM_OVERLAP")) counted = warm_count_enqueue(c, warm_R) == M2S_OK;

    for (TexPlan& p : tex_plan) {
        uint32_t* mem = (uint32_t*)(A + p.arena_off);
        const m2s_status st = staged_h2d(c, (const char*)p.src, (size_t)p.d.w * p.d.h * 4, kStageChunk, (char*)mem, turn,
                                         [](char*, size_t, size_t) {});
        if (st != M2S_OK) return st;
        for (uint32_t l = 1; l < p.d.n_levels; ++l)
            launch_mip_level(mem + p.d.off[l - 1], std::max(1u, p.d.w >> (l - 1)), std::max(1u, p.d.h >> (l - 1)),
                             mem + p.d.off[l], std::max(1u, p.d.w >> l), std::max(1u, p.d.h >> l), c->stream);
    }
    for (ComboPlan& cp : combo_plan) {
        uint32_t* mem = (uint32_t*)(A + cp.arena_off);
        const TexDesc &ta = tex_plan[cp.ia].d, &tn = tex_plan[cp.in].d, &tm = tex_plan[cp.im].d;
        for (uint32_t l = 0; l < ta.n_levels; ++l)
            launch_combo_level(ta.texels + ta.off[l], tn.texels + tn.off[l], tm.texels + tm.off[l], std::max(1u, ta.w >> l),
                               std::max(1u, ta.h >> l), mem + cp.d.coff[l], c->stream);
    }
    HIPCHK(c, hipStreamSynchronize(c->stream));
    HIPCHK(c, hipGetLastError());
    c->last_upload_ms[2] = ms_since(t_tex);
    c->has_scene = true;
    const auto t_warm = std::chrono::steady_clock::now();
    if (warm) {
        const m2s_status ws = warm_scene(c, warm_R, counted);
        if (ws != M2S_OK) { c->has_scene = false; return ws; }
    }
    c->last_upload_ms[4] = ms_since(t_warm);
    c->last_upload_ms[0] = ms_since(t_begin);
    return M2S_OK;
}

m2s_status m2s_prepare(m2s_ctx* c, uint32_t flags) {
    if (!c) return M2S_ERR_INVALID;
    HIPCHK(c, hipSetDevice(c->device));
    if (flags & M2S_PREPARE_UPLOAD) { const m2s_status s = ensure_stage(c); if (s != M2S_OK) return s; }
    if (flags & M2S_PREPARE_EXPORT)
        for (int k = 0; k < 2; ++k)
            M2S_TRY(c->h_export[k].ensure(c->err, m2s_ply::kChunkRows * sizeof(m2s_gaussian)));
    if ((flags & M2S_PREPARE_KERNELS) && !debug_on("M2S_NO_PRELOAD")) {
        HIPCHK(c, preload_fused2()); HIPCHK(c, preload_fused3()); HIPCHK(c, preload_sparse()); HIPCHK(c, preload_multipass());
        HIPCHK(c, preload_export()); HIPCHK(c, preload_prepass()); HIPCHK(c, preload_sort()); HIPCHK(c, preload_splat()); HIPCHK(c, preload_light()); HIPCHK(c, preload_meshdepth()); HIPCHK(c, preload_meshrender()); HIPCHK(c, preload_score());
    }
    return M2S_OK;
}

m2s_status m2s_last_upload_ms(const m2s_ctx* c, float out_ms[4]) {
    if (!c || !out_ms) return M2S_ERR_INVALID;
    memcpy(out_ms, c->last_upload_ms, 4 * sizeof(float));
    return M2S_OK;
}

float m2s_last_warm_ms(const m2s_ctx* c) { return c ? c->last_upload_ms[4] : 0.0f; }

m2s_status m2s_set_resolution_hint(m2s_ctx* c, uint32_t R) {
    if (!c) return M2S_ERR_INVALID;
    if (R > 4096) return fail(c, M2S_ERR_INVALID, "R must be in [0, 4096]");
    c->hint_R = R;
    return M2S_OK;
}

}
```

Measured before the change: 27.86 billion.

## Deduplicate triangle vertices into an indexed vertex table for the fused3 emit kernel

Builds a vertex table on the device at upload time: triangle corners are hashed and deduplicated, unique rows holding position, normal and extra attributes are emitted, and each triangle stores three packed 21-bit vertex ids. The fused3 kernel gets an indexed variant that fetches positions, normals and D-attributes through these ids instead of per-triangle planes, and derives combo mip offsets from the level rather than storing them. The aim is to cut per-triangle attribute bandwidth in the shading loop when vertices are shared. In exchange it adds an upload-time hash and scan pass, extra device memory, and an extra level of indirection in loads.

New measurement: 28.40 billion, median of 6. 1.9% higher.

```diff
diff --git a/__graft_entry__.py b/__graft_entry__.py
--- a/__graft_entry__.py
+++ b/__graft_entry__.py
@@ -14,6 +14,7 @@
     subprocess.run(["make", "-C", os.path.join(ROOT, "oracle"), "all"], check=True, stdout=subprocess.DEVNULL)
     subprocess.run(["make", "-C", os.path.join(ROOT, "tests", "stub_rccl")], check=True, stdout=subprocess.DEVNULL)
     subprocess.run(["make", "-C", os.path.join(ROOT, "tests", "exact_math")], check=True, stdout=subprocess.DEVNULL)
+    subprocess.run(["make", "-C", os.path.join(ROOT, "tests", "vdedup")], check=True, stdout=subprocess.DEVNULL)
     import mesh2splat_amd
 
 
diff --git a/include/m2s.h b/include/m2s.h
--- a/include/m2s.h
+++ b/include/m2s.h
@@ -327,6 +327,7 @@
        M2S_PIPELINE_LEAN = 5  };
 m2s_status m2s_set_pipeline(m2s_ctx* ctx, int pipeline);
 int m2s_last_pipeline(const m2s_ctx* ctx);
+m2s_status m2s_vertex_table(const m2s_ctx* ctx, uint64_t* out_rows, int* out_in_use);
 
 enum { M2S_K_COUNT = 0, M2S_K_SCAN = 1, M2S_K_OFFSETS = 2, M2S_K_EMIT = 3, M2S_K_FUSED = 4, M2S_K_N = 5 };
 m2s_status m2s_set_profiling(m2s_ctx* ctx, int enabled);
diff --git a/mesh2splat_amd/_lib.py b/mesh2splat_amd/_lib.py
--- a/mesh2splat_amd/_lib.py
+++ b/mesh2splat_amd/_lib.py
@@ -44,6 +44,7 @@
     "m2s_device_sorted_sources", "m2s_download_sorted_sources", "m2s_upload_quad_sources", "m2s_contrib_begin", "m2s_contrib_accumulate", "m2s_device_contrib",
     "m2s_download_contrib", "m2s_last_contrib_ms", "m2s_last_contrib_stage_ms", "m2s_prune", "m2s_last_prune_counts", "m2s_last_prune_ms",
     "m2s_write_ply_compact", "m2s_export_ply_compact", "m2s_last_compact_stage_ms",
+    "m2s_vertex_table",
 )
 
 
@@ -249,6 +250,7 @@
         "m2s_write_ply_compact": (C.c_int, [C.c_char_p, vp, vp, u32, u64, C.c_float, C.POINTER(u64)]),
         "m2s_export_ply_compact": (C.c_int, [vp, C.c_char_p, C.c_float, C.c_int, C.POINTER(u64)]),
         "m2s_last_compact_stage_ms": (C.c_int, [vp, C.POINTER(C.c_float)]),
+        "m2s_vertex_table": (C.c_int, [vp, C.POINTER(u64), C.POINTER(C.c_int)]),
     }
     for name, (res, args) in sigs.items():
         fn = getattr(L, name)
diff --git a/mesh2splat_amd/converter.py b/mesh2splat_amd/converter.py
--- a/mesh2splat_amd/converter.py
+++ b/mesh2splat_amd/converter.py
@@ -787,6 +787,11 @@
     def last_pipeline(self) -> str:
         return {0: "none", 1: "multipass", 3: "team", 4: "sparse", 5: "lean"}[self._L.m2s_last_pipeline(self._h)]
 
+    def vertex_table(self) -> dict:
+        rows, used = C.c_uint64(0), C.c_int(0)
+        self._check(self._L.m2s_vertex_table(self._h, C.byref(rows), C.byref(used)))
+        return {"rows": int(rows.value), "in_use": bool(used.value)}
+
     def set_profiling(self, on: bool):
         self._check(self._L.m2s_set_profiling(self._h, 1 if on else 0))
 
diff --git a/mesh2splat_amd/csrc/m2s_context.cpp b/mesh2splat_amd/csrc/m2s_context.cpp
--- a/mesh2splat_amd/csrc/m2s_context.cpp
+++ b/mesh2splat_amd/csrc/m2s_context.cpp
@@ -41,6 +41,8 @@
     c->warm_R = 0; c->warm_total = 0; c->warm_mismatch_seen = false;
     c->sparse_off_R = c->team_off_R = c->lean_off_R = UINT32_MAX;
     c->lean_ok = false;
+    c->d_vt_rows.release(); c->d_vt_ids.release();
+    c->vt_rows = 0; c->vt_use = false;
     c->scene = SceneDev{};
     c->has_scene = false;
 }
@@ -219,6 +221,13 @@
 
 int m2s_last_pipeline(const m2s_ctx* c) { return c ? c->last_pipeline : 0; }
 
+m2s_status m2s_vertex_table(const m2s_ctx* c, uint64_t* out_rows, int* out_in_use) {
+    if (!c) return M2S_ERR_INVALID;
+    if (out_rows) *out_rows = c->vt_rows;
+    if (out_in_use) *out_in_use = c->vt_use ? 1 : 0;
+    return M2S_OK;
+}
+
 int m2s_positions_ready(const m2s_ctx* c) {
     return c && c->d_pos_plane && c->last_records && c->pos_plane_of == c->last_records && c->pos_plane_n == c->last_stored &&
            c->pos_plane_epoch == c->records_epoch && c->last_stored ? 1 : 0;
diff --git a/mesh2splat_amd/csrc/m2s_ctx.h b/mesh2splat_amd/csrc/m2s_ctx.h
--- a/mesh2splat_amd/csrc/m2s_ctx.h
+++ b/mesh2splat_amd/csrc/m2s_ctx.h
@@ -2,6 +2,7 @@
 #include "../../include/m2s.h"
 #include "m2s_devbuf.h"
 #include "m2s_device.h"
+#include "m2s_vdedup.h"
 
 #include <cstdint>
 #include <cstdlib>
@@ -43,6 +44,10 @@
     bool has_scene = false;
     bool lean_ok = false;
     uint64_t range_first = 0, range_count = UINT64_MAX;
+    m2s_host::DevBuf<float4> d_vt_rows;
+    m2s_host::DevBuf<m2s::VtIds> d_vt_ids;
+    uint32_t vt_rows = 0;
+    bool vt_use = false;
 
     uint32_t* d_cnt = nullptr;
     uint32_t* d_off = nullptr;
diff --git a/mesh2splat_amd/csrc/m2s_devfn.h b/mesh2splat_amd/csrc/m2s_devfn.h
--- a/mesh2splat_amd/csrc/m2s_devfn.h
+++ b/mesh2splat_amd/csrc/m2s_devfn.h
@@ -1,6 +1,7 @@
 #pragma once
 #include "m2s_device.h"
 #include "m2s_exact.h"
+#include "m2s_vtable.h"
 
 #pragma clang fp contract(off)
 
@@ -593,6 +594,19 @@
     uint32_t mesh;
 };
 static_assert(sizeof(TriShadeS) == 64, "TriShadeS must be four float4");
+
+struct TriShadeSI {
+    short a1, b1, a2, b2;
+    int e1, e2;
+    float inva, sx, sy, lod0;
+    float4 rot;
+    uint32_t vid_lo, vid_hi;
+    uint32_t org;
+    uint32_t mesh;
+};
+static_assert(sizeof(TriShadeSI) == 64, "TriShadeSI must be four float4");
+template <class TS> inline constexpr bool kTsHasIds = false;
+template <> inline constexpr bool kTsHasIds<TriShadeSI> = true;
 
 __device__ __forceinline__ float lod_from_grad(float fw, float fh, float dudx, float dvdx, float dudy, float dvdy) {
     const float sx = dudx * fw, tx = dvdx * fh, sy = dudy * fw, ty = dvdy * fh;
@@ -798,8 +812,16 @@
 __device__ __forceinline__ void combo_issue(MP mp, TD t, float uf, float vf, const TS& ts, ComboFetch& cf) {
     const uint32_t w = t->w, h = t->h;
     const float f = ts.lod0;
-    const uint32_t off0 = __float_as_uint(ts.lod1), off1 = __float_as_uint(ts.lod2);
     const uint32_t l0 = (ts.mesh >> 24) & 15u, l1 = ts.mesh >> 28;
+    uint32_t off0, off1;
+    if constexpr (kTsHasIds<TS>) {
+        const uint32_t c1 = mp->combo.coff[1], c2 = mp->combo.coff[2], c3 = mp->combo.coff[3], c4 = mp->combo.coff[4];
+        off0 = l0 == 0 ? 0u : l0 == 1 ? c1 : l0 == 2 ? c2 : l0 == 3 ? c3 : c4;
+        off1 = l1 == 0 ? 0u : l1 == 1 ? c1 : l1 == 2 ? c2 : l1 == 3 ? c3 : c4;
+    } else {
+        off0 = __float_as_uint(ts.lod1);
+        off1 = __float_as_uint(ts.lod2);
+    }
     const uint32_t* __restrict__ base = mp->combo.texels;
     ComboTap& tlo = cf.tlo;
     ComboTap& thi = cf.thi;
@@ -853,12 +875,21 @@
     }
 }
 
+__device__ __forceinline__ float4 ld_row4(const float4* rows, uint32_t id, uint32_t k) {
+    return *reinterpret_cast<const float4*>(reinterpret_cast<const char*>(rows) + (size_t)(id * 48u + k * 16u));
+}
+struct RowXYZ { float x, y, z; };
+__device__ __forceinline__ RowXYZ ld_row3(const float4* rows, uint32_t id, uint32_t k) {
+    const float* p = reinterpret_cast<const float*>(__builtin_assume_aligned(reinterpret_cast<const char*>(rows) + (size_t)(id * 48u + k * 16u), 16));
+    return RowXYZ{ p[0], p[1], p[2] };
+}
+
 
 template <class MP, class TS = TriShade, bool kComboOnly = false, bool kStreamAttr = false>
 __device__ __forceinline__ void shade_from_tri(const TriPlanes& tp, uint32_t t, int x, int y, MP mp,
                                                const TS& ts, float4 rec[6], unsigned long long* stamps = nullptr,
                                                const float2* uvl = nullptr ,
-                                               const float* posl = nullptr ) {
+                                               const float4* vrows = nullptr ) {
     const int dx256 = (x - (int)(ts.org & 0xFFFu)) * 256, dy256 = (y - (int)(ts.org >> 12)) * 256;
     float l1, l2;
     if constexpr (sizeof(ts.e1) == 4) {
@@ -879,19 +910,22 @@
         b0 = ld_plane(tp.B0, t);
         b1 = ld_plane(tp.B1, t);
     }
-    float4 a0, a1;
-    float a2;
-    if (posl == nullptr) {
+    float4 a0, a1, c0, c1, d0, d1, d2;
+    float a2, c2;
+    if constexpr (kTsHasIds<TS>) {
+        uint32_t i0, i1, i2;
+        vt_unpack(VtIds{ ts.vid_lo, ts.vid_hi }, i0, i1, i2);
+        const RowXYZ p0 = ld_row3(vrows, i0, 0), p1 = ld_row3(vrows, i1, 0), p2 = ld_row3(vrows, i2, 0);
+        const RowXYZ n0 = ld_row3(vrows, i0, 1), n1 = ld_row3(vrows, i1, 1), n2 = ld_row3(vrows, i2, 1);
+        d0 = ld_row4(vrows, i0, 2); d1 = ld_row4(vrows, i1, 2); d2 = ld_row4(vrows, i2, 2);
+        a0 = make_float4(p0.x, p0.y, p0.z, p1.x); a1 = make_float4(p1.y, p1.z, p2.x, p2.y); a2 = p2.z;
+        c0 = make_float4(n0.x, n0.y, n0.z, n1.x); c1 = make_float4(n1.y, n1.z, n2.x, n2.y); c2 = n2.z;
+    } else {
         a0 = ld_plane(tp.A0, t); a1 = ld_plane(tp.A1, t);
         a2 = ld_plane(tp.A2, t);
-    }
-    const float4 c0 = ld_attr<kStreamAttr>(tp.C0, t), c1 = ld_attr<kStreamAttr>(tp.C1, t);
-    const float c2 = ld_attr<kStreamAttr>(tp.C2, t);
-    const float4 d0 = ld_attr<kStreamAttr>(tp.D0, t), d1 = ld_attr<kStreamAttr>(tp.D1, t), d2 = ld_attr<kStreamAttr>(tp.D2, t);
-    if (posl != nullptr) {
-        a0 = make_float4(posl[0], posl[1], posl[2], posl[3]);
-        a1 = make_float4(posl[4], posl[5], posl[6], posl[7]);
-        a2 = posl[8];
+        c0 = ld_attr<kStreamAttr>(tp.C0, t); c1 = ld_attr<kStreamAttr>(tp.C1, t);
+        c2 = ld_attr<kStreamAttr>(tp.C2, t);
+        d0 = ld_attr<kStreamAttr>(tp.D0, t); d1 = ld_attr<kStreamAttr>(tp.D1, t); d2 = ld_attr<kStreamAttr>(tp.D2, t);
     }
     float U, V;
     {
diff --git a/mesh2splat_amd/csrc/m2s_device.h b/mesh2splat_amd/csrc/m2s_device.h
--- a/mesh2splat_amd/csrc/m2s_device.h
+++ b/mesh2splat_amd/csrc/m2s_device.h
@@ -2,6 +2,8 @@
 #include <cstdlib>
 #include <hip/hip_runtime.h>
 #include <stdint.h>
+
+#include "m2s_vtable.h"
 
 namespace m2s {
 
@@ -131,7 +133,7 @@
                    const RunInfo& runs, const BatchTable& batches, hipStream_t st);
 void launch_fused3(const SceneDev& sc, uint32_t R, unsigned long long* chain, uint64_t limit, float4* out,
                    unsigned long long* total, uint32_t* status, uint32_t epoch, BigItem* biglist, uint32_t* bigmeta,
-                   const RunInfo& runs, const BatchTable& batches, hipStream_t st);
+                   const RunInfo& runs, const BatchTable& batches, hipStream_t st, const VtxTable* vt = nullptr);
 void launch_sparse(const SceneDev& sc, uint32_t R, unsigned long long* chain, uint64_t limit, float4* out,
                    unsigned long long* total, uint32_t* status, uint32_t epoch, BigItem* biglist, uint32_t* bigmeta,
                    const RunInfo& runs, hipStream_t st, float4* plane = nullptr);
diff --git a/mesh2splat_amd/csrc/m2s_fused3.hip b/mesh2splat_amd/csrc/m2s_fused3.hip
--- a/mesh2splat_amd/csrc/m2s_fused3.hip
+++ b/mesh2splat_amd/csrc/m2s_fused3.hip
@@ -1,4 +1,6 @@
 #include "m2s_fused_common.h"
+
+#include <type_traits>
 
 #pragma clang fp contract(off)
 
@@ -111,13 +113,17 @@
 #define TLFV(k, v) do { } while (0)
 #endif
 
+struct VtNone { };
+template <bool kIndexed>
 __global__ void __launch_bounds__(kL3Threads, M2S_FUSED3_WAVES) k_fused3(SceneDev sc, uint32_t R, unsigned long long* __restrict__ chain,
                                                       unsigned long long limit, float4* __restrict__ out,
                                                       unsigned long long* __restrict__ total_out,
                                                       uint32_t* __restrict__ status , uint32_t epoch,
                                                       BigItem* __restrict__ biglist, uint32_t* __restrict__ bigmeta,
                                                       uint32_t tpw ,
-                                                      RunInfo runs, BatchTable bt) {
+                                                      RunInfo runs, BatchTable bt,
+                                                      std::conditional_t<kIndexed, VtxTable, VtNone> vt) {
+    using TS = std::conditional_t<kIndexed, TriShadeSI, TriShadeS>;
     __shared__ F3Lds S;
     F3Ctl& C = S.ctl;
     const int lane = threadIdx.x & 63;
@@ -180,6 +186,7 @@
         uint32_t m = 0;
         float4 uvb0 = make_float4(0, 0, 0, 0);
         float2 uvb1 = make_float2(0, 0);
+        [[maybe_unused]] uint2 vid = make_uint2(0, 0);
         bool uniform_mesh = false;
         uint32_t m0 = 0;
         if (has_batch) {
@@ -190,6 +197,7 @@
                 load_positions(sc.tri, t, p);
                 uvb0 = sc.tri.B0[t];
                 uvb1 = sc.tri.B1[t];
+                if constexpr (kIndexed) vid = ld_plane(reinterpret_cast<const uint2*>(vt.ids), t);
                 if (uniform_mesh) geo_setup_mp(p, kConstMesh(sc.meshes + m0), g);
                 else { m = find_mesh(sc, sc.tri_first + t); geo_setup_mp(p, sc.meshes + m, g); }
                 box = raster_head(g, R, h);
@@ -213,7 +221,9 @@
             else tri_shade_small(p, g, h, rs, sc.meshes + m, uvb0, uvb1, m, c);
             const float4* src = reinterpret_cast<const float4*>(&c);
 #pragma unroll
-            for (int k = 0; k < 4; ++k) S.tri[wave][lane * 4 + k] = src[k];
+            for (int k = 0; k < 3; ++k) S.tri[wave][lane * 4 + k] = src[k];
+            if constexpr (kIndexed) S.tri[wave][lane * 4 + 3] = make_float4(__uint_as_float(vid.x), __uint_as_float(vid.y), src[3].z, src[3].w);
+            else S.tri[wave][lane * 4 + 3] = src[3];
             float2* const uvs = &S.uv[wave][lane * 3];
             uvs[0] = make_float2(uvb0.x, uvb0.y);
             uvs[1] = make_float2(uvb0.z - uvb0.x, uvb0.w - uvb0.y);
@@ -402,7 +412,7 @@
             const uint32_t m_now = __builtin_amdgcn_readlane(my_mesh, __ffsll((long long)todo) - 1);
             const bool mine = have && my_mesh == m_now;
             if (mine) {
-                const TriShadeS& ts = *reinterpret_cast<const TriShadeS*>(&S.tri[ow][tl * 4]);
+                const TS& ts = *reinterpret_cast<const TS*>(&S.tri[ow][tl * 4]);
                 const uint32_t tt = C.t0[ow] + tl;
                 const uint32_t org = ts.org;
                 const int x = (int)(org & 0xFFFu) + (int)(bit & 7u), y = (int)(org >> 12) + (int)(bit >> 3);
@@ -411,13 +421,10 @@
 #else
                 const float2* const uvl = &S.uv[ow][tl * 3];
 #endif
-#ifdef M2S_FUSED3_ABL_POS
-                const float* const posl = reinterpret_cast<const float*>(&S.tri[ow][tl * 4]);
-#else
-                const float* const posl = nullptr;
-#endif
-                shade_from_tri<ConstMeshPtr, TriShadeS, true, kF3StreamAttr>(sc.tri, tt, x, y, kConstMesh(sc.meshes + __builtin_amdgcn_readfirstlane(my_mesh)),
-                                                                              ts, rec, nullptr, uvl, posl);
+                const float4* vrows = nullptr;
+                if constexpr (kIndexed) vrows = reinterpret_cast<const float4*>(vt.rows);
+                shade_from_tri<ConstMeshPtr, TS, true, kF3StreamAttr>(sc.tri, tt, x, y, kConstMesh(sc.meshes + __builtin_amdgcn_readfirstlane(my_mesh)),
+                                                                       ts, rec, nullptr, uvl, vrows);
             }
             todo &= ~__ballot(mine);
         }
@@ -481,7 +488,7 @@
 
 void launch_fused3(const SceneDev& sc, uint32_t R, unsigned long long* chain, uint64_t limit, float4* out,
                    unsigned long long* total, uint32_t* status, uint32_t epoch, BigItem* biglist, uint32_t* bigmeta,
-                   const RunInfo& runs, const BatchTable& bt, hipStream_t st) {
+                   const RunInfo& runs, const BatchTable& bt, hipStream_t st, const VtxTable* vt) {
     const uint32_t tpw = fused_tpw(sc.n_tri);
     const uint32_t n_batches = bt.first ? bt.n : n_fused_waves(sc.n_tri);
     if (!n_batches) return;
@@ -491,8 +498,12 @@
     if (r.base) r.out = nullptr;
     if (r.base) nb = ((nb + (8u << r.shift) - 1u) / (8u << r.shift)) * (8u << r.shift);
     else nb = (nb + 7u) & ~7u;
-    hipLaunchKernelGGL(k_fused3, dim3(nb), dim3(kL3Threads), 0, st, sc, R, chain, (unsigned long long)limit, out, total, status,
-                       epoch & 0xFFFFu, biglist, bigmeta, tpw, r, bt);
+    if (vt && vt->rows && vt->ids)
+        hipLaunchKernelGGL(k_fused3<true>, dim3(nb), dim3(kL3Threads), 0, st, sc, R, chain, (unsigned long long)limit, out, total, status,
+                           epoch & 0xFFFFu, biglist, bigmeta, tpw, r, bt, *vt);
+    else
+        hipLaunchKernelGGL(k_fused3<false>, dim3(nb), dim3(kL3Threads), 0, st, sc, R, chain, (unsigned long long)limit, out, total, status,
+                           epoch & 0xFFFFu, biglist, bigmeta, tpw, r, bt, VtNone{});
 }
 
 #ifdef M2S_TIMELINE
@@ -507,7 +518,7 @@
 }
 namespace m2s {
 #endif
-uint32_t fused3_resident_workgroups() { return resident_workgroups(reinterpret_cast<const void*>(&k_fused3), kL3Threads); }
-hipError_t preload_fused3() { hipFuncAttributes a; return hipFuncGetAttributes(&a, reinterpret_cast<const void*>(&k_fused3)); }
-
-}
+uint32_t fused3_resident_workgroups() { return resident_workgroups(reinterpret_cast<const void*>(&k_fused3<false>), kL3Threads); }
+hipError_t preload_fused3() { hipFuncAttributes a; return hipFuncGetAttributes(&a, reinterpret_cast<const void*>(&k_fused3<false>)); }
+
+}
diff --git a/mesh2splat_amd/csrc/m2s_pass.cpp b/mesh2splat_amd/csrc/m2s_pass.cpp
--- a/mesh2splat_amd/csrc/m2s_pass.cpp
+++ b/mesh2splat_amd/csrc/m2s_pass.cpp
@@ -60,8 +60,11 @@
     uint32_t* status = reinterpret_cast<uint32_t*>(&res[1]);
     if (ri.form == M2S_PIPELINE_SPARSE)
         launch_sparse(c->scene, R, chain, limit, d_out, &res[0], status, epoch, c->d_biglist, c->d_bigmeta, runs, st, plane);
-    else if (ri.form == M2S_PIPELINE_LEAN)
-        launch_fused3(c->scene, R, chain, limit, d_out, &res[0], status, epoch, c->d_biglist, c->d_bigmeta, runs, batches_for(c, ri), st);
+    else if (ri.form == M2S_PIPELINE_LEAN) {
+        const VtxTable vt{ c->d_vt_rows.get(), c->d_vt_ids.get() };
+        launch_fused3(c->scene, R, chain, limit, d_out, &res[0], status, epoch, c->d_biglist, c->d_bigmeta, runs, batches_for(c, ri), st,
+                      c->vt_use ? &vt : nullptr);
+    }
     else
         launch_fused2(c->scene, R, chain, limit, d_out, &res[0], status, epoch, c->d_biglist, c->d_bigmeta, runs, batches_for(c, ri), st);
 }
diff --git a/mesh2splat_amd/csrc/m2s_upload.cpp b/mesh2splat_amd/csrc/m2s_upload.cpp
--- a/mesh2splat_amd/csrc/m2s_upload.cpp
+++ b/mesh2splat_amd/csrc/m2s_upload.cpp
@@ -254,6 +254,12 @@
     const bool warm = !debug_on("M2S_NO_WARM");
     bool counted = false;
     if (warm && !debug_on("M2S_NO_WARM_OVERLAP")) counted = warm_count_enqueue(c, warm_R) == M2S_OK;
+    VtWork vt_work;
+    bool vt_begun = false;
+    if (vt_size_ok(c->lean_ok, n_tri) && !debug_on("M2S_NO_VTABLE")) {
+        vt_begun = vt_dedup_begin(tp, n_tri, vt_work, c->stream) == hipSuccess;
+        if (!vt_begun) (void)hipGetLastError();
+    }
 
     for (TexPlan& p : tex_plan) {
         uint32_t* mem = (uint32_t*)(A + p.arena_off);
@@ -273,6 +279,13 @@
     }
     HIPCHK(c, hipStreamSynchronize(c->stream));
     HIPCHK(c, hipGetLastError());
+    if (vt_begun) {
+        if (vt_dedup_finish(tp, n_tri, vt_work, kVtIdLimit, kVtMinSharing, c->d_vt_rows, c->d_vt_ids, &c->vt_rows, &c->vt_use, c->stream) != hipSuccess) {
+            (void)hipGetLastError();
+            c->d_vt_rows.release(); c->d_vt_ids.release();
+            c->vt_use = false;
+        }
+    }
     c->last_upload_ms[2] = ms_since(t_tex);
     c->has_scene = true;
     const auto t_warm = std::chrono::steady_clock::now();
diff --git a/mesh2splat_amd/csrc/m2s_vdedup.h b/mesh2splat_amd/csrc/m2s_vdedup.h
--- /dev/null
+++ b/mesh2splat_amd/csrc/m2s_vdedup.h
@@ -0,0 +1,25 @@
+#pragma once
+#include "m2s_devbuf.h"
+#include "m2s_device.h"
+#include "m2s_vtable.h"
+
+namespace m2s {
+
+struct VtWork {
+    void* mem = nullptr;
+    uint32_t *table = nullptr, *owner = nullptr, *flags = nullptr, *rank = nullptr;
+    void* temp = nullptr;
+    size_t temp_bytes = 0;
+    uint32_t corners = 0;
+    VtWork() = default;
+    VtWork(const VtWork&) = delete;
+    VtWork& operator=(const VtWork&) = delete;
+    ~VtWork() { release(); }
+    void release();
+};
+uint32_t vt_hash_words(uint32_t corners);
+hipError_t vt_dedup_begin(const TriPlanes& tp, uint32_t n_tri, VtWork& w, hipStream_t st);
+hipError_t vt_dedup_finish(const TriPlanes& tp, uint32_t n_tri, VtWork& w, uint32_t id_limit, uint32_t min_sharing, m2s_host::DevBuf<float4>& rows,
+                           m2s_host::DevBuf<VtIds>& ids, uint32_t* n_rows, bool* eligible, hipStream_t st);
+
+}
diff --git a/mesh2splat_amd/csrc/m2s_vdedup.hip b/mesh2splat_amd/csrc/m2s_vdedup.hip
--- /dev/null
+++ b/mesh2splat_amd/csrc/m2s_vdedup.hip
@@ -0,0 +1,175 @@
+#include "m2s_vdedup.h"
+
+#include <rocprim/device/device_scan.hpp>
+
+namespace m2s {
+namespace {
+constexpr uint32_t kVtEmpty = 0xFFFFFFFFu;
+
+struct Planes32 {
+    const uint32_t *A0, *A1, *A2, *B0, *B1, *C0, *C1, *C2, *D0, *D1, *D2;
+};
+__host__ Planes32 as_words(const TriPlanes& tp) {
+    return Planes32{ (const uint32_t*)tp.A0, (const uint32_t*)tp.A1, (const uint32_t*)tp.A2, (const uint32_t*)tp.B0, (const uint32_t*)tp.B1,
+                     (const uint32_t*)tp.C0, (const uint32_t*)tp.C1, (const uint32_t*)tp.C2, (const uint32_t*)tp.D0, (const uint32_t*)tp.D1,
+                     (const uint32_t*)tp.D2 };
+}
+__device__ __forceinline__ uint32_t word9(const uint32_t* p0, const uint32_t* p1, const uint32_t* p2, uint32_t t, uint32_t j) {
+    return j < 4u ? p0[4u * t + j] : j < 8u ? p1[4u * t + (j - 4u)] : p2[t];
+}
+__device__ __forceinline__ void load_corner(const Planes32& P, uint32_t c, uint32_t k[12]) {
+    const uint32_t t = c / 3u, v = c - 3u * t;
+#pragma unroll
+    for (uint32_t i = 0; i < 3u; ++i) {
+        k[i] = word9(P.A0, P.A1, P.A2, t, 3u * v + i);
+        k[4u + i] = word9(P.C0, P.C1, P.C2, t, 3u * v + i);
+    }
+    k[3] = v < 2u ? P.B0[4u * t + 2u * v] : P.B1[2u * t];
+    k[7] = v < 2u ? P.B0[4u * t + 2u * v + 1u] : P.B1[2u * t + 1u];
+    const uint32_t* d = v == 0u ? P.D0 : v == 1u ? P.D1 : P.D2;
+#pragma unroll
+    for (uint32_t i = 0; i < 4u; ++i) k[8u + i] = d[4u * t + i];
+}
+__device__ __forceinline__ uint32_t hash12(const uint32_t k[12]) {
+    uint32_t h = 0x9E3779B9u;
+#pragma unroll
+    for (int i = 0; i < 12; ++i) {
+        h = (h ^ k[i]) * 0x85EBCA6Bu;
+        h ^= h >> 13;
+    }
+    h *= 0xC2B2AE35u;
+    return h ^ (h >> 16);
+}
+
+__global__ void __launch_bounds__(256) k_vt_insert(Planes32 P, uint32_t n_tri, uint32_t* table, uint32_t mask, uint32_t* __restrict__ slot_of) {
+    const uint32_t t = blockIdx.x * 256u + threadIdx.x;
+    if (t >= n_tri) return;
+    for (uint32_t v = 0; v < 3u; ++v) {
+        const uint32_t c = 3u * t + v;
+        uint32_t key[12];
+        load_corner(P, c, key);
+        uint32_t slot = hash12(key) & mask;
+        for (;;) {
+            uint32_t cur = __hip_atomic_load(&table[slot], __ATOMIC_RELAXED, __HIP_MEMORY_SCOPE_AGENT);
+            if (cur == kVtEmpty) {
+                cur = atomicCAS(&table[slot], kVtEmpty, c);
+                if (cur == kVtEmpty) break;
+            }
+            uint32_t other[12];
+            load_corner(P, cur, other);
+            bool same = true;
+#pragma unroll
+            for (int i = 0; i < 12; ++i) same = same && key[i] == other[i];
+            if (same) { atomicMin(&table[slot], c); break; }
+            slot = (slot + 1u) & mask;
+        }
+        slot_of[c] = slot;
+    }
+}
+
+__global__ void __launch_bounds__(256) k_vt_flags(const uint32_t* __restrict__ table, uint32_t corners, uint32_t* __restrict__ slot_of, uint32_t* __restrict__ flags) {
+    const uint32_t c = blockIdx.x * 256u + threadIdx.x;
+    if (c > corners) return;
+    if (c == corners) { flags[c] = 0u; return; }
+    const uint32_t own = table[slot_of[c]];
+    slot_of[c] = own;
+    flags[c] = own == c ? 1u : 0u;
+}
+
+__global__ void __launch_bounds__(256) k_vt_emit(Planes32 P, uint32_t n_tri, const uint32_t* __restrict__ owner, const uint32_t* __restrict__ rank,
+                                                  uint32_t n_rows, uint4* __restrict__ rows, VtIds* __restrict__ ids) {
+    const uint32_t t = blockIdx.x * 256u + threadIdx.x;
+    if (t >= n_tri) return;
+    uint32_t id[3];
+#pragma unroll
+    for (uint32_t v = 0; v < 3u; ++v) {
+        const uint32_t c = 3u * t + v, own = owner[c];
+        id[v] = rank[own];
+        if (own == c && id[v] < n_rows) {
+            uint32_t k[12];
+            load_corner(P, c, k);
+            uint4* r = rows + (size_t)id[v] * kVtRowF4;
+            r[0] = make_uint4(k[0], k[1], k[2], k[3]);
+            r[1] = make_uint4(k[4], k[5], k[6], k[7]);
+            r[2] = make_uint4(k[8], k[9], k[10], k[11]);
+        }
+    }
+    ids[t] = vt_pack(id[0], id[1], id[2]);
+}
+
+size_t scan_temp_bytes(uint32_t n) {
+    size_t b = 0;
+    (void)rocprim::exclusive_scan(nullptr, b, (const uint32_t*)nullptr, (uint32_t*)nullptr, 0u, (size_t)n, rocprim::plus<uint32_t>(), (hipStream_t)0);
+    return b < 256 ? 256 : b;
+}
+}
+
+uint32_t vt_hash_words(uint32_t corners) {
+    uint32_t w = 1024u;
+    while (w < 2u * corners) w <<= 1;
+    return w;
+}
+
+void VtWork::release() {
+    if (mem) (void)hipFree(mem);
+    mem = nullptr;
+    table = owner = flags = rank = nullptr;
+    temp = nullptr;
+    temp_bytes = 0;
+    corners = 0;
+}
+
+hipError_t vt_dedup_begin(const TriPlanes& tp, uint32_t n_tri, VtWork& w, hipStream_t st) {
+    w.release();
+    if (n_tri == 0 || n_tri > kVtMaxTriangles) return hipErrorInvalidValue;
+    const uint32_t corners = 3u * n_tri, words = vt_hash_words(corners);
+    const size_t tb = scan_temp_bytes(corners + 1u);
+    auto up = [](size_t v) { return (v + 255) / 256 * 256; };
+    const size_t o_owner = up((size_t)words * 4), o_flags = o_owner + up((size_t)corners * 4), o_rank = o_flags + up(((size_t)corners + 1) * 4),
+                 o_temp = o_rank + up(((size_t)corners + 1) * 4);
+    hipError_t e = hipMalloc(&w.mem, o_temp + tb);
+    if (e != hipSuccess) { w.mem = nullptr; return e; }
+    char* const m = (char*)w.mem;
+    w.table = (uint32_t*)m; w.owner = (uint32_t*)(m + o_owner); w.flags = (uint32_t*)(m + o_flags); w.rank = (uint32_t*)(m + o_rank);
+    w.temp = m + o_temp;
+    w.temp_bytes = tb;
+    w.corners = corners;
+    const Planes32 P = as_words(tp);
+    if ((e = hipMemsetAsync(w.table, 0xFF, (size_t)words * 4, st)) != hipSuccess) return e;
+    hipLaunchKernelGGL(k_vt_insert, dim3((n_tri + 255u) / 256u), dim3(256), 0, st, P, n_tri, w.table, words - 1u, w.owner);
+    hipLaunchKernelGGL(k_vt_flags, dim3((corners + 1u + 255u) / 256u), dim3(256), 0, st, (const uint32_t*)w.table, corners, w.owner, w.flags);
+    size_t bytes = w.temp_bytes;
+    if ((e = rocprim::exclusive_scan(w.temp, bytes, (const uint32_t*)w.flags, w.rank, 0u, (size_t)corners + 1u, rocprim::plus<uint32_t>(), st)) != hipSuccess) return e;
+    return hipGetLastError();
+}
+
+hipError_t vt_dedup_finish(const TriPlanes& tp, uint32_t n_tri, VtWork& w, uint32_t id_limit, uint32_t min_sharing, m2s_host::DevBuf<float4>& rows,
+                           m2s_host::DevBuf<VtIds>& ids, uint32_t* n_rows, bool* eligible, hipStream_t st) {
+    *n_rows = 0;
+    *eligible = false;
+    if (!w.rank || w.corners != 3u * n_tri) { w.release(); return hipErrorInvalidValue; }
+    uint32_t U = 0;
+    hipError_t e = hipMemcpyAsync(&U, w.rank + w.corners, sizeof(U), hipMemcpyDeviceToHost, st);
+    if (e == hipSuccess) e = hipStreamSynchronize(st);
+    if (e != hipSuccess) { w.release(); return e; }
+    *n_rows = U;
+    if (vt_rows_ok(U, w.corners, id_limit, min_sharing)) {
+        std::string err;
+        rows.release();
+        ids.release();
+        if (rows.reserve(err, (uint64_t)U * kVtRowF4, sizeof(float4)) != M2S_OK || ids.reserve(err, n_tri, sizeof(VtIds)) != M2S_OK) {
+            rows.release(); ids.release(); w.release();
+            (void)hipGetLastError();
+            return hipErrorOutOfMemory;
+        }
+        hipLaunchKernelGGL(k_vt_emit, dim3((n_tri + 255u) / 256u), dim3(256), 0, st, as_words(tp), n_tri, (const uint32_t*)w.owner, (const uint32_t*)w.rank, U,
+                           reinterpret_cast<uint4*>(rows.get()), ids.get());
+        e = hipGetLastError();
+        if (e == hipSuccess) e = hipStreamSynchronize(st);
+        *eligible = e == hipSuccess;
+    }
+    w.release();
+    return e;
+}
+
+}
diff --git a/mesh2splat_amd/csrc/m2s_vtable.h b/mesh2splat_amd/csrc/m2s_vtable.h
--- /dev/null
+++ b/mesh2splat_amd/csrc/m2s_vtable.h
@@ -0,0 +1,40 @@
+#pragma once
+#include <stdint.h>
+
+#if defined(__HIPCC__) || defined(__CUDACC__)
+#define M2S_VT_HD __host__ __device__ inline
+#else
+#define M2S_VT_HD inline
+#endif
+
+namespace m2s {
+
+constexpr uint32_t kVtRowF4 = 3;
+constexpr uint32_t kVtIdBits = 21;
+constexpr uint32_t kVtIdLimit = 1u << kVtIdBits;
+constexpr uint32_t kVtMaxTriangles = 1u << 22;
+constexpr uint32_t kVtMinSharing = 2;
+
+struct VtIds { uint32_t lo, hi; };
+M2S_VT_HD VtIds vt_pack(uint32_t i0, uint32_t i1, uint32_t i2) {
+    const unsigned long long w = (unsigned long long)i0 | ((unsigned long long)i1 << kVtIdBits) | ((unsigned long long)i2 << (2 * kVtIdBits));
+    return VtIds{ (uint32_t)w, (uint32_t)(w >> 32) };
+}
+M2S_VT_HD void vt_unpack(VtIds p, uint32_t& i0, uint32_t& i1, uint32_t& i2) {
+    const uint32_t m = kVtIdLimit - 1u;
+    i0 = p.lo & m;
+    i1 = ((p.lo >> kVtIdBits) | (p.hi << (32u - kVtIdBits))) & m;
+    i2 = (p.hi >> (2u * kVtIdBits - 32u)) & m;
+}
+
+M2S_VT_HD bool vt_size_ok(bool lean_ok, uint64_t n_tri) { return lean_ok && n_tri >= 1 && n_tri <= kVtMaxTriangles; }
+M2S_VT_HD bool vt_rows_ok(uint64_t rows, uint64_t corners, uint32_t id_limit, uint32_t min_sharing) {
+    return rows >= 1 && rows < id_limit && rows * min_sharing <= corners;
+}
+
+struct VtxTable {
+    const void* rows;
+    const void* ids;
+};
+
+}
```
